# 77even/Fast-nnUNet

Measured on AMD Instinct MI355X. Metric: 3d_fullres patches/sec (distilled r=2 student, sliding window, one 512^3 CT; volume resident in HBM at step start; step ends with: fp16 logits resident in HBM), higher is better.
Workload: dtype f16; 1 GPU; bone_turbo_r2: PlainConvUNet student r=2, features [16, 32, 64, 128, 160, 160], 1 input channel, patch 160x96x96, 61 classes, 512^3 volume, tile_step_size 0.5, Gaussian on, mirroring off, 600 patches/volume; patches_per_forward=32, folds=1, accumulators=fp16, step_output=fp16 logits [heads, X, Y, Z] in HBM (predict_sliding_window_return_logits), gpu_max_hw_queues=4, parallelism=single GPU

## Files before the change

fast-nnunet_amd/csrc/conv3d.hip:

```cpp
#include "fnn_device.h"
#include "conv_common.h"
#include <cstdlib>

template <int NB>
__global__ __launch_bounds__(256) void conv3d_mfma_kernel(const ConvParams p) {
    extern __shared__ __attribute__((aligned(16))) char smem[];
    const int tid = threadIdx.x, lane = tid & 63, wave = tid >> 6;

    int t = blockIdx.x;
    const int tw = t % p.tiles_w; t /= p.tiles_w;
    const int th = t % p.tiles_h; t /= p.tiles_h;
    const int td = t % p.tiles_d;
    const int n = t / p.tiles_d;
    const int cb0 = blockIdx.y * NB;

    const int od0 = td * FNN_TILE_D, oh0 = th * FNN_TILE_H, ow0 = tw * FNN_TILE_W;
    const int ID = (FNN_TILE_D - 1) * p.sd + p.kd;
    const int IH = (FNN_TILE_H - 1) * p.sh + p.kh;
    const int IW = (FNN_TILE_W - 1) * p.sw + p.kw;
    const int IVOX = ID * IH * IW;
    const int T = p.kd * p.kh * p.kw;
    const int cin_total = p.chunks * 16;

    char *sA = smem;
    char *sB = sA + ((IVOX * 32 + 1023) & ~1023);
    int *sOff = (int *)(sB + p.ksteps * NB * 1024);
    float2 *sSS = (float2 *)(sOff + ((IVOX + 3) & ~3));
    int *sTap = (int *)(sSS + cin_total);

    {
        const int id0 = od0 * p.sd - p.pd, ih0 = oh0 * p.sh - p.ph, iw0 = ow0 * p.sw - p.pw;
        for (int v = tid; v < IVOX; v += 256) {
            const int zw = v % IW, zh = (v / IW) % IH, zd = v / (IW * IH);
            const int gd = id0 + zd, gh = ih0 + zh, gw = iw0 + zw;
            const bool ok = gd >= 0 && gd < p.Di && gh >= 0 && gh < p.Hi && gw >= 0 && gw < p.Wi;
            sOff[v] = ok ? ((n * p.Di + gd) * p.Hi + gh) * p.Wi + gw : -1;
        }
        if (tid < 2 * p.ksteps) {
            int off = 0;
            if (tid < T) {
                const int a = tid / (p.kh * p.kw), b = (tid / p.kw) % p.kh, c = tid % p.kw;
                off = ((a * IH + b) * IW + c) * 32;
            }
            sTap[tid] = off;
        }
        for (int c = tid; c < cin_total; c += 256) {
            const int s = (c < p.src[0].C) ? 0 : 1;
            const int cl = c - (s ? p.src[0].C : 0);
            sSS[c] = p.src[s].ss ? make_float2(p.src[s].ss[(size_t)(2 * n) * p.src[s].C + cl], p.src[s].ss[(size_t)(2 * n + 1) * p.src[s].C + cl])
                                 : make_float2(1.f, 0.f);
        }
    }

    int base[4];
#pragma unroll
    for (int mb = 0; mb < 4; ++mb) {
        const int r = lane & 15;
        const int oh_l = 2 * mb + (r >> 3), ow_l = r & 7;
        base[mb] = ((wave * p.sd * IH + oh_l * p.sh) * IW + ow_l * p.sw) * 32 + ((lane >> 4) & 1) * 16;
    }

    f32x4 acc[4][NB];
#pragma unroll
    for (int mb = 0; mb < 4; ++mb)
#pragma unroll
        for (int nb = 0; nb < NB; ++nb) acc[mb][nb] = (f32x4){0.f, 0.f, 0.f, 0.f};

    __syncthreads();

    const int cg = tid & 1;
    for (int ch = 0; ch < p.chunks; ++ch) {
        const int c_glob = ch * 16;
        const int s = (c_glob < p.src[0].C) ? 0 : 1;
        const int c_loc = c_glob - (s ? p.src[0].C : 0) + cg * 8;
        const int sC = p.src[s].C;
        const size_t nvox = (size_t)n * p.Di * p.Hi * p.Wi;
        const int vs = FNN_VS(p.src[s]);
        const f16 *sp = p.src[s].ptr + nvox * sC + (c_loc >> 4) * FNN_CS(p.src[s]) + (c_loc & 15);
        const f16 slope_h = (f16)p.src[s].slope;
        float sc[8], sh[8];
#pragma unroll
        for (int j = 0; j < 8; ++j) {
            const float2 v = sSS[c_glob + cg * 8 + j];
            sc[j] = v.x; sh[j] = v.y;
        }
        for (int base = tid; base < IVOX * 2; base += 256 * 8) {
            int off[8];
            f16x8 x[8];
#pragma unroll
            for (int u = 0; u < 8; ++u) {
                const int idx = base + u * 256;
                off[u] = idx < IVOX * 2 ? sOff[idx >> 1] : -2;
            }
#pragma unroll
            for (int u = 0; u < 8; ++u)
                x[u] = *(const f16x8 *)(sp + (off[u] >= 0 ? (size_t)off[u] - nvox : 0) * vs);
#pragma unroll
            for (int u = 0; u < 8; ++u) {
                if (off[u] == -2) continue;
                f16x8 o;
                if (off[u] >= 0) {
#pragma unroll
                    for (int j = 0; j < 8; ++j) o[j] = (f16)fmaf((float)x[u][j], sc[j], sh[j]);
                    o = __builtin_elementwise_max(o, o * slope_h);
                } else {
#pragma unroll
                    for (int j = 0; j < 8; ++j) o[j] = (f16)0.f;
                }
                *(f16x8 *)(sA + ((base + u * 256) >> 1) * 32 + cg * 16) = o;
            }
        }
        {
            const int per_nb = p.ksteps * 64;
            const int total = NB * per_nb;
            for (int base = tid; base < total; base += 256 * 8) {
                uint4 v[8];
#pragma unroll
                for (int u = 0; u < 8; ++u) {
                    const int idx = base + u * 256;
                    const int idc = idx < total ? idx : 0;
                    const int nb = idc / per_nb, r = idc - nb * per_nb;
                    v[u] = ((const uint4 *)(p.wpk + ((size_t)((cb0 + nb) * p.chunks + ch) * p.ksteps) * 512))[r];
                }
#pragma unroll
                for (int u = 0; u < 8; ++u) {
                    const int idx = base + u * 256;
                    if (idx < total) ((uint4 *)sB)[idx] = v[u];
                }
            }
        }
        __syncthreads();

        for (int ks = 0; ks < p.ksteps; ++ks) {
            const int toff = sTap[2 * ks + (lane >> 5)];
            f16x8 xf[4];
#pragma unroll
            for (int mb = 0; mb < 4; ++mb) xf[mb] = *(const f16x8 *)(sA + base[mb] + toff);
#pragma unroll
            for (int nb = 0; nb < NB; ++nb) {
                const f16x8 wf = *(const f16x8 *)(sB + ((nb * p.ksteps + ks) * 64 + lane) * 16);
#pragma unroll
                for (int mb = 0; mb < 4; ++mb)
                    acc[mb][nb] = __builtin_amdgcn_mfma_f32_16x16x32_f16(wf, xf[mb], acc[mb][nb], 0, 0, 0);
            }
        }
        __syncthreads();
    }

    const int q = lane >> 4, r = lane & 15;
    const int od = od0 + wave;
    float s1[NB][4], s2[NB][4];
#pragma unroll
    for (int nb = 0; nb < NB; ++nb)
#pragma unroll
        for (int j = 0; j < 4; ++j) { s1[nb][j] = 0.f; s2[nb][j] = 0.f; }

#pragma unroll
    for (int mb = 0; mb < 4; ++mb) {
        const int oh = oh0 + 2 * mb + (r >> 3), ow = ow0 + (r & 7);
        const bool ok = od < p.Do && oh < p.Ho && ow < p.Wo;
        const size_t vox = ((size_t)od * p.Ho + oh) * p.Wo + ow;
        f16 *outn = p.out + (size_t)n * p.Do * p.Ho * p.Wo * p.Cout;
#pragma unroll
        for (int nb = 0; nb < NB; ++nb) {
            const int co = (cb0 + nb) * 16 + q * 4;
            const float4 bv = *(const float4 *)(p.bias + co);
            f16x4 o;
            o[0] = (f16)(acc[mb][nb][0] + bv.x);
            o[1] = (f16)(acc[mb][nb][1] + bv.y);
            o[2] = (f16)(acc[mb][nb][2] + bv.z);
            o[3] = (f16)(acc[mb][nb][3] + bv.w);
            if (ok) {
                *(f16x4 *)(outn + vox * FNN_OVS(p) + (co >> 4) * FNN_OCS(p) + (co & 15)) = o;
#pragma unroll
                for (int j = 0; j < 4; ++j) {
                    const float v = (float)o[j];
                    s1[nb][j] += v; s2[nb][j] += v * v;
                }
            }
        }
    }
    if (p.stats_out) {
#pragma unroll
        for (int nb = 0; nb < NB; ++nb)
#pragma unroll
            for (int j = 0; j < 4; ++j) {
#pragma unroll
                for (int m = 1; m < 16; m <<= 1) {
                    s1[nb][j] += __shfl_xor(s1[nb][j], m, 64);
                    s2[nb][j] += __shfl_xor(s2[nb][j], m, 64);
                }
            }
        float *sRed = (float *)smem;
        if (r == 0) {
#pragma unroll
            for (int nb = 0; nb < NB; ++nb)
#pragma unroll
                for (int j = 0; j < 4; ++j) {
                    const int c = nb * 16 + q * 4 + j;
                    sRed[(wave * NB * 16 + c) * 2] = s1[nb][j];
                    sRed[(wave * NB * 16 + c) * 2 + 1] = s2[nb][j];
                }
        }
        __syncthreads();
        if (tid < NB * 16 * 2) {
            const int c = tid >> 1, which = tid & 1;
            double v = 0;
#pragma unroll
            for (int w = 0; w < 4; ++w) v += (double)sRed[(w * NB * 16 + c) * 2 + which];
            double *dst = p.stats_out + (((size_t)n * FNN_STAT_REPL + (blockIdx.x & (FNN_STAT_REPL - 1))) * p.Cout
                                         + cb0 * 16 + c) * 2 + which;
            unsafeAtomicAdd(dst, v);
        }
    }
}

static int lds_pitch(int IW) { return (IW & 7) ? ((IW + 3) & ~7) + 4 : IW; }

template <int NB, int MB, int PF>
__global__ __launch_bounds__(256, 2) void conv3d_lds_kernel(const ConvParams p) {
    extern __shared__ __attribute__((aligned(16))) char smem[];
    const int tid = threadIdx.x, lane = tid & 63, wave = tid >> 6;
    FNN_STAMP_DECL
    FNN_STAMP();
    constexpr int TD = MB == 2 ? 2 : MB;

    int t = fnn_xcd_tile(gridDim.x, blockIdx.x);
    const int tw = t % p.tiles_w; t /= p.tiles_w;
    const int th = t % p.tiles_h; t /= p.tiles_h;
    const int td = t % p.tiles_d;
    const int n = t / p.tiles_d;
    const int cb0 = blockIdx.y * NB;

    const int od0 = td * TD, oh0 = th * FNN_TILE_H, ow0 = tw * FNN_TILE_W;
    const int ID = (TD - 1) * p.sd + p.kd, IH = (FNN_TILE_H - 1) * p.sh + p.kh, IW = (FNN_TILE_W - 1) * p.sw + p.kw;
    const int IVOX = ID * IH * IW;
    const int T = p.kd * p.kh * p.kw;
    const int swz = p.sw == 1 && (IW & 7) != 0;
    const int PWp = swz ? ((IW + 3) & ~7) + 4 : IW;
    const int abytes = (ID * IH * PWp * 32 + 1023) & ~1023;

    constexpr int WPF = (NB * 14 * 64 + 255) / 256;
    char *sA0 = smem;
    char *sW = smem + abytes;
    int *sTap = (int *)(sW + NB * p.ksteps * 1024);
    float *sBias = (float *)(sTap + 4 * p.ksteps + 4);

    {
        if (tid < 2 * p.ksteps) {
            int off = 0, par = 0;
            if (tid < T) {
                const int a = tid / (p.kh * p.kw), b = (tid / p.kw) % p.kh, c = tid % p.kw;
                off = ((a * IH + b) * PWp + c) * 32;
                par = swz & b & 1;
            }
            sTap[tid * 2] = off + 16 * par;
            sTap[tid * 2 + 1] = off + 16 * (1 - par);
        }
        if (tid >= 64 && tid < 64 + NB * 16) sBias[tid - 64] = p.bias[cb0 * 16 + tid - 64];
    }

    int base[MB];
#pragma unroll
    for (int mb = 0; mb < MB; ++mb) {
        const int r = lane & 15;
        int od_l, oh_l, ow_l;
        mb_coords<MB>(wave, mb, r, od_l, oh_l, ow_l);
        base[mb] = ((od_l * p.sd * IH + oh_l * p.sh) * PWp + ow_l * p.sw) * 32;
    }
    const int kgp = ((lane >> 4) & 1) ^ (swz & ((lane & 15) >> 3));

    f32x4 acc[MB][NB];
#pragma unroll
    for (int mb = 0; mb < MB; ++mb)
#pragma unroll
        for (int nb = 0; nb < NB; ++nb) acc[mb][nb] = (f32x4){0.f, 0.f, 0.f, 0.f};

    const int per_nb = p.ksteps * 64;
    const int wtotal = NB * per_nb;
    f16x8 wr[WPF];
    int wofs[WPF];
#pragma unroll
    for (int u = 0; u < WPF; ++u) {
        const int idx = tid + u * 256;
        const int idc = idx < wtotal ? idx : wtotal - 1;
        const int nb = (idc >= per_nb) + (idc >= 2 * per_nb) + (idc >= 3 * per_nb);
        wofs[u] = (cb0 + nb) * p.chunks * per_nb + idc - nb * per_nb;
    }
    float4 scr[2], shr[2];
    float slope_next = 1.f;
    __syncthreads();

    const int cg = tid & 1;
    int offv[PF];
    int ldso[PF];
    {
        const int id0 = od0 * p.sd - p.pd, ih0 = oh0 * p.sh - p.ph, iw0 = ow0 * p.sw - p.pw;
        const float rcp_iw = 1.0f / (float)IW, rcp_ih = 1.0f / (float)IH;
#pragma unroll
        for (int u = 0; u < PF; ++u) {
            const int idx = tid + u * 256;
            const int v = idx >> 1;
            const int row = small_div(v, IW, rcp_iw), zw = v - row * IW;
            const int zd = small_div(row, IH, rcp_ih), zh = row - zd * IH;
            const int gd = id0 + zd, gh = ih0 + zh, gw = iw0 + zw;
            const bool ok = gd >= 0 && gd < p.Di && gh >= 0 && gh < p.Hi && gw >= 0 && gw < p.Wi;
            offv[u] = idx < IVOX * 2 ? (ok ? ((n * p.Di + gd) * p.Hi + gh) * p.Wi + gw : -1) : -2;
            ldso[u] = ((zd * IH + zh) * PWp + zw) * 32 + ((cg ^ (swz & zh & 1)) * 16);
        }
    }
    f16x8 xr[PF];

    auto issue = [&](int ch) {
        const int c_glob = ch * 16;
        const int s = (c_glob < p.src[0].C) ? 0 : 1;
        const int sC = p.src[s].C, c_loc = c_glob - (s ? p.src[0].C : 0) + cg * 8;
        const size_t nvox = (size_t)n * p.Di * p.Hi * p.Wi;
        const int vs = FNN_VS(p.src[s]);
        const f16 *sp = p.src[s].ptr + nvox * sC + (c_loc >> 4) * FNN_CS(p.src[s]) + (c_loc & 15);
#pragma unroll
        for (int u = 0; u < PF; ++u)
            xr[u] = *(const f16x8 *)(sp + (offv[u] >= 0 ? (size_t)offv[u] - nvox : 0) * vs);
#pragma unroll
        for (int u = 0; u < WPF; ++u) wr[u] = ((const f16x8 *)p.wpk)[wofs[u] + ch * per_nb];
        slope_next = p.src[s].slope;
        if (p.src[s].ss) {
            const float *q4 = p.src[s].ss + (size_t)(2 * n) * sC + (c_glob - (s ? p.src[0].C : 0)) + cg * 8;
            scr[0] = *(const float4 *)q4; scr[1] = *(const float4 *)(q4 + 4);
            shr[0] = *(const float4 *)(q4 + sC); shr[1] = *(const float4 *)(q4 + sC + 4);
        } else {
            scr[0] = scr[1] = make_float4(1.f, 1.f, 1.f, 1.f);
            shr[0] = shr[1] = make_float4(0.f, 0.f, 0.f, 0.f);
        }
    };
    auto commit = [&](int ch, char *dst) {
        (void)ch;
        const f16 slope_h = (f16)slope_next;
        const float sc[8] = {scr[0].x, scr[0].y, scr[0].z, scr[0].w, scr[1].x, scr[1].y, scr[1].z, scr[1].w};
        const float sh[8] = {shr[0].x, shr[0].y, shr[0].z, shr[0].w, shr[1].x, shr[1].y, shr[1].z, shr[1].w};
#pragma unroll
        for (int u = 0; u < PF; ++u) {
            if (u * 256 >= IVOX * 2 || offv[u] == -2) continue;
            f16x8 o;
            if (offv[u] >= 0) {
#pragma unroll
                for (int j = 0; j < 8; ++j) o[j] = (f16)fmaf((float)xr[u][j], sc[j], sh[j]);
                o = __builtin_elementwise_max(o, o * slope_h);
            } else {
#pragma unroll
                for (int j = 0; j < 8; ++j) o[j] = (f16)0.f;
            }
            *(f16x8 *)(dst + ldso[u]) = o;
        }
#pragma unroll
        for (int u = 0; u < WPF; ++u) {
            const int idx = tid + u * 256;
            if (idx < wtotal) ((f16x8 *)sW)[idx] = wr[u];
        }
    };

    FNN_STAMP();
    issue(0);
    FNN_STAMP();
    commit(0, sA0);
    __syncthreads();
    FNN_STAMP();

    auto kloop = [&]() {
        for (int ks = 0; ks < p.ksteps; ++ks) {
            const int toff = sTap[(2 * ks + (lane >> 5)) * 2 + kgp];
            f16x8 xf[MB];
#pragma unroll
            for (int mb = 0; mb < MB; ++mb) xf[mb] = *(const f16x8 *)(sA0 + base[mb] + toff);
#pragma unroll
            for (int nb = 0; nb < NB; ++nb) {
                const f16x8 wf = *(const f16x8 *)(sW + ((nb * p.ksteps + ks) * 64 + lane) * 16);
#pragma unroll
                for (int mb = 0; mb < MB; ++mb)
                    acc[mb][nb] = __builtin_amdgcn_mfma_f32_16x16x32_f16(wf, xf[mb], acc[mb][nb], 0, 0, 0);
            }
        }
    };
    for (int ch = 0; ch + 1 < p.chunks; ++ch) {
        issue(ch + 1);
        kloop();
        FNN_STAMP();
        __syncthreads();
        commit(ch + 1, sA0);
        __syncthreads();
        FNN_STAMP();
    }
    kloop();
    FNN_STAMP();
    __syncthreads();

    {
        float4 bv[NB];
#pragma unroll
        for (int nb = 0; nb < NB; ++nb) bv[nb] = *(const float4 *)(sBias + nb * 16 + (lane >> 4) * 4);
        float t1[NB][4], t2[NB][4];
#pragma unroll
        for (int nb = 0; nb < NB; ++nb)
#pragma unroll
            for (int j = 0; j < 4; ++j) { t1[nb][j] = 0.f; t2[nb][j] = 0.f; }
        tile_epilogue<NB, MB>(p, acc, bv, n, od0, oh0, ow0, cb0, wave, lane, t1, t2);
        if (p.stats_out) stats_to_global<NB>(p, t1, t2, (float *)smem, n, cb0, wave, lane, tid);
    }
    FNN_STAMP();
    FNN_STAMP_FLUSH(p.dbg);
}

static size_t ldsk_lds_bytes(const ConvParams &p, int nb, int mb) {
    const int td = mb == 2 ? 2 : mb;
    const int ID = (td - 1) * p.sd + p.kd, IH = (FNN_TILE_H - 1) * p.sh + p.kh, IW = (FNN_TILE_W - 1) * p.sw + p.kw;
    const int pitch = p.sw == 1 ? lds_pitch(IW) : IW;
    size_t b = (size_t)((ID * IH * pitch * 32 + 1023) & ~1023) + (size_t)nb * p.ksteps * 1024;
    b += 4 * p.ksteps * 4 + 16 + (size_t)nb * 16 * 4 + 64;
    const size_t red = (size_t)4 * nb * 16 * 2 * 4;
    return b > red ? b : red;
}

template <int NB, int MB, int PF = 8>
static int launch_ldsk(ConvParams p, hipStream_t st) {
    constexpr int TD = MB == 2 ? 2 : MB;
    p.tile_d = TD;
    p.tiles_d = (p.Do + TD - 1) / TD;
    p.tiles_h = (p.Ho + FNN_TILE_H - 1) / FNN_TILE_H;
    p.tiles_w = (p.Wo + FNN_TILE_W - 1) / FNN_TILE_W;
    const size_t lds = ldsk_lds_bytes(p, NB, MB);
    dim3 grid(p.N * p.tiles_d * p.tiles_h * p.tiles_w, (p.Cout / 16) / NB);
    return fnn_launch_lds<conv3d_lds_kernel<NB, MB, PF>>(grid, dim3(256), lds, st, p);
}

template <int NB, int MB, bool WRES, int KS, int CH, int PF = 8, bool SBUF = false>
__global__ __launch_bounds__(256, (NB == 1 && MB == 4 && WRES && PF == 4) ? 3 : 2) void conv3d_persist_kernel(const ConvParams p, const int total_tiles) {
    extern __shared__ __attribute__((aligned(16))) char smem[];
    const int tid = threadIdx.x, lane = tid & 63, wave = tid >> 6;
    FNN_STAMP_DECL
    constexpr int TD = MB;

    const int ID = (TD - 1) * p.sd + p.kd, IH = (FNN_TILE_H - 1) * p.sh + p.kh, IW = (FNN_TILE_W - 1) * p.sw + p.kw;
    const int IVOX = ID * IH * IW;
    const int T = p.kd * p.kh * p.kw;
    const int TS = p.chunks * p.ksteps;
    const int swz = p.sw == 1 && (IW & 7) != 0;
    const int PWp = swz ? ((IW + 3) & ~7) + 4 : IW;
    const int abytes = (ID * IH * PWp * 32 + 1023) & ~1023;
    const int cb0 = blockIdx.y * NB;

    constexpr int NBUF = (WRES && !SBUF) ? 2 : 1;
    constexpr int WPF = WRES ? 1 : (NB * 14 * 64 + 255) / 256;
    char *sA0 = smem;
    char *sW = smem + NBUF * abytes;
    int *sTap = (int *)(sW + NB * (WRES ? TS : p.ksteps) * 1024);
    double *sRed = (double *)(sTap + 64);

    int t_begin, t_end;
    {
        const int nwg = gridDim.x, bid = blockIdx.x;
        const int g = fnn_xcd_tile(nwg, bid);
        t_begin = (int)((long long)total_tiles * g / nwg);
        t_end = (int)((long long)total_tiles * (g + 1) / nwg);
    }
    if (t_begin >= t_end) return;

    if (WRES) {
        for (int idx = tid; idx < NB * TS * 64; idx += 256) {
            const int nb = idx / (TS * 64), r = idx - nb * (TS * 64);
            ((uint4 *)sW)[idx] = ((const uint4 *)(p.wpk + (size_t)(cb0 + nb) * TS * 512))[r];
        }
    }
    const int per_nb = p.ksteps * 64, wtotal = NB * per_nb;
    f16x8 wr[WPF];
    int wofs[WPF];
#pragma unroll
    for (int u = 0; u < WPF; ++u) {
        const int idx = tid + u * 256;
        const int idc = idx < wtotal ? idx : wtotal - 1;
        const int nb = idc / per_nb, r = idc - nb * per_nb;
        wofs[u] = (cb0 + nb) * p.chunks * per_nb + r;
    }
    if (tid < 2 * p.ksteps) {
        int off = 0, par = 0;
        if (tid < T) {
            const int a = tid / (p.kh * p.kw), b = (tid / p.kw) % p.kh, c = tid % p.kw;
            off = ((a * IH + b) * PWp + c) * 32;
            par = swz & b & 1;
        }
        sTap[tid * 2] = off + 16 * par;
        sTap[tid * 2 + 1] = off + 16 * (1 - par);
    }
    const int cg = tid & 1;
    constexpr bool REL_LDS = false && PF >= 12;
    int *sRel = (int *)(sRed + 4 * NB * 16 * 2) + tid;
    int relr[REL_LDS ? 1 : PF];
#pragma unroll
    for (int u = 0; u < PF; ++u) {
        const int idx = tid + u * 256;
        const int v = idx >> 1;
        const int zw = v % IW, zh = (v / IW) % IH, zd = v / (IW * IH);
        const int rv = idx < IVOX * 2 ? (zd << 16) | (zh << 8) | zw : -1;
        if (REL_LDS) sRel[u * 256] = rv; else relr[REL_LDS ? 0 : u] = rv;
    }
#define FNN_REL(u) (REL_LDS ? sRel[(u) * 256] : relr[REL_LDS ? 0 : (u)])
    int base[MB];
#pragma unroll
    for (int mb = 0; mb < MB; ++mb) {
        const int r = lane & 15;
        int od_l, oh_l, ow_l;
        mb_coords<MB>(wave, mb, r, od_l, oh_l, ow_l);
        base[mb] = ((od_l * p.sd * IH + oh_l * p.sh) * PWp + ow_l * p.sw) * 32;
    }
    const int kgp = ((lane >> 4) & 1) ^ (swz & ((lane & 15) >> 3));

    f32x4 acc[MB][NB];
    for (int i = tid; i < 4 * NB * 16 * 2; i += 256) sRed[i] = 0.0;
    double dsum[NB][4][2];
#pragma unroll
    for (int nb = 0; nb < NB; ++nb)
#pragma unroll
        for (int j = 0; j < 4; ++j) { dsum[nb][j][0] = 0.0; dsum[nb][j][1] = 0.0; }

    float4 bv[NB];
#pragma unroll
    for (int nb = 0; nb < NB; ++nb) bv[nb] = *(const float4 *)(p.bias + (cb0 + nb) * 16 + (lane >> 4) * 4);

    int offv[PF];
    f16x8 xr[PF];
    float4 scr[2], shr[2];
    float slope_next = 1.f;

    auto tile_coords = [&](int t, int &n, int &od0, int &oh0, int &ow0) {
        const int tw = t % p.tiles_w; t /= p.tiles_w;
        const int th = t % p.tiles_h; t /= p.tiles_h;
        const int td = t % p.tiles_d;
        n = t / p.tiles_d;
        od0 = td * TD; oh0 = th * FNN_TILE_H; ow0 = tw * FNN_TILE_W;
    };
    auto next_tile = [&](int &n, int &od0, int &oh0, int &ow0) {
        ow0 += FNN_TILE_W;
        if (ow0 >= p.tiles_w * FNN_TILE_W) {
            ow0 = 0; oh0 += FNN_TILE_H;
            if (oh0 >= p.tiles_h * FNN_TILE_H) {
                oh0 = 0; od0 += TD;
                if (od0 >= p.tiles_d * TD) { od0 = 0; ++n; }
            }
        }
    };
    auto set_offsets = [&](int od0, int oh0, int ow0) {
        const int id0 = od0 * p.sd - p.pd, ih0 = oh0 * p.sh - p.ph, iw0 = ow0 * p.sw - p.pw;
#pragma unroll
        for (int u = 0; u < PF; ++u) {
            const int rel_u = FNN_REL(u);
            const unsigned gd = (unsigned)(id0 + (rel_u >> 16)), gh = (unsigned)(ih0 + ((rel_u >> 8) & 255)),
                           gw = (unsigned)(iw0 + (rel_u & 255));
            const bool ok = rel_u >= 0 && gd < (unsigned)p.Di && gh < (unsigned)p.Hi && gw < (unsigned)p.Wi;
            offv[u] = ok ? (int)(__umul24(__umul24(gd, (unsigned)p.Hi) + gh, (unsigned)p.Wi) + gw) : -1;
        }
    };
    auto issue = [&](int n, int ch) {
        const int c_glob = ch * 16;
        const int s = (c_glob < p.src[0].C) ? 0 : 1;
        const int c_loc = c_glob - (s ? p.src[0].C : 0) + cg * 8;
        const int sC = p.src[s].C;
        const int vs = FNN_VS(p.src[s]);
        const char *sp = (const char *)(p.src[s].ptr + (size_t)n * p.Di * p.Hi * p.Wi * sC + (c_loc >> 4) * FNN_CS(p.src[s]) + (c_loc & 15));
        slope_next = p.src[s].slope;
        const float *qs = p.src[s].ss ? p.src[s].ss + (size_t)(2 * n) * sC + c_loc : p.ident_ss + c_loc;
        const float *qh = p.src[s].ss ? qs + sC : p.ident_ss + 512 + c_loc;
        scr[0] = *(const float4 *)qs; scr[1] = *(const float4 *)(qs + 4);
        shr[0] = *(const float4 *)qh; shr[1] = *(const float4 *)(qh + 4);
        __builtin_amdgcn_sched_barrier(0);
#pragma unroll
        for (int u = 0; u < PF; ++u)
            xr[u] = *(const f16x8 *)(sp + (unsigned)((offv[u] >= 0 ? offv[u] : 0) * vs * 2));
        if (!WRES) {
#pragma unroll
            for (int u = 0; u < WPF; ++u) wr[u] = ((const f16x8 *)p.wpk)[wofs[u] + ch * per_nb];
        }
    };
    auto commit = [&](char *dst) {
        const f16 slope_h = (f16)slope_next;
        const float sc[8] = {scr[0].x, scr[0].y, scr[0].z, scr[0].w, scr[1].x, scr[1].y, scr[1].z, scr[1].w};
        const float sh[8] = {shr[0].x, shr[0].y, shr[0].z, shr[0].w, shr[1].x, shr[1].y, shr[1].z, shr[1].w};
#pragma unroll
        for (int u = 0; u < PF; ++u) {
            if (u * 256 >= IVOX * 2) continue;
            f16x8 o = fnn_norm_leaky8(xr[u], sc, sh, slope_h);
            if (offv[u] < 0) o = (f16x8){0, 0, 0, 0, 0, 0, 0, 0};
            const int rel_u = FNN_REL(u);
            const int zd = rel_u >> 16, zh = (rel_u >> 8) & 255, zw = rel_u & 255;
            if (rel_u >= 0) *(f16x8 *)(dst + ((zd * IH + zh) * PWp + zw) * 32 + ((cg ^ (swz & zh & 1)) * 16)) = o;
        }
        if (!WRES) {
#pragma unroll
            for (int u = 0; u < WPF; ++u) {
                const int idx = tid + u * 256;
                if (idx < wtotal) ((f16x8 *)sW)[idx] = wr[u];
            }
        }
    };
    auto flush_stats = [&](int n) {
        if (!p.stats_out) return;
        {
            const int q = lane >> 4;
#pragma unroll
            for (int nb = 0; nb < NB; ++nb)
#pragma unroll
                for (int j = 0; j < 4; ++j) {
                    const double a = row16_sum_f64(dsum[nb][j][0]), b = row16_sum_f64(dsum[nb][j][1]);
                    if ((lane & 15) == 0) {
                        double *slot = sRed + (wave * NB * 16 + nb * 16 + q * 4 + j) * 2;
                        slot[0] = a; slot[1] = b;
                    }
                    dsum[nb][j][0] = 0.0; dsum[nb][j][1] = 0.0;
                }
        }
        __syncthreads();
        if (tid < NB * 16 * 2) {
            const int c = tid >> 1, which = tid & 1;
            double v = 0;
#pragma unroll
            for (int w = 0; w < 4; ++w) { v += sRed[(w * NB * 16 + c) * 2 + which]; sRed[(w * NB * 16 + c) * 2 + which] = 0.0; }
            unsafeAtomicAdd(p.stats_out + (((size_t)n * FNN_STAT_REPL + (blockIdx.x & (FNN_STAT_REPL - 1))) * p.Cout
                                           + cb0 * 16 + c) * 2 + which, v);
        }
        __syncthreads();
    };

    int n_cur, od0, oh0, ow0;
    tile_coords(t_begin, n_cur, od0, oh0, ow0);
    set_offsets(od0, oh0, ow0);
    issue(n_cur, 0);
    commit(sA0);
    __syncthreads();
    int toffs[14];
    if (KS) {
#pragma unroll
        for (int ks = 0; ks < (KS < 14 ? KS : 14); ++ks) toffs[ks] = sTap[(2 * ks + (lane >> 5)) * 2 + kgp];
    }

    int buf = 0;
    for (int t = t_begin; t < t_end; ++t) {
#pragma unroll
        for (int mb = 0; mb < MB; ++mb)
#pragma unroll
            for (int nb = 0; nb < NB; ++nb) acc[mb][nb] = (f32x4){0.f, 0.f, 0.f, 0.f};
        int n_next = n_cur, nod0 = od0, noh0 = oh0, now0 = ow0;
        constexpr int CHU = CH ? CH : 1;
#pragma unroll CHU
        for (int ch = 0; ch < (CH ? CH : p.chunks); ++ch) {
#ifdef FNN_STAMPS
            const bool stamp_it = t == t_begin + 2 && ch == 0;
            if (stamp_it) FNN_STAMP();
#endif
            const bool last_chunk = ch + 1 == (CH ? CH : p.chunks);
            if (last_chunk) {
                if (t + 1 < t_end) next_tile(n_next, nod0, noh0, now0);
                set_offsets(nod0, noh0, now0);
                issue(n_next, 0);
            } else {
                issue(n_cur, ch + 1);
            }
#ifdef FNN_STAMPS
            if (stamp_it) FNN_STAMP();
#endif
            const char *sA = sA0 + (NBUF == 2 ? buf * abytes : 0);
#pragma unroll
            for (int ks = 0; ks < (KS ? KS : p.ksteps); ++ks) {
                const int toff = KS ? toffs[ks < 14 ? ks : 0] : sTap[(2 * ks + (lane >> 5)) * 2 + kgp];
                f16x8 xf[MB];
#pragma unroll
                for (int mb = 0; mb < MB; ++mb) xf[mb] = *(const f16x8 *)(sA + base[mb] + toff);
#pragma unroll
                for (int nb = 0; nb < NB; ++nb) {
                    const f16x8 wf = *(const f16x8 *)(sW + ((size_t)(WRES ? nb * TS + ch * p.ksteps + ks : nb * p.ksteps + ks) * 64 + lane) * 16);
#pragma unroll
                    for (int mb = 0; mb < MB; ++mb)
                        acc[mb][nb] = __builtin_amdgcn_mfma_f32_16x16x32_f16(wf, xf[mb], acc[mb][nb], 0, 0, 0);
                }
            }
#ifdef FNN_STAMPS
            if (stamp_it) FNN_STAMP();
#endif
            if (last_chunk) {
                float t1[NB][4], t2[NB][4];
#pragma unroll
                for (int nb = 0; nb < NB; ++nb)
#pragma unroll
                    for (int j = 0; j < 4; ++j) { t1[nb][j] = 0.f; t2[nb][j] = 0.f; }
                tile_epilogue<NB, MB>(p, acc, bv, n_cur, od0, oh0, ow0, cb0, wave, lane, t1, t2);
                if (p.stats_out) {
#pragma unroll
                    for (int nb = 0; nb < NB; ++nb)
#pragma unroll
                        for (int j = 0; j < 4; ++j) {
                            dsum[nb][j][0] += (double)t1[nb][j];
                            dsum[nb][j][1] += (double)t2[nb][j];
                        }
                }
                if (NBUF == 1) __syncthreads();
                commit(sA0 + (NBUF == 2 ? (buf ^ 1) * abytes : 0));
            } else {
                if (NBUF == 1) __syncthreads();
                commit(sA0 + (NBUF == 2 ? (buf ^ 1) * abytes : 0));
            }
#ifdef FNN_STAMPS
            if (stamp_it) FNN_STAMP();
#endif
            __syncthreads();
#ifdef FNN_STAMPS
            if (stamp_it) FNN_STAMP();
#endif
            buf ^= 1;
        }
        if (n_next != n_cur || t + 1 == t_end) flush_stats(n_cur);
        n_cur = n_next; od0 = nod0; oh0 = noh0; ow0 = now0;
    }
    FNN_STAMP_FLUSH(p.dbg);
#undef FNN_REL
}

static size_t persist_lds_bytes(const ConvParams &p, int nb, int mb, bool wres, bool sbuf = false, int pf = 8) {
    const int ID = (mb - 1) * p.sd + p.kd, IH = (FNN_TILE_H - 1) * p.sh + p.kh, IW = (FNN_TILE_W - 1) * p.sw + p.kw;
    const size_t ab = (size_t)((ID * IH * (p.sw == 1 ? lds_pitch(IW) : IW) * 32 + 1023) & ~1023);
    return (wres && !sbuf ? 2 : 1) * ab + (size_t)nb * (wres ? p.chunks : 1) * p.ksteps * 1024 + 256 + (size_t)4 * nb * 16 * 2 * 8 +
           (false && pf >= 12 ? (size_t)pf * 256 * 4 : 0);
}

template <int NB, int MB, bool WRES, int KS, int CH = 0, int PF = 8, bool SBUF = false>
static int launch_persist_ks(ConvParams p, int wgs_per_cu, hipStream_t st, int gx_exact = 0) {
    p.tile_d = MB;
    p.tiles_d = (p.Do + MB - 1) / MB;
    p.tiles_h = (p.Ho + FNN_TILE_H - 1) / FNN_TILE_H;
    p.tiles_w = (p.Wo + FNN_TILE_W - 1) / FNN_TILE_W;
    const int total = p.N * p.tiles_d * p.tiles_h * p.tiles_w;
    p.ident_ss = conv3d_identity_ss();
    if (!p.ident_ss) return -2;
    const size_t lds = persist_lds_bytes(p, NB, MB, WRES, SBUF, PF);
    int gx = gx_exact > 0 ? gx_exact : 256 * wgs_per_cu;
    if (gx > total) gx = total;
    dim3 grid(gx, (p.Cout / 16) / NB);
    return fnn_launch_lds<conv3d_persist_kernel<NB, MB, WRES, KS, CH, PF, SBUF>>(grid, dim3(256), lds, st, p, total);
}

static int launch_persist(const ConvParams &p, const ConvChoice &c, hipStream_t st) {
    const int mb = c.t[1], wres = c.t[2], ks = c.t[3], ch = c.t[4];
    if (c.t[0] == 2) return launch_persist_ks<2, 2, true, 0, 1, 12, true>(p, c.wpc, st, c.gx);
    if (ch == 1) return launch_persist_ks<1, 4, true, 5, 1, 4>(p, c.wpc, st);
    if (ch == 2) return launch_persist_ks<1, 4, true, 5, 2, 4>(p, c.wpc, st);
    if (mb == 8) {
        if (wres) return ks == 5 ? launch_persist_ks<1, 8, true, 5>(p, c.wpc, st) : launch_persist_ks<1, 8, true, 0>(p, c.wpc, st);
        return ks == 5 ? launch_persist_ks<1, 8, false, 5>(p, c.wpc, st) : launch_persist_ks<1, 8, false, 14>(p, c.wpc, st);
    }
    if (wres) return ks == 5 ? launch_persist_ks<1, 4, true, 5>(p, c.wpc, st) : launch_persist_ks<1, 4, true, 0>(p, c.wpc, st);
    return launch_persist_ks<1, 4, false, 5>(p, c.wpc, st);
}

size_t conv3d_lds_bytes(const ConvParams &p, int nb) {
    const int ID = (FNN_TILE_D - 1) * p.sd + p.kd;
    const int IH = (FNN_TILE_H - 1) * p.sh + p.kh;
    const int IW = (FNN_TILE_W - 1) * p.sw + p.kw;
    const int IVOX = ID * IH * IW;
    size_t b = (size_t)((IVOX * 32 + 1023) & ~1023);
    b += (size_t)p.ksteps * nb * 1024;
    b += (size_t)((IVOX + 3) & ~3) * 4;
    b += (size_t)p.chunks * 16 * 8;
    b += 2 * p.ksteps * 4 + 64;
    const size_t red = (size_t)4 * nb * 16 * 2 * 4;
    return b > red ? b : red;
}

const float *conv3d_identity_ss() {
    static const float *tab[16] = {nullptr};
    int dev = 0;
    if (hipGetDevice(&dev) != hipSuccess || dev < 0 || dev >= 16) return nullptr;
    if (!tab[dev]) {
        float h[1024];
        for (int i = 0; i < 512; ++i) { h[i] = 1.f; h[512 + i] = 0.f; }
        float *d = nullptr;
        if (hipMalloc((void **)&d, sizeof(h)) != hipSuccess) return nullptr;
        if (hipMemcpy(d, h, sizeof(h), hipMemcpyHostToDevice) != hipSuccess) { (void)hipFree(d); return nullptr; }
        tab[dev] = d;
    }
    return tab[dev];
}

const unsigned short *conv3d_identity_ssh() {
    static const unsigned short *tab[16] = {nullptr};
    int dev = 0;
    if (hipGetDevice(&dev) != hipSuccess || dev < 0 || dev >= 16) return nullptr;
    if (!tab[dev]) {
        unsigned short h[1024];
        for (int i = 0; i < 1024; ++i) h[i] = (i & 8) ? 0 : 0x3c00;
        unsigned short *d = nullptr;
        if (hipMalloc((void **)&d, sizeof(h)) != hipSuccess) return nullptr;
        if (hipMemcpy(d, h, sizeof(h), hipMemcpyHostToDevice) != hipSuccess) { (void)hipFree(d); return nullptr; }
        tab[dev] = d;
    }
    return tab[dev];
}

int conv3d_pick_nb(int nblk) { return (nblk % 4 == 0) ? 4 : (nblk % 2 == 0) ? 2 : 1; }

template <int NB>
static int launch_conv_nb(ConvParams p, hipStream_t st) {
    p.tile_d = FNN_TILE_D;
    p.tiles_d = (p.Do + FNN_TILE_D - 1) / FNN_TILE_D;
    p.tiles_h = (p.Ho + FNN_TILE_H - 1) / FNN_TILE_H;
    p.tiles_w = (p.Wo + FNN_TILE_W - 1) / FNN_TILE_W;
    const size_t lds = conv3d_lds_bytes(p, NB);
    dim3 grid(p.N * p.tiles_d * p.tiles_h * p.tiles_w, (p.Cout / 16) / NB);
    return fnn_launch_lds<conv3d_mfma_kernel<NB>>(grid, dim3(256), lds, st, p);
}

static void set_persist(ConvChoice &c, int nb, int mb, int wres, int ks, int ch, int pf, int sbuf, int wpc) {
    c.kernel = CK_PERSIST;
    const int t[7] = {nb, mb, wres, ks, ch, pf, sbuf};
    for (int i = 0; i < 7; ++i) c.t[i] = t[i];
    c.wpc = wpc;
    snprintf(c.name, sizeof c.name, "conv3d_persist_kernel<%d,%d,%d,%d,%d,%d,%d>", nb, mb, wres, ks, ch, pf, sbuf);
}

static void set_ldsk(ConvChoice &c, int nb, int mb, int pf) {
    c.kernel = CK_LDSK; c.t[0] = nb; c.t[1] = mb; c.t[2] = pf;
    snprintf(c.name, sizeof c.name, "conv3d_lds_kernel<%d,%d,%d>", nb, mb, pf);
}

static bool conv_choose_linear(const ConvParams &p_in, const ConvOverrides &o, ConvChoice &c) {
    ConvParams p = p_in;
    c.packing = FNN_PACK_LINEAR; c.ksteps = conv3d_ksteps(FNN_PACK_LINEAR, p.kd * p.kh * p.kw); c.chunks = p.chunks;
    p.ksteps = c.ksteps;
    p.tiles_h = (p.Ho + FNN_TILE_H - 1) / FNN_TILE_H;
    p.tiles_w = (p.Wo + FNN_TILE_W - 1) / FNN_TILE_W;
    const int plan_n = p.plan_N > 0 ? p.plan_N : p.N;
    int nb = conv3d_pick_nb(p.Cout / 16);
    if (!o.conv_v1 && p.sd == 1 && p.sh == 1 && p.sw == 1) {
        const int nblk = p.Cout / 16;
        const int cand[4][2] = {{2, 8}, {2, 4}, {1, 8}, {1, 4}};
        int pick = -1, best = -1;
        long long best_wgs = -1;
        for (int i = 0; i < 4; ++i) {
            const int cnb = cand[i][0], cmb = cand[i][1];
            if (nblk % cnb) continue;
            if (cmb == 8 && p.Do < 8) continue;
            const long long wgs = (long long)plan_n * ((p.Do + cmb - 1) / cmb) * p.tiles_h * p.tiles_w * (nblk / cnb);
            if (pick < 0 && wgs >= 768) pick = i;
            if (wgs > best_wgs) { best_wgs = wgs; best = i; }
        }
        if (pick < 0) pick = best;
        nb = cand[pick][0];
        const int mbsel = cand[pick][1];
        if (p.ksteps <= 14 && nb == 1) {
            for (int mb = mbsel; mb >= 4; mb -= 4) {
                const long long tiles = (long long)plan_n * ((p.Do + mb - 1) / mb) * p.tiles_h * p.tiles_w;
                if (tiles < 256LL * 2 * 4) continue;
                for (int wres = 1; wres >= 0; --wres) {
                    if (!wres && !(p.ksteps == 5 || (p.ksteps == 14 && mb == 8))) continue;
                    const size_t lds = persist_lds_bytes(p, nb, mb, wres != 0);
                    const int per_cu = (int)((160 * 1024) / lds);
                    if (per_cu < 2) continue;
                    const int wpc = per_cu > 3 ? 3 : per_cu;
                    if (wres && mb == 8 && p.ksteps == 5 && (p.chunks == 1 || p.chunks == 2)) {
                        const int ivox4 = (3 * p.sd + p.kd) * ((FNN_TILE_H - 1) * p.sh + p.kh) * ((FNN_TILE_W - 1) * p.sw + p.kw);
                        if (ivox4 * 2 <= 4 * 256 && persist_lds_bytes(p, 1, 4, true) * 3 <= 160 * 1024) {
                            set_persist(c, 1, 4, 1, 5, p.chunks, 4, 0, 3);
                            return true;
                        }
                    }
                    set_persist(c, 1, mb, wres, p.ksteps == 5 ? 5 : wres ? 0 : 14, 0, 8, 0, wpc);
                    return true;
                }
            }
        }
        if (p.ksteps <= 14) {
            set_ldsk(c, nb, mbsel, 8);
            return true;
        }
    }
    if (!o.conv_v1 && s2_choose(p, c)) return true;
    if (!o.conv_v1 && p.ksteps <= 14) {
        const int nbs = (p.Cout / 16) % 2 == 0 ? 2 : 1;
        const int ID = (2 - 1) * p.sd + p.kd, IH = (FNN_TILE_H - 1) * p.sh + p.kh, IW = (FNN_TILE_W - 1) * p.sw + p.kw;
        const long long tiles = (long long)plan_n * ((p.Do + 1) / 2) * p.tiles_h * p.tiles_w;
        const int groups = (p.Cout / 16) / nbs;
        if (nbs == 2 && ID * IH * IW * 2 <= 12 * 256 && persist_lds_bytes(p, 2, 2, false, false, 12) <= 80 * 1024 &&
            tiles >= 8LL * (512 / groups) && 512 / groups >= 8 && p.chunks == 1 && persist_lds_bytes(p, 2, 2, true, true, 12) <= 80 * 1024) {
            set_persist(c, 2, 2, 1, 0, 1, 12, 1, 2);
            c.gx = 512 / groups;
            return true;
        }
        if (ID * IH * IW * 2 <= 16 * 256 && ldsk_lds_bytes(p, nbs, 2) <= 80 * 1024) {
            set_ldsk(c, nbs, 2, ID * IH * IW * 2 <= 8 * 256 ? 8 : 16);
            return true;
        }
    }
    if (nb == 4 && conv3d_lds_bytes(p, 4) > 160 * 1024) nb = 2;
    if (conv3d_lds_bytes(p, nb) > 160 * 1024) return false;
    c.kernel = CK_NB; c.t[0] = nb;
    snprintf(c.name, sizeof c.name, "conv3d_mfma_kernel<%d> (generic fallback)", nb);
    return true;
}

ConvOverrides ConvOverrides::from_env() {
    ConvOverrides o;
    o.conv_v1 = fnn_knob("FNN_CONV_V1") != nullptr;
    o.no_row = fnn_knob("FNN_NO_ROW") != nullptr;
    o.no_stem_row = fnn_knob("FNN_NO_STEM_ROW") != nullptr;
    o.no_zr6 = fnn_knob("FNN_NO_ZR6") != nullptr;
    o.no_zrp = fnn_knob("FNN_NO_ZRP") != nullptr;
    o.no_zq12 = fnn_knob("FNN_NO_ZQ12") != nullptr;
    o.no_zsw = fnn_knob("FNN_NO_ZSW") != nullptr;
    o.no_zp = fnn_knob("FNN_NO_ZP") != nullptr;
    o.zp_no_half = fnn_knob("FNN_ZP_NO_HALF") != nullptr;
    o.zps_no_half = fnn_knob("FNN_ZPS_NO_HALF") != nullptr;
    if (const char *v = fnn_knob("FNN_ZR_MIN_WGS")) o.zr_min_wgs = atoi(v);
    if (const char *v = fnn_knob("FNN_FP8_LEVELS")) o.fp8_levels = atoi(v);
    return o;
}

bool conv_choose(const ThinParams &tp, const ConvOverrides &o, ConvChoice &c) {
    c = ConvChoice{};
    if (tp.fuse) {
        ConvChoice t;
        if (!thin_choose(tp, t)) return false;
        if (!row_choose(tp, o, c)) c = t;
        return true;
    }
    const ConvParams &p = tp.c;
    const unsigned long long out_item = 2ull * p.Do * p.Ho * p.Wo * p.Cout;
    unsigned long long in_item = 0;
    for (int i = 0; i < p.n_src; ++i) {
        const unsigned long long b = 2ull * p.Di * p.Hi * p.Wi * p.src[i].C;
        in_item = b > in_item ? b : in_item;
    }
    if (out_item >= (1ull << 31) || in_item >= (1ull << 32) || (long long)p.Di * p.Hi >= (1 << 24) || p.Wi >= (1 << 24)) return false;
    if (zp_choose(p, o, c) || zr_choose(p, o, c)) return true;
    c = ConvChoice{};
    return row_choose(tp, o, c) || conv_choose_linear(p, o, c);
}

bool conv_choose_fp8(ThinParams &tp, const ConvOverrides &o, ConvChoice &c) {
    ConvParams &p = tp.c;
    if (p.fp8 && !(p.kd * p.kh * p.kw == 27 && p.sd == 1 && p.sh == 1 && p.sw == 1)) p.fp8 = 0;
    bool ok = conv_choose(tp, o, c);
    if (p.fp8 && c.packing != FNN_PACK_ZR) { p.fp8 = 0; ok = conv_choose(tp, o, c); }
    return ok;
}

int launch_conv(const ThinParams &tp_in, const ConvChoice &c, hipStream_t st) {
    if (c.kernel == CK_ROW_STEM && tp_in.Y * tp_in.Z >= (1ll << 30)) {
        ConvChoice t;
        return thin_choose(tp_in, t) ? launch_conv(tp_in, t, st) : -1;
    }
    fnn_note_kernel("%s", c.name);
    ThinParams tp = tp_in;
    ConvParams &p = tp.c;
    p.packing = c.packing; p.ksteps = c.ksteps; p.chunks = c.chunks; p.stats_slots = c.stats_slots;
    switch (c.kernel) {
        case CK_ZS: case CK_ZSP: case CK_ZSW: case CK_ZR: case CK_ZR8: case CK_ZQ12: case CK_ZR12: case CK_ZRW:
            return launch_conv3d_zr(p, c, st);
        case CK_ZP: case CK_ZPS: return launch_conv2d_zp(p, c, st);
        case CK_ROW: case CK_ROW_STEM: return launch_conv_row(tp, c, st);
        case CK_THIN: return launch_conv_thin(tp, c, st);
        case CK_PERSIST: return launch_persist(p, c, st);
        case CK_LDSK:
            if (c.t[1] == 2) {
                if (c.t[2] == 8) return c.t[0] == 2 ? launch_ldsk<2, 2, 8>(p, st) : launch_ldsk<1, 2, 8>(p, st);
                return c.t[0] == 2 ? launch_ldsk<2, 2, 16>(p, st) : launch_ldsk<1, 2, 16>(p, st);
            }
            if (c.t[0] == 1) return c.t[1] == 8 ? launch_ldsk<1, 8>(p, st) : launch_ldsk<1, 4>(p, st);
            return c.t[1] == 8 ? launch_ldsk<2, 8>(p, st) : launch_ldsk<2, 4>(p, st);
        case CK_S2: return launch_conv3d_s2(p, c, st);
        case CK_NB: return c.t[0] == 4 ? launch_conv_nb<4>(p, st) : c.t[0] == 2 ? launch_conv_nb<2>(p, st) : launch_conv_nb<1>(p, st);
    }
    return -1;
}
```

fast-nnunet_amd/csrc/conv3d_zq.hip:

```cpp
#include "fnn_device.h"
#include "conv_zr_common.h"
#include <cstdlib>

namespace {

typedef unsigned zq_u32x4 __attribute__((ext_vector_type(4)));

constexpr int ZQ_TD = 8, ZQ_ID = ZQ_TD + 2, ZQ_IH = 14, ZQ_IW = 14;
using Zq12Lds = Zr12Lds<ZQ_TD, 8>;
constexpr int ZQ_PW = Zq12Lds::PW, ZQ_PS = Zq12Lds::PS;
constexpr int ZQ_ABYTES = Zq12Lds::image;
constexpr int ZQ_KS = 15, ZQ_WB = ZQ_KS * 64;
constexpr int ZQ_NT = 512, ZQ_NB = 2;
constexpr int ZQ_WBYTES = Zq12Lds::weights;

__global__ __launch_bounds__(512, 2) void conv3d_zq12_kernel(const ConvParams p) {
    extern __shared__ __attribute__((aligned(16))) char smem[];
    const int tid = threadIdx.x, lane = tid & 63, wave = __builtin_amdgcn_readfirstlane(tid >> 6);
    const int dq = wave >> 1, grp = (wave ^ (wave >> 2)) & 1;
    const int nblk = grp ? 4 : 5, b0 = grp ? 5 : 0;
    const int td = blockIdx.x % p.tiles_d, n = blockIdx.x / p.tiles_d;
    const int cb0 = blockIdx.y * ZQ_NB;
    const int od0 = td * ZQ_TD;

    char *sA = smem;
    char *sW = smem + ZQ_ABYTES;
    float *sRed = (float *)(sW + ZQ_WBYTES);

    const int col = tid >> 1, cg = tid & 1;
    const int zh = (col * 2341) >> 15, zw = col - zh * ZQ_IW;
    const bool has_col = tid < 2 * ZQ_IH * ZQ_IW;
    const int gh = zh - 1, gw = zw - 1;
    const bool ok_hw = has_col & ((unsigned)gh < (unsigned)p.Hi) & ((unsigned)gw < (unsigned)p.Wi);
    const int hw_lin = __mul24(gh, p.Wi) + gw;
    const int ldso0 = (zh * ZQ_PW + zw) * 32 + ((cg ^ (zh & 1)) * 16);
    const int wlds = ZQ_ABYTES + tid * 16;
    unsigned pmask = (1u << ZQ_ID) - 1;
    if (od0 == 0) pmask &= ~1u;
    {
        const int over = od0 + ZQ_TD + 1 - p.Di;
        if (over > 0) pmask &= (1u << (ZQ_ID - over)) - 1;
    }
    pmask = __builtin_amdgcn_readfirstlane(pmask);

    f32x4 acc[5][2][ZQ_NB];
    zq_u32x4 xr[ZQ_ID], wr[ZQ_NB][2];
    zq_u32x4 ssv[2];
    float slope_next = 1.f;
    __amdgpu_buffer_rsrc_t rx, rw[ZQ_NB];
    unsigned voff = 0x80000000u, plane_bytes = 0;
    auto prep = [&](int ch) {
        const int c_glob = ch * 16;
        const int s = (c_glob < p.src[0].C) ? 0 : 1;
        const int c_uni = c_glob - (s ? p.src[0].C : 0);
        const int sC = p.src[s].C;
        const int vs = FNN_VS(p.src[s]);
        const unsigned item_bytes = (unsigned)p.Di * p.Hi * p.Wi * sC * 2;
        const f16 *sp = p.src[s].ptr + (size_t)n * (item_bytes >> 1) + (c_uni >> 4) * FNN_CS(p.src[s]);
        rx = __builtin_amdgcn_make_buffer_rsrc((void *)sp, 0, item_bytes, 0x00020000);
        slope_next = p.src[s].slope;
        {
            const zq_u32x4 *qv = (const zq_u32x4 *)(fnn_ssh_rows(p.src[s].ssh, sC, n, c_uni, p.ident_ssh) + cg * 16);
            ssv[0] = qv[0]; ssv[1] = qv[1];
        }
        voff = ok_hw ? (unsigned)hw_lin * (unsigned)(vs * 2) + cg * 16 : 0x80000000u;
        plane_bytes = (unsigned)p.Hi * p.Wi * vs * 2;
#pragma unroll
        for (int nb = 0; nb < ZQ_NB; ++nb) {
            const f16 *wp = p.wpk + ((size_t)((cb0 + nb) * p.chunks + ch) * ZQ_WB) * 8;
            rw[nb] = __builtin_amdgcn_make_buffer_rsrc((void *)wp, 0, ZQ_WB * 16, 0x00020000);
        }
    };
    auto load_part = [&](int part) {
#pragma unroll
        for (int u = 0; u < ZQ_ID; ++u) {
            if (u * 5 / ZQ_ID != part) continue;
            int gd = od0 - 1 + u;
            gd = gd < 0 ? 0 : (gd >= p.Di ? p.Di - 1 : gd);
            xr[u] = __builtin_bit_cast(zq_u32x4, __builtin_amdgcn_raw_buffer_load_b128(rx, voff, (unsigned)gd * plane_bytes, 0));
        }
#pragma unroll
        for (int e = 0; e < ZQ_NB * 2; ++e) {
            if (e * 5 / (ZQ_NB * 2) != part) continue;
            const int nb = e >> 1, u = e & 1;
            wr[nb][u] = __builtin_bit_cast(zq_u32x4, __builtin_amdgcn_raw_buffer_load_b128(rw[nb], tid * 16, u * 8192, 0));
        }
    };
    auto commit = [&]() {
        const f16 slope_h = (f16)slope_next;
        const zq_u32x4 zero4 = {0u, 0u, 0u, 0u};
        const f16x8 sc_h = __builtin_bit_cast(f16x8, ok_hw ? ssv[0] : zero4), sh_h = __builtin_bit_cast(f16x8, ok_hw ? ssv[1] : zero4);
        if (has_col) {
#pragma unroll
            for (int u = 0; u < ZQ_ID; ++u)
                *(f16x8 *)(sA + ldso0 + u * ZQ_PS) = fnn_norm_leaky8(__builtin_bit_cast(f16x8, xr[u]), sc_h, sh_h, slope_h);
            if (pmask != (1u << ZQ_ID) - 1) {
                unsigned pm = pmask;
                asm volatile("" : "+s"(pm));
#pragma unroll
                for (int u = 0; u < ZQ_ID; ++u)
                    if (!((pm >> u) & 1)) *(f16x8 *)(sA + ldso0 + u * ZQ_PS) = (f16x8){0, 0, 0, 0, 0, 0, 0, 0};
            }
        }
#pragma unroll
        for (int nb = 0; nb < ZQ_NB; ++nb) {
            *(zq_u32x4 *)(smem + wlds + nb * ZQ_WB * 16) = wr[nb][0];
            if (tid < ZQ_WB - 512) *(zq_u32x4 *)(smem + wlds + (nb * ZQ_WB + 512) * 16) = wr[nb][1];
        }
    };

    int toff[5];
    zr_tap_offsets<ZQ_PW, true>(toff, lane, [](int r) { return r >> 2; }, [](int r) { return r & 3; }, dq * 2 * ZQ_PS);
    int boff[5];
#pragma unroll
    for (int i = 0; i < 5; ++i) {
        const int b = b0 + i, bh = (b * 11) >> 5, bw = b - bh * 3;
        boff[i] = __builtin_amdgcn_readfirstlane((4 * bh * ZQ_PW + 4 * bw) * 32);
    }

    auto read_x = [&](f16x8 (&xf)[4], int pr, int i) {
        const char *bp = sA + toff[pr] + boff[i];
#pragma unroll
        for (int pl = 0; pl < 4; ++pl) xf[pl] = *(const f16x8 *)(bp + pl * ZQ_PS);
    };
    auto kloop = [&](bool prefetch) {
#pragma unroll
        for (int pr = 0; pr < 5; ++pr) {
            if (prefetch) load_part(pr);
            f16x8 wf[3][ZQ_NB];
#pragma unroll
            for (int dz = 0; dz < 3; ++dz)
#pragma unroll
                for (int nb = 0; nb < ZQ_NB; ++nb) wf[dz][nb] = *(const f16x8 *)(sW + ((nb * ZQ_KS + pr * 3 + dz) * 64 + lane) * 16);
            f16x8 xa[4], xb[4];
            read_x(xa, pr, 0);
#pragma unroll
            for (int i = 0; i < 5; ++i) {
                f16x8 (&cur)[4] = (i & 1) ? xb : xa;
                f16x8 (&nxt)[4] = (i & 1) ? xa : xb;
                if (i + 1 < 5 && (i + 1 < 4 || nblk == 5)) read_x(nxt, pr, i + 1);
                __builtin_amdgcn_sched_barrier(0);
                if (i < 4 || nblk == 5) {
#pragma unroll
                    for (int dz = 0; dz < 3; ++dz)
#pragma unroll
                        for (int j = 0; j < 2; ++j)
#pragma unroll
                            for (int nb = 0; nb < ZQ_NB; ++nb)
                                acc[i][j][nb] = __builtin_amdgcn_mfma_f32_16x16x32_f16(wf[dz][nb], cur[j + dz], acc[i][j][nb], 0, 0, 0);
                }
                __builtin_amdgcn_sched_barrier(0);
            }
        }
    };

    prep(0);
#pragma unroll
    for (int part = 0; part < 5; ++part) load_part(part);
    __builtin_amdgcn_sched_barrier(0);
#pragma unroll
    for (int i = 0; i < 5; ++i)
#pragma unroll
        for (int j = 0; j < 2; ++j)
#pragma unroll
            for (int nb = 0; nb < ZQ_NB; ++nb) acc[i][j][nb] = (f32x4){0.f, 0.f, 0.f, 0.f};
    commit();
    __syncthreads();
    for (int ch = 0; ch + 1 < p.chunks; ++ch) {
        prep(ch + 1);
        kloop(true);
        __syncthreads();
        commit();
        __syncthreads();
    }
    kloop(false);

    {
        const int q = lane >> 4, r = lane & 15;
        float4 bv[ZQ_NB];
#pragma unroll
        for (int nb = 0; nb < ZQ_NB; ++nb) bv[nb] = *(const float4 *)(p.bias + cb0 * 16 + q * 8 + nb * 4);
        float t1[ZQ_NB][4], t2[ZQ_NB][4];
#pragma unroll
        for (int nb = 0; nb < ZQ_NB; ++nb)
#pragma unroll
            for (int j = 0; j < 4; ++j) { t1[nb][j] = 0.f; t2[nb][j] = 0.f; }
#pragma unroll
        for (int i = 0; i < 5; ++i) {
            if (i == 4 && nblk == 4) break;
            const int b = b0 + i, bh = (b * 11) >> 5, bw = b - bh * 3;
            zr_epilogue_pair<2>(p, acc[i], bv, n, od0 + 2 * dq, 4 * bh + (r >> 2), 4 * bw + (r & 3), cb0, lane, t1, t2);
        }
        if (p.stats_out) {
#pragma unroll
            for (int nb = 0; nb < ZQ_NB; ++nb)
#pragma unroll
                for (int j = 0; j < 4; ++j) {
                    const float a = row16_sum(t1[nb][j]), b = row16_sum(t2[nb][j]);
                    if (r == 0) {
                        const int c = q * 8 + nb * 4 + j;
                        sRed[(wave * 32 + c) * 2] = a;
                        sRed[(wave * 32 + c) * 2 + 1] = b;
                    }
                }
            __syncthreads();
            if (tid < 64) {
                const int c = tid >> 1, which = tid & 1;
                double v = 0;
#pragma unroll
                for (int w = 0; w < 8; ++w) v += (double)sRed[(w * 32 + c) * 2 + which];
                p.stats_out[(((size_t)n * p.stats_slots + td) * p.Cout + cb0 * 16 + c) * 2 + which] = v;
            }
        }
    }
}

}

bool conv3d_zq12_fits(const ConvParams &p, int stats_slots) {
    if (p.fp8 || (p.Cout / 16) % 2 != 0 || p.Ho <= 8 || p.Ho > 12 || p.Wo <= 8 || p.Wo > 12 || p.Do < ZQ_TD) return false;
    if (((p.Do + 7) / 8) * 8 * 10 > ((p.Do + 3) / 4) * 4 * 11) return false;
    return stats_slots >= (p.Do + ZQ_TD - 1) / ZQ_TD;
}

int launch_conv3d_zq12(ConvParams p, hipStream_t st) {
    p.tile_d = ZQ_TD;
    p.tiles_d = (p.Do + ZQ_TD - 1) / ZQ_TD; p.tiles_h = 1; p.tiles_w = 1;
    p.ident_ss = conv3d_identity_ss();
    p.ident_ssh = conv3d_identity_ssh();
    if (!p.ident_ss || !p.ident_ssh) return -2;
    dim3 grid(p.N * p.tiles_d, (p.Cout / 16) / ZQ_NB);
    return fnn_launch_lds<conv3d_zq12_kernel>(grid, dim3(ZQ_NT), Zq12Lds::bytes(), st, p);
}
```

fast-nnunet_amd/csrc/conv3d_zr.hip:

```cpp
#include "fnn_device.h"
#include "conv_common.h"
#include "conv_zr_common.h"
#include <type_traits>
#include <cstdlib>

bool zr_choose(const ConvParams &p, const ConvOverrides &o, ConvChoice &c) {
    if (p.kd != 3 || p.kh != 3 || p.kw != 3 || p.sd != 1) return false;
    const int nblk = p.Cout / 16;
    const int plan_n = p.plan_N > 0 ? p.plan_N : p.N;
    c.packing = FNN_PACK_ZR; c.ksteps = 15; c.chunks = p.chunks;
    bool zr6_shape = false;
    if (p.sh == 2 && p.sw == 2) {
        if (p.fp8 || nblk % 2 != 0 || (long long)p.Di * p.Hi * p.Wi >= (1 << 23) || p.Do < 8) return false;
        const int tiles_d = (p.Do + 7) / 8, tiles_h = (p.Ho + 3) / 4, tiles_w = (p.Wo + 7) / 8, groups = nblk / 2;
        if ((long long)plan_n * tiles_d * tiles_h * tiles_w * (p.Cout / 32) < 768) return false;
        c.stats_slots = tiles_d * tiles_h * tiles_w;
        const bool persistent = p.chunks == 1 && p.n_src == 1 && plan_n * c.stats_slots >= 512 * 8;
        if (persistent && !o.no_zsw && tiles_d >= 4) {
            const long long cols = (long long)plan_n * tiles_h * tiles_w * groups;
            int segs = 1;
            while (cols * segs < 8 * 512 && segs * 2 <= tiles_d / 2) segs *= 2;
            c.tps = (tiles_d + segs - 1) / segs;
            c.segs = (tiles_d + c.tps - 1) / c.tps;
            c.kernel = CK_ZSW;
            snprintf(c.name, sizeof c.name, "conv3d_zsw_kernel");
        } else if (persistent) {
            c.gx = 512 / groups < 8 ? 8 : 512 / groups;
            c.kernel = CK_ZSP;
            snprintf(c.name, sizeof c.name, "conv3d_zsp_kernel");
        } else {
            c.kernel = CK_ZS; c.t[0] = 2;
            snprintf(c.name, sizeof c.name, "conv3d_zs_kernel<2>");
        }
        return true;
    }
    if (p.sh != 1 || p.sw != 1) return false;
    const long long vox = (long long)p.Do * p.Ho * p.Wo;
    if (vox >= (1 << 23)) return false;
    if (vox * 32 * (p.chunks > 0 ? p.chunks : 1) >= (1ll << 31) || vox * 2 * p.Cout >= (1ll << 31)) return false;
    const int nb = nblk % 2 == 0 ? 2 : 1;
    const int th = (p.Ho + 7) / 8, tw = (p.Wo + 7) / 8;
    zr6_shape = nb == 2 && !p.fp8 && p.Ho <= 6 && p.Wo <= 8 && p.Do >= 10 && p.Do % 10 == 0 &&
                (long long)plan_n * (p.Do / 10) * (nblk / 2) >= 160;
    if (zr6_shape && !o.no_zr6) {
        c.stats_slots = ((p.Do + 9) / 10) * th * tw;
        c.kernel = CK_ZR; c.t[0] = 2; c.t[1] = 10; c.t[2] = 6;
        snprintf(c.name, sizeof c.name, "conv3d_zr_kernel<%d,%d,%d>", 2, 10, 6);
        return true;
    }
    int td = 8;
    while (td >= 4 && (p.Do < td || (long long)plan_n * ((p.Do + td - 1) / td) * th * tw * (nblk / nb) < o.zr_min_wgs)) td -= 4;
    if (td < 4) return false;
    c.stats_slots = ((p.Do + td - 1) / td) * th * tw;
    c.t[0] = nb; c.t[1] = td;
    if (p.fp8) {
        c.kernel = CK_ZR8;
        snprintf(c.name, sizeof c.name, "conv3d_zr8_kernel<%d,%d>", nb, td);
    } else if (nb == 2 && !o.no_zq12 && conv3d_zq12_fits(p, c.stats_slots)) {
        c.kernel = CK_ZQ12;
        snprintf(c.name, sizeof c.name, "conv3d_zq12_kernel");
    } else if (nb == 2 && p.Ho > 8 && p.Ho <= 12 && p.Wo > 8 && p.Wo <= 12 && c.stats_slots >= (p.Do + 3) / 4) {
        c.kernel = CK_ZR12; c.t[0] = 4;
        snprintf(c.name, sizeof c.name, "conv3d_zr12_kernel<%d>", 4);
    } else if (p.chunks == 1 && td == 8 && (p.Do + 7) / 8 >= 4) {
        const int tiles_d = (p.Do + 7) / 8;
        const long long cols = (long long)plan_n * th * tw * (nblk / nb);
        int segs = 1;
        while (cols * segs < 2 * 768 && segs * 2 <= tiles_d / 2) segs *= 2;
        c.tps = (tiles_d + segs - 1) / segs;
        c.segs = (tiles_d + c.tps - 1) / c.tps;
        c.kernel = CK_ZRW;
        snprintf(c.name, sizeof c.name, "conv3d_zrw_kernel<%d>", nb);
    } else {
        c.kernel = CK_ZR;
        if (p.chunks >= 2 && !zr6_shape && !o.no_zrp) c.packing = FNN_PACK_ZRP;
        snprintf(c.name, sizeof c.name, "conv3d_zr_kernel<%d,%d>", nb, td);
    }
    return true;
}

typedef unsigned fnn_u32x4v __attribute__((ext_vector_type(4)));
template <int NB, int TD, int TH = 8>
__global__ __launch_bounds__(TH * 32, 2) void conv3d_zr_kernel(const ConvParams p) {
    extern __shared__ __attribute__((aligned(16))) char smem[];
    const int tid = threadIdx.x, lane = tid & 63, wave = __builtin_amdgcn_readfirstlane(tid >> 6);
    FNN_STAMP_DECL
    FNN_STAMP();
    constexpr int NT = TH * 32;
    using L = ZrLds<NB, TD, TH>;
    constexpr int IH = TH + 2, IW = 10, PW = L::PW, ID = TD + 2;
    constexpr int PS = L::PS, ABYTES = L::image;
    constexpr int KS = 15;
    constexpr int WB = KS * 64;
    constexpr int WPB = (WB + NT - 1) / NT;
    static_assert(WB - (WPB - 1) * NT == 192, "the last weight element group covers exactly waves 0 .. 2");

    int t = __builtin_amdgcn_readfirstlane(fnn_xcd_tile(gridDim.x, blockIdx.x));
    const int tw = __builtin_amdgcn_readfirstlane(t % p.tiles_w); t = __builtin_amdgcn_readfirstlane(t / p.tiles_w);
    const int th = __builtin_amdgcn_readfirstlane(t % p.tiles_h); t = __builtin_amdgcn_readfirstlane(t / p.tiles_h);
    const int td = __builtin_amdgcn_readfirstlane(t % p.tiles_d);
    const int n = __builtin_amdgcn_readfirstlane(t / p.tiles_d);
    const int cb0 = blockIdx.y * NB;
    const int od0 = td * TD, oh0 = th * 8, ow0 = tw * 8;

    char *sA = smem;
    char *sW = smem + ABYTES;

    const int col = tid >> 1, cg = tid & 1;
    const int zh = (col * 205) >> 11, zw = col - zh * IW;
    const bool has_col = tid < 2 * IH * IW;
    const int gh = oh0 - 1 + zh, gw = ow0 - 1 + zw;
    const bool ok_hw = has_col & ((unsigned)gh < (unsigned)p.Hi) & ((unsigned)gw < (unsigned)p.Wi);
    const int hw_lin = __mul24(gh, p.Wi) + gw;
    const int ldso0 = (zh * PW + zw) * 32 + ((cg ^ (zh & 1)) * 16);
    const int wlds = ABYTES + tid * 16;
    unsigned pmask = (1u << ID) - 1;
    if (od0 == 0) pmask &= ~1u;
    {
        const int over = od0 + TD + 1 - p.Di;
        if (over > 0) pmask &= (1u << (ID - over)) - 1;
    }
    pmask = __builtin_amdgcn_readfirstlane(pmask);

    f32x4 acc[TD][NB];
    fnn_u32x4v xr[ID], wr[NB][WPB];
    constexpr bool PAIR = TH == 8;
    const bool paired = PAIR && p.packing == FNN_PACK_ZRP;
    f16x8 xl[PAIR ? ID : 1];
#ifdef FNN_NORM_FP32
    float scu[16], shu[16];
#else
    fnn_u32x4v ssv[2];
#endif
    float slope_next = 1.f;
#ifdef FNN_TMODE
    bool first_chunk = true;
#endif

    __amdgpu_buffer_rsrc_t rx, rw[NB];
    unsigned voff = 0x80000000u, plane_bytes = 0;
    auto prep = [&](int ch) {
        const int c_glob = ch * 16;
        const int s = (c_glob < p.src[0].C) ? 0 : 1;
        const int c_uni = c_glob - (s ? p.src[0].C : 0);
        const int sC = p.src[s].C;
        const int vs = FNN_VS(p.src[s]);
        const unsigned item_bytes = (unsigned)p.Di * p.Hi * p.Wi * sC * 2;
        const f16 *sp = p.src[s].ptr + (size_t)n * (item_bytes >> 1) + (c_uni >> 4) * FNN_CS(p.src[s]);
        rx = __builtin_amdgcn_make_buffer_rsrc((void *)sp, 0, item_bytes, 0x00020000);
        slope_next = p.src[s].slope;
#ifdef FNN_NORM_FP32
        const float *qs, *qh;
        fnn_ss_rows(p.src[s].ss, sC, n, c_uni, p.ident_ss, qs, qh);
#pragma unroll
        for (int j = 0; j < 16; ++j) { scu[j] = qs[j]; shu[j] = qh[j]; }
#else
        {
            const fnn_u32x4v *qv = (const fnn_u32x4v *)(fnn_ssh_rows(p.src[s].ssh, sC, n, c_uni, p.ident_ssh) + cg * 16);
            ssv[0] = qv[0]; ssv[1] = qv[1];
        }
#endif
        voff = ok_hw ? (unsigned)hw_lin * (unsigned)(vs * 2) + cg * 16 : 0x80000000u;
        plane_bytes = (unsigned)p.Hi * p.Wi * vs * 2;
        const int wbytes = paired && ch % 2 == 0 && ch + 1 < p.chunks ? 12 * 64 * 16 : WB * 16;
#pragma unroll
        for (int nb = 0; nb < NB; ++nb) {
            const f16 *wp = p.wpk + ((size_t)((cb0 + nb) * p.chunks + ch) * WB) * 8;
            rw[nb] = __builtin_amdgcn_make_buffer_rsrc((void *)wp, 0, wbytes, 0x00020000);
        }
    };
#ifndef FNN_ZR_SLICES
#define FNN_ZR_SLICES 5
#endif
    constexpr int SL = FNN_ZR_SLICES;
    auto load_part = [&](int part) {
#pragma unroll
        for (int u = 0; u < ID; ++u) {
            if (u * SL / ID != part) continue;
            int gd = od0 - 1 + u;
            gd = gd < 0 ? 0 : (gd >= p.Di ? p.Di - 1 : gd);
            xr[u] = __builtin_bit_cast(fnn_u32x4v, __builtin_amdgcn_raw_buffer_load_b128(rx, voff, (unsigned)gd * plane_bytes, 0));
        }
#ifdef FNN_TMODE
        if ((p.tmode & 8) && !first_chunk) return;
#endif
#pragma unroll
        for (int e = 0; e < NB * WPB; ++e) {
            if (e * SL / (NB * WPB) != part) continue;
            const int nb = e / WPB, u = e % WPB;
            wr[nb][u] = __builtin_bit_cast(fnn_u32x4v, __builtin_amdgcn_raw_buffer_load_b128(rw[nb], tid * 16, u * (NT * 16), 0));
        }
    };
    auto commit = [&]() {
        const f16 slope_h = (f16)slope_next;
#ifdef FNN_NORM_FP32
        float sc[8], sh[8];
#pragma unroll
        for (int j = 0; j < 8; ++j) {
            sc[j] = ok_hw ? (cg ? scu[8 + j] : scu[j]) : 0.f;
            sh[j] = ok_hw ? (cg ? shu[8 + j] : shu[j]) : 0.f;
        }
#else
        const fnn_u32x4v zero4 = {0u, 0u, 0u, 0u};
        const f16x8 sc = __builtin_bit_cast(f16x8, ok_hw ? ssv[0] : zero4), sh = __builtin_bit_cast(f16x8, ok_hw ? ssv[1] : zero4);
#endif
        if (has_col) {
#pragma unroll
            for (int u = 0; u < ID; ++u)
                *(f16x8 *)(sA + ldso0 + u * PS) = fnn_norm_leaky8(__builtin_bit_cast(f16x8, xr[u]), sc, sh, slope_h);
            if (pmask != (1u << ID) - 1) {
                unsigned pm = pmask;
#ifdef FNN_NORM_FP32
                pm = __builtin_amdgcn_readfirstlane(pm);
#endif
                asm volatile("" : "+s"(pm));
#pragma unroll
                for (int u = 0; u < ID; ++u)
                    if (!((pm >> u) & 1)) *(f16x8 *)(sA + ldso0 + u * PS) = (f16x8){0, 0, 0, 0, 0, 0, 0, 0};
            }
        }
#ifdef FNN_TMODE
        if ((p.tmode & 8) && !first_chunk) return;
#endif
#pragma unroll
        for (int nb = 0; nb < NB; ++nb)
#pragma unroll
            for (int u = 0; u < WPB; ++u)
                if (u + 1 < WPB || wave < 3) *(fnn_u32x4v *)(smem + wlds + (nb * WB + u * NT) * 16) = wr[nb][u];
    };
    int toff[5];
    const bool khalf1 = lane >= 32;
    auto kloop = [&](bool prefetch, auto mode_c) __attribute__((always_inline)) {
        constexpr int MODE = decltype(mode_c)::value;
#pragma unroll
        for (int i = 0; i < 5; ++i) {
            const int pr = MODE == 2 ? (i + 4) % 5 : i;
            if (prefetch && i < SL) load_part(i);
            const char *bp = sA + toff[pr];
            if (MODE == 1 && pr == 4) {
#pragma unroll
                for (int pl = 0; pl < ID; ++pl) xl[pl] = *(const f16x8 *)(bp + pl * PS);
                break;
            }
            f16x8 xf[ID];
#pragma unroll
            for (int pl = 0; pl < ID; ++pl) xf[pl] = *(const f16x8 *)(bp + pl * PS);
            if (MODE == 2 && pr == 4) {
#pragma unroll
                for (int pl = 0; pl < ID; ++pl) xf[pl] = khalf1 ? xf[pl] : xl[pl];
            }
            zr_pair_mfma<TD, NB, KS>(acc, xf, sW, pr, lane);
        }
    };
    prep(0);
#pragma unroll
    for (int part = 0; part < SL; ++part) load_part(part);
    __builtin_amdgcn_sched_barrier(0);
    FNN_STAMP();
    {
        f32x4 b0[NB];
#pragma unroll
        for (int nb = 0; nb < NB; ++nb)
            b0[nb] = *(const f32x4 *)(p.bias + cb0 * 16 + (NB == 2 ? (lane >> 4) * 8 + nb * 4 : nb * 16 + (lane >> 4) * 4));
#pragma unroll
        for (int j = 0; j < TD; ++j)
#pragma unroll
            for (int nb = 0; nb < NB; ++nb) acc[j][nb] = b0[nb];
    }
    {
        const int r = lane & 15, hl = lane >> 5, kh = (lane >> 4) & 1;
#pragma unroll
        for (int pr = 0; pr < 5; ++pr) {
            const int tp = 2 * pr + hl < 9 ? 2 * pr + hl : 8;
            const int row = 2 * wave + (r >> 3) + tp / 3, col2 = (r & 7) + tp % 3;
            toff[pr] = (row * PW + col2) * 32 + ((kh ^ (row & 1)) * 16);
        }
    }

    commit();
#ifdef FNN_TMODE
    first_chunk = false;
#endif
    __syncthreads();
    FNN_STAMP();
    using M0 = std::integral_constant<int, 0>;
    using M1 = std::integral_constant<int, 1>;
    using M2 = std::integral_constant<int, 2>;
    auto next_chunk = [&](int ch, auto mode_c) __attribute__((always_inline)) {
        prep(ch + 1);
        kloop(true, mode_c);
        FNN_STAMP();
        __syncthreads();
        commit();
        __syncthreads();
        FNN_STAMP();
    };
    if (PAIR && paired) {
        int ch = 0;
        for (; ch + 2 < p.chunks; ch += 2) {
            next_chunk(ch, M1{});
            next_chunk(ch + 1, M2{});
        }
        if (ch + 1 < p.chunks) {
            next_chunk(ch, M1{});
            kloop(false, M2{});
        } else {
            kloop(false, M0{});
        }
    } else {
        for (int ch = 0; ch + 1 < p.chunks; ++ch) next_chunk(ch, M0{});
        kloop(false, M0{});
    }
    FNN_STAMP();
    __syncthreads();

    {
        float4 bv[NB];
#pragma unroll
        for (int nb = 0; nb < NB; ++nb) bv[nb] = make_float4(0.f, 0.f, 0.f, 0.f);
        float t1[NB][4], t2[NB][4];
#pragma unroll
        for (int nb = 0; nb < NB; ++nb)
#pragma unroll
            for (int j = 0; j < 4; ++j) { t1[nb][j] = 0.f; t2[nb][j] = 0.f; }
        if constexpr (NB == 2) zr_epilogue_pair<TD, false>(p, acc, bv, n, od0, oh0 + 2 * wave + ((lane & 15) >> 3), ow0 + (lane & 7), cb0, lane, t1, t2);
        else tile_epilogue<NB, TD, true, false>(p, acc, bv, n, od0, oh0, ow0, cb0, wave, lane, t1, t2);
        if (p.stats_out) stats_to_global<NB, true, NB == 2, TH / 2>(p, t1, t2, (float *)smem, n, cb0, wave, lane, tid, (td * p.tiles_h + th) * p.tiles_w + tw);
    }
    FNN_STAMP();
    FNN_STAMP_FLUSH(p.dbg);
}


template <int NB>
__global__ __launch_bounds__(256, NB == 1 ? 3 : 2) void conv3d_zrw_kernel(const ConvParams p, const int segs, const int tps) {
    extern __shared__ __attribute__((aligned(16))) char smem[];
    const int tid = threadIdx.x, lane = tid & 63, wave = __builtin_amdgcn_readfirstlane(tid >> 6);
    using L = ZrLds<NB, 8>;
    constexpr int TD = 8, IH = 10, IW = 10, PW = L::PW, ID = TD + 2;
    constexpr int PS = L::PS, ABYTES = L::image, KS = 15, WB = KS * 64, WPB = (WB + 255) / 256;

    int t = __builtin_amdgcn_readfirstlane(fnn_xcd_tile(gridDim.x, blockIdx.x));
    const int tw = __builtin_amdgcn_readfirstlane(t % p.tiles_w); t = __builtin_amdgcn_readfirstlane(t / p.tiles_w);
    const int th = __builtin_amdgcn_readfirstlane(t % p.tiles_h); t = __builtin_amdgcn_readfirstlane(t / p.tiles_h);
    const int seg = __builtin_amdgcn_readfirstlane(t % segs);
    const int n = __builtin_amdgcn_readfirstlane(t / segs);
    const int td0 = seg * tps, td1 = td0 + tps < p.tiles_d ? td0 + tps : p.tiles_d;
    if (td0 >= td1) return;
    const int cb0 = blockIdx.y * NB;
    const int oh0 = th * 8, ow0 = tw * 8;

    char *sA = smem;
    char *sW = smem + ABYTES;
    auto sred_at = [&](int i) { const int k = i >> 4; return (float *)(sA + (k / IH) * PS + ((k % IH) * PW + IW) * 32) + (i & 15); };

    const int col = tid >> 1, cg = tid & 1;
    const int zh = (col * 205) >> 11, zw = col - zh * IW;
    const bool has_col = tid < 2 * IH * IW;
    const int gh = oh0 - 1 + zh, gw = ow0 - 1 + zw;
    const bool ok_hw = has_col & ((unsigned)gh < (unsigned)p.Hi) & ((unsigned)gw < (unsigned)p.Wi);
    const int hw_lin = __mul24(gh, p.Wi) + gw;
    const int ldso0 = (zh * PW + zw) * 32 + ((cg ^ (zh & 1)) * 16);

    const int sC = p.src[0].C, vs = FNN_VS(p.src[0]);
    const unsigned item_bytes = (unsigned)p.Di * p.Hi * p.Wi * sC * 2;
    const __amdgpu_buffer_rsrc_t rx = __builtin_amdgcn_make_buffer_rsrc((void *)(p.src[0].ptr + (size_t)n * (item_bytes >> 1)), 0, item_bytes, 0x00020000);
    const unsigned voff = ok_hw ? (unsigned)hw_lin * (unsigned)(vs * 2) + cg * 16 : 0x80000000u;
    const unsigned plane_bytes = (unsigned)p.Hi * p.Wi * vs * 2;
    const f16 slope_h = (f16)p.src[0].slope;
#ifdef FNN_NORM_FP32
    float sc[8], sh[8];
    {
        const float *qs, *qh;
        fnn_ss_rows(p.src[0].ss, sC, n, 0, p.ident_ss, qs, qh);
#pragma unroll
        for (int j = 0; j < 8; ++j) { sc[j] = ok_hw ? qs[cg * 8 + j] : 0.f; sh[j] = ok_hw ? qh[cg * 8 + j] : 0.f; }
    }
#else
    f16x8 sc, sh;
    {
        const fnn_u32x4v *qv = (const fnn_u32x4v *)(fnn_ssh_rows(p.src[0].ssh, sC, n, 0, p.ident_ssh) + cg * 16);
        const fnn_u32x4v zero4 = {0u, 0u, 0u, 0u};
        sc = __builtin_bit_cast(f16x8, ok_hw ? qv[0] : zero4); sh = __builtin_bit_cast(f16x8, ok_hw ? qv[1] : zero4);
    }
#endif

    fnn_u32x4v xr[ID];
    auto load_planes = [&](int td, int u0) {
#pragma unroll
        for (int u = 0; u < ID; ++u) {
            if (u < u0) continue;
            int gd = td * TD - 1 + u;
            gd = gd < 0 ? 0 : (gd >= p.Di ? p.Di - 1 : gd);
            xr[u] = __builtin_bit_cast(fnn_u32x4v, __builtin_amdgcn_raw_buffer_load_b128(rx, voff, (unsigned)gd * plane_bytes, 0));
        }
    };
    auto stage = [&](int td, int u0) {
        if (!has_col) return;
        const int k0 = (td - td0) * TD;
#pragma unroll
        for (int u = 0; u < ID; ++u) {
            if (u < u0) continue;
            f16x8 o = fnn_norm_leaky8(__builtin_bit_cast(f16x8, xr[u]), sc, sh, slope_h);
            const int gd = td * TD - 1 + u;
            if ((unsigned)gd >= (unsigned)p.Di) o = (f16x8){0, 0, 0, 0, 0, 0, 0, 0};
            *(f16x8 *)(sA + ldso0 + ((k0 + u) % ID) * PS) = o;
        }
    };
    int toff[5];
    f32x4 acc[TD][NB];
    auto kloop = [&](int td) {
        const int k0 = (td - td0) * TD;
        int roff[ID];
#pragma unroll
        for (int pl = 0; pl < ID; ++pl) roff[pl] = ((k0 + pl) % ID) * PS;
        zr_kloop<TD, NB, KS>(acc, sA, toff, sW, lane, [&](int pl) { return roff[pl]; });
    };

    load_planes(td0, 0);
    fnn_u32x4v wr[NB][WPB];
#pragma unroll
    for (int nb = 0; nb < NB; ++nb) {
        const f16 *wp = p.wpk + ((size_t)((cb0 + nb) * p.chunks) * WB) * 8;
        const __amdgpu_buffer_rsrc_t rw = __builtin_amdgcn_make_buffer_rsrc((void *)wp, 0, WB * 16, 0x00020000);
#pragma unroll
        for (int u = 0; u < WPB; ++u) wr[nb][u] = __builtin_bit_cast(fnn_u32x4v, __builtin_amdgcn_raw_buffer_load_b128(rw, tid * 16, u * 4096, 0));
    }
    f32x4 b0[NB];
#pragma unroll
    for (int nb = 0; nb < NB; ++nb)
        b0[nb] = *(const f32x4 *)(p.bias + cb0 * 16 + (NB == 2 ? (lane >> 4) * 8 + nb * 4 : nb * 16 + (lane >> 4) * 4));
    zr_tap_offsets<PW, true>(toff, lane, [=](int r) { return 2 * wave + (r >> 3); }, [](int r) { return r & 7; });
    stage(td0, 0);
#pragma unroll
    for (int nb = 0; nb < NB; ++nb)
#pragma unroll
        for (int u = 0; u < WPB; ++u)
            if (u + 1 < WPB || wave < 3) *(fnn_u32x4v *)(sW + ((nb * WB + u * 256) + tid) * 16) = wr[nb][u];
    __syncthreads();

    auto finish = [&](int td) {
        float4 bv[NB];
#pragma unroll
        for (int nb = 0; nb < NB; ++nb) bv[nb] = make_float4(0.f, 0.f, 0.f, 0.f);
        float t1[NB][4], t2[NB][4];
#pragma unroll
        for (int nb = 0; nb < NB; ++nb)
#pragma unroll
            for (int j = 0; j < 4; ++j) { t1[nb][j] = 0.f; t2[nb][j] = 0.f; }
        if constexpr (NB == 2) zr_epilogue_pair<TD, false>(p, acc, bv, n, td * TD, oh0 + 2 * wave + ((lane & 15) >> 3), ow0 + (lane & 7), cb0, lane, t1, t2);
        else tile_epilogue<NB, TD, true, false>(p, acc, bv, n, td * TD, oh0, ow0, cb0, wave, lane, t1, t2);
        if (p.stats_out) stats_to_global_at<NB, true, NB == 2>(p, t1, t2, sred_at, n, cb0, wave, lane, tid, (td * p.tiles_h + th) * p.tiles_w + tw);
        else __syncthreads();
    };
    for (int td = td0; td + 1 < td1; ++td) {
#pragma unroll
        for (int j = 0; j < TD; ++j)
#pragma unroll
            for (int nb = 0; nb < NB; ++nb) acc[j][nb] = b0[nb];
        load_planes(td + 1, 2);
        kloop(td);
        __syncthreads();
        stage(td + 1, 2);
        finish(td);
    }
#pragma unroll
    for (int j = 0; j < TD; ++j)
#pragma unroll
        for (int nb = 0; nb < NB; ++nb) acc[j][nb] = b0[nb];
    kloop(td1 - 1);
    __syncthreads();
    finish(td1 - 1);
}

template <int TD>
__global__ __launch_bounds__(576, 1) void conv3d_zr12_kernel(const ConvParams p) {
    constexpr int NB = 2, NT = 576;
    extern __shared__ __attribute__((aligned(16))) char smem[];
    const int tid = threadIdx.x, lane = tid & 63, wave = tid >> 6;
    using L = Zr12Lds<TD, 9>;
    constexpr int IH = 14, IW = 14, PW = L::PW, ID = TD + 2;
    constexpr int PS = L::PS, ABYTES = L::image;
    constexpr int KS = 15;
    constexpr int IELEM = ID * IH * IW * 2;
    constexpr int PF = (IELEM + NT - 1) / NT;
    constexpr int WTOT = NB * KS * 64;
    constexpr int WPF = (WTOT + NT - 1) / NT;

    const int td = blockIdx.x % p.tiles_d, n = blockIdx.x / p.tiles_d;
    const int cb0 = blockIdx.y * NB;
    const int od0 = td * TD;
    const int bh = wave / 3, bw = wave - bh * 3;

    char *sA = smem;
    char *sW = smem + ABYTES;
    float *sRed = (float *)(sW + L::weights);

    const int cg = tid & 1;
    int offv[PF], ldso[PF];
#pragma unroll
    for (int u = 0; u < PF; ++u) {
        const int idx = tid + u * NT;
        const int v = idx >> 1;
        const int zd = v / (IH * IW), rem = v - zd * (IH * IW), zh = rem / IW, zw = rem - zh * IW;
        const int gd = od0 - 1 + zd, gh = zh - 1, gw = zw - 1;
        const bool ok = ((unsigned)gd < (unsigned)p.Di) & ((unsigned)gh < (unsigned)p.Hi) & ((unsigned)gw < (unsigned)p.Wi);
        offv[u] = idx < IELEM ? (ok ? __mul24(__mul24(gd, p.Hi) + gh, p.Wi) + gw : -1) : -2;
        ldso[u] = zd * PS + (zh * PW + zw) * 32 + ((cg ^ (zh & 1)) * 16);
    }
    const int wbase = cb0 * p.chunks * (KS * 64), wskip = (p.chunks - 1) * (KS * 64);
    f16x8 xr[PF], wr[WPF];
    float scu[16], shu[16];
    float slope_next = 1.f;
    auto issue = [&](int ch) {
        const int c_glob = ch * 16;
        const int s = (c_glob < p.src[0].C) ? 0 : 1;
        const int c_uni = c_glob - (s ? p.src[0].C : 0);
        const int sC = p.src[s].C;
        const int vs = FNN_VS(p.src[s]);
        const char *sp = (const char *)(p.src[s].ptr + (size_t)n * p.Di * p.Hi * p.Wi * sC + (c_uni >> 4) * FNN_CS(p.src[s]));
        slope_next = p.src[s].slope;
        const float *qs, *qh;
        fnn_ss_rows(p.src[s].ss, sC, n, c_uni, p.ident_ss, qs, qh);
#pragma unroll
        for (int j = 0; j < 16; ++j) { scu[j] = qs[j]; shu[j] = qh[j]; }
#pragma unroll
        for (int u = 0; u < PF; ++u)
            xr[u] = *(const f16x8 *)(sp + (unsigned)(((offv[u] >= 0 ? offv[u] : 0) * vs + cg * 8) * 2));
#pragma unroll
        for (int u = 0; u < WPF; ++u) {
            const int idx = tid + u * NT, idc = idx < WTOT ? idx : WTOT - 1;
            int e = idc + (idc >= KS * 64 ? wskip : 0);
            asm volatile("" : "+v"(e));
            wr[u] = *(const f16x8 *)((const char *)p.wpk + (unsigned)((wbase + e + ch * (KS * 64)) * 16));
        }
    };
    auto commit = [&]() {
        const f16 slope_h = (f16)slope_next;
        float sc[8], sh[8];
#pragma unroll
        for (int j = 0; j < 8; ++j) { sc[j] = cg ? scu[8 + j] : scu[j]; sh[j] = cg ? shu[8 + j] : shu[j]; }
#pragma unroll
        for (int u = 0; u < PF; ++u) {
            if ((u + 1) * NT > IELEM && offv[u] == -2) continue;
            f16x8 o = fnn_norm_leaky8(xr[u], sc, sh, slope_h);
            if (offv[u] < 0) o = (f16x8){0, 0, 0, 0, 0, 0, 0, 0};
            *(f16x8 *)(sA + ldso[u]) = o;
        }
#pragma unroll
        for (int u = 0; u < WPF; ++u) {
            const int idx = tid + u * NT;
            if ((u + 1) * NT <= WTOT || idx < WTOT) ((f16x8 *)sW)[idx] = wr[u];
        }
    };
    int toff[5];
    f32x4 acc[TD][NB];
    auto kloop = [&]() { zr_kloop<TD, NB, KS>(acc, sA, toff, sW, lane, [](int pl) { return pl * PS; }); };

    issue(0);
    __builtin_amdgcn_sched_barrier(0);
    zr_tap_offsets<PW, true>(toff, lane, [=](int r) { return 4 * bh + (r >> 2); }, [=](int r) { return 4 * bw + (r & 3); });
#pragma unroll
    for (int j = 0; j < TD; ++j)
#pragma unroll
        for (int nb = 0; nb < NB; ++nb) acc[j][nb] = (f32x4){0.f, 0.f, 0.f, 0.f};
    commit();
    __syncthreads();
    for (int ch = 0; ch + 1 < p.chunks; ++ch) {
        issue(ch + 1);
        kloop();
        __syncthreads();
        commit();
        __syncthreads();
    }
    kloop();

    {
        const int q = lane >> 4, r = lane & 15;
        float4 bv[NB];
#pragma unroll
        for (int nb = 0; nb < NB; ++nb) bv[nb] = *(const float4 *)(p.bias + cb0 * 16 + q * 8 + nb * 4);
        float t1[NB][4], t2[NB][4];
#pragma unroll
        for (int nb = 0; nb < NB; ++nb)
#pragma unroll
            for (int j = 0; j < 4; ++j) { t1[nb][j] = 0.f; t2[nb][j] = 0.f; }
        zr_epilogue_pair<TD>(p, acc, bv, n, od0, 4 * bh + (r >> 2), 4 * bw + (r & 3), cb0, lane, t1, t2);
        if (p.stats_out) {
#pragma unroll
            for (int nb = 0; nb < NB; ++nb)
#pragma unroll
                for (int j = 0; j < 4; ++j) {
                    const float a = row16_sum(t1[nb][j]), b = row16_sum(t2[nb][j]);
                    if (r == 0) {
                        const int c = q * 8 + nb * 4 + j;
                        sRed[(wave * 32 + c) * 2] = a;
                        sRed[(wave * 32 + c) * 2 + 1] = b;
                    }
                }
            __syncthreads();
            if (tid < 64) {
                const int c = tid >> 1, which = tid & 1;
                double v = 0;
#pragma unroll
                for (int w = 0; w < 9; ++w) v += (double)sRed[(w * 32 + c) * 2 + which];
                p.stats_out[(((size_t)n * p.stats_slots + td) * p.Cout + cb0 * 16 + c) * 2 + which] = v;
            }
        }
    }
}

template <int TD>
static int launch_zr12(ConvParams p, hipStream_t st) {
    p.tile_d = TD;
    p.tiles_d = (p.Do + TD - 1) / TD; p.tiles_h = 1; p.tiles_w = 1;
    p.ident_ss = conv3d_identity_ss();
    if (!p.ident_ss) return -2;
    dim3 grid(p.N * p.tiles_d, (p.Cout / 16) / 2);
    return fnn_launch_lds<conv3d_zr12_kernel<TD>>(grid, dim3(576), Zr12Lds<TD, 9>::bytes(), st, p);
}

template <int NB>
__global__ __launch_bounds__(256, 2) void conv3d_zs_kernel(const ConvParams p) {
    static_assert(NB == 2, "two cout blocks per workgroup");
    extern __shared__ __attribute__((aligned(16))) char smem[];
    const int tid = threadIdx.x, lane = tid & 63, wave = tid >> 6;
    using L = ZsLds<NB, false>;
    constexpr int TD = 8, TH = 4, TDW = 4;
    constexpr int ID = TD + 2, IH = 2 * TH + 1, IW = 17, PW = L::PW;
    constexpr int PS = L::PS, ABYTES = L::image;
    constexpr int KS = 15;
    constexpr int IELEM = ID * IH * IW * 2;
    constexpr int PF = (IELEM + 255) / 256;
    constexpr int WTOT = NB * KS * 64;
    constexpr int WPF = (WTOT + 255) / 256;

    int t = fnn_xcd_tile(gridDim.x, blockIdx.x);
    const int tw = t % p.tiles_w; t /= p.tiles_w;
    const int th = t % p.tiles_h; t /= p.tiles_h;
    const int td = t % p.tiles_d;
    const int n = t / p.tiles_d;
    const int cb0 = blockIdx.y * NB;
    const int od0 = td * TD, oh0 = th * TH, ow0 = tw * 8;
    const int hp = wave & 1, dh = wave >> 1;

    char *sA = smem;
    char *sW = smem + ABYTES;
    float *sBias = (float *)(sW + L::weights);

    int toff[5];
    f32x4 acc[TDW][NB];
    const int cg = tid & 1;
    int offv[PF], ldso[PF];
    {
        const int id0 = od0 - 1, ih0 = 2 * oh0 - 1, iw0 = 2 * ow0 - 1;
#pragma unroll
        for (int u = 0; u < PF; ++u) {
            const int idx = tid + u * 256;
            const int v = idx >> 1;
            const int zd = v / (IH * IW), rem = v - zd * (IH * IW), zh = rem / IW, zw = rem - zh * IW;
            const int gd = id0 + zd, gh = ih0 + zh, gw = iw0 + zw;
            const bool ok = ((unsigned)gd < (unsigned)p.Di) & ((unsigned)gh < (unsigned)p.Hi) & ((unsigned)gw < (unsigned)p.Wi);
            const int lin = __mul24(__mul24(gd, p.Hi) + gh, p.Wi) + gw;
            offv[u] = idx < IELEM ? (ok ? lin : -1) : -2;
            ldso[u] = zd * PS + (zh * PW + zw) * 32 + cg * 16;
        }
    }
    int wofs[WPF];
#pragma unroll
    for (int u = 0; u < WPF; ++u) {
        const int idx = tid + u * 256;
        const int idc = idx < WTOT ? idx : WTOT - 1;
        const int nb = idc >= KS * 64 ? 1 : 0;
        wofs[u] = (cb0 + nb) * p.chunks * (KS * 64) + idc - nb * (KS * 64);
    }
    f16x8 xr[PF], wr[WPF];
    float scu[16], shu[16];
    float slope_next = 1.f;

    auto issue = [&](int ch) {
        const int c_glob = ch * 16;
        const int s = (c_glob < p.src[0].C) ? 0 : 1;
        const int c_uni = c_glob - (s ? p.src[0].C : 0);
        const int sC = p.src[s].C;
        const int vs = FNN_VS(p.src[s]);
        const char *sp = (const char *)(p.src[s].ptr + (size_t)n * p.Di * p.Hi * p.Wi * sC + (c_uni >> 4) * FNN_CS(p.src[s]));
        slope_next = p.src[s].slope;
        const float *qs = p.src[s].ss ? p.src[s].ss + (size_t)(2 * n) * sC + c_uni : p.ident_ss + c_uni;
        const float *qh = p.src[s].ss ? qs + sC : p.ident_ss + 512 + c_uni;
#pragma unroll
        for (int j = 0; j < 16; ++j) { scu[j] = qs[j]; shu[j] = qh[j]; }
#pragma unroll
        for (int u = 0; u < PF; ++u)
            xr[u] = *(const f16x8 *)(sp + (unsigned)(((offv[u] >= 0 ? offv[u] : 0) * vs + cg * 8) * 2));
#pragma unroll
        for (int u = 0; u < WPF; ++u) wr[u] = *(const f16x8 *)((const char *)p.wpk + (unsigned)((wofs[u] + ch * (KS * 64)) * 16));
    };
    auto commit = [&]() {
        const f16 slope_h = (f16)slope_next;
        float sc[8], sh[8];
#pragma unroll
        for (int j = 0; j < 8; ++j) { sc[j] = cg ? scu[8 + j] : scu[j]; sh[j] = cg ? shu[8 + j] : shu[j]; }
#pragma unroll
        for (int u = 0; u < PF; ++u) {
            if ((u + 1) * 256 > IELEM && offv[u] == -2) continue;
            f16x8 o = fnn_norm_leaky8(xr[u], sc, sh, slope_h);
            if (offv[u] < 0) o = (f16x8){0, 0, 0, 0, 0, 0, 0, 0};
            *(f16x8 *)(sA + ldso[u]) = o;
        }
#pragma unroll
        for (int u = 0; u < WPF; ++u) {
            const int idx = tid + u * 256;
            if ((u + 1) * 256 <= WTOT || idx < WTOT) ((f16x8 *)sW)[idx] = wr[u];
        }
    };
    auto kloop = [&]() { zr_kloop<TDW, NB, KS>(acc, sA, toff, sW, lane, [](int pl) { return pl * PS; }); };

    if (tid < NB * 16) sBias[tid] = p.bias[cb0 * 16 + tid];
    issue(0);
    __builtin_amdgcn_sched_barrier(0);
    zr_tap_offsets<PW, false>(toff, lane, [=](int r) { return 2 * (2 * hp + (r >> 3)); }, [](int r) { return 2 * (r & 7); }, (TDW * dh) * PS);
#pragma unroll
    for (int j = 0; j < TDW; ++j)
#pragma unroll
        for (int nb = 0; nb < NB; ++nb) acc[j][nb] = (f32x4){0.f, 0.f, 0.f, 0.f};

    commit();
    __syncthreads();
    for (int ch = 0; ch + 1 < p.chunks; ++ch) {
        issue(ch + 1);
        kloop();
        __syncthreads();
        commit();
        __syncthreads();
    }
    kloop();
    __syncthreads();

    {
        const int q = lane >> 4, r = lane & 15;
        float4 bv[NB];
#pragma unroll
        for (int nb = 0; nb < NB; ++nb) bv[nb] = *(const float4 *)(sBias + q * 8 + nb * 4);
        float t1[NB][4], t2[NB][4];
#pragma unroll
        for (int nb = 0; nb < NB; ++nb)
#pragma unroll
            for (int j = 0; j < 4; ++j) { t1[nb][j] = 0.f; t2[nb][j] = 0.f; }
        zr_epilogue_pair<TDW>(p, acc, bv, n, od0 + TDW * dh, oh0 + 2 * hp + (r >> 3), ow0 + (r & 7), cb0, lane, t1, t2);
        if (p.stats_out) stats_to_global<NB, true, true>(p, t1, t2, (float *)smem, n, cb0, wave, lane, tid, (td * p.tiles_h + th) * p.tiles_w + tw);
    }
}

__global__ __launch_bounds__(256, 2) void conv3d_zsp_kernel(const ConvParams p, const int total_tiles) {
    constexpr int NB = 2;
    extern __shared__ __attribute__((aligned(16))) char smem[];
    const int tid = threadIdx.x, lane = tid & 63, wave = tid >> 6;
    using L = ZsLds<NB, true>;
    constexpr int TD = 8, TH = 4, TDW = 4;
    constexpr int ID = TD + 2, IH = 2 * TH + 1, IW = 17, PW = L::PW;
    constexpr int PS = L::PS, ABYTES = L::image;
    constexpr int KS = 15;
    constexpr int IELEM = ID * IH * IW * 2;
    constexpr int PF = (IELEM + 255) / 256;
    constexpr int WTOT = NB * KS * 64;
    const int hp = wave & 1, dh = wave >> 1;

    char *sA = smem;
    char *sW = smem + ABYTES;
    float *sRed = (float *)(sW + L::weights);

    int t_first, t_stride, t_end;
    {
        const int nwg = gridDim.x, idx = blockIdx.x >> 3;
        int wg_lo, wg_n;
        fnn_xcd_range(nwg, blockIdx.x, wg_lo, wg_n);
        const int r_lo = (int)((long long)total_tiles * wg_lo / nwg), r_hi = (int)((long long)total_tiles * (wg_lo + wg_n) / nwg);
        t_first = r_lo + idx; t_stride = wg_n; t_end = r_hi;
    }
    if (t_first >= t_end) return;
    const int cb0 = blockIdx.y * NB;

    for (int idx = tid; idx < WTOT; idx += 256) {
        const int nb = idx >= KS * 64 ? 1 : 0;
        ((f16x8 *)sW)[idx] = ((const f16x8 *)p.wpk)[(cb0 + nb) * p.chunks * (KS * 64) + idx - nb * (KS * 64)];
    }
    const int cg = tid & 1;
    unsigned relp[PF / 2];
    static_assert(PF % 2 == 0, "pairs");
#pragma unroll
    for (int u = 0; u < PF; ++u) {
        const int idx = tid + u * 256, v = (idx < IELEM ? idx : IELEM - 1) >> 1;
        const int zd = v / (IH * IW), rem = v - zd * (IH * IW), zh = rem / IW, zw = rem - zh * IW;
        const unsigned t = (unsigned)((zd << 9) | (zh << 5) | zw);
        if (u & 1) relp[u >> 1] |= t << 16; else relp[u >> 1] = t;
    }
    const bool has_last = tid + (PF - 1) * 256 < IELEM;
#define ZSP_REL(u) ((relp[(u) >> 1] >> (((u) & 1) * 16)) & 0x1fffu)
    int toff[5];
    zr_tap_offsets<PW, false>(toff, lane, [=](int r) { return 2 * (2 * hp + (r >> 3)); }, [](int r) { return 2 * (r & 7); }, (TDW * dh) * PS);
    const int q = lane >> 4, r = lane & 15;
    float4 bv[NB];
#pragma unroll
    for (int nb = 0; nb < NB; ++nb) bv[nb] = *(const float4 *)(p.bias + cb0 * 16 + q * 8 + nb * 4);

    int offv[PF];
    f16x8 xr[PF];
    float scu[16], shu[16];
    auto tile_coords = [&](int t, int &n, int &od0, int &oh0, int &ow0, int &slot) {
        const int tw = t % p.tiles_w; t /= p.tiles_w;
        const int th = t % p.tiles_h; t /= p.tiles_h;
        const int td = t % p.tiles_d;
        n = t / p.tiles_d;
        od0 = td * TD; oh0 = th * TH; ow0 = tw * 8;
        slot = (td * p.tiles_h + th) * p.tiles_w + tw;
    };
    auto set_offsets = [&](int od0, int oh0, int ow0) {
        const int id0 = od0 - 1, ih0 = 2 * oh0 - 1, iw0 = 2 * ow0 - 1;
#pragma unroll
        for (int u = 0; u < PF; ++u) {
            unsigned t = ZSP_REL(u);
            asm volatile("" : "+v"(t));
            const unsigned gd = (unsigned)(id0 + (int)(t >> 9)), gh = (unsigned)(ih0 + (int)((t >> 5) & 15)), gw = (unsigned)(iw0 + (int)(t & 31));
            const bool ok = gd < (unsigned)p.Di && gh < (unsigned)p.Hi && gw < (unsigned)p.Wi;
            offv[u] = ok ? (int)(__umul24(__umul24(gd, (unsigned)p.Hi) + gh, (unsigned)p.Wi) + gw) : -1;
        }
    };
    auto issue = [&](int n) {
        const int sC = p.src[0].C;
        const int vs = FNN_VS(p.src[0]);
        const char *sp = (const char *)(p.src[0].ptr + (size_t)n * p.Di * p.Hi * p.Wi * sC);
        const float *qs, *qh;
        fnn_ss_rows(p.src[0].ss, sC, n, 0, p.ident_ss, qs, qh);
#pragma unroll
        for (int j = 0; j < 16; ++j) { scu[j] = qs[j]; shu[j] = qh[j]; }
#pragma unroll
        for (int u = 0; u < PF; ++u)
            xr[u] = *(const f16x8 *)(sp + (unsigned)(((offv[u] >= 0 ? offv[u] : 0) * vs + cg * 8) * 2));
    };
    auto commit = [&]() {
        const f16 slope_h = (f16)p.src[0].slope;
        float sc[8], sh[8];
#pragma unroll
        for (int j = 0; j < 8; ++j) { sc[j] = cg ? scu[8 + j] : scu[j]; sh[j] = cg ? shu[8 + j] : shu[j]; }
#pragma unroll
        for (int u = 0; u < PF; ++u) {
            f16x8 o = fnn_norm_leaky8(xr[u], sc, sh, slope_h);
            if (offv[u] < 0) o = (f16x8){0, 0, 0, 0, 0, 0, 0, 0};
            unsigned t = ZSP_REL(u);
            asm volatile("" : "+v"(t));
            const int zd = (int)(t >> 9), zh = (int)((t >> 5) & 15), zw = (int)(t & 31);
            if (u + 1 < PF || has_last) *(f16x8 *)(sA + zd * PS + (zh * PW + zw) * 32 + cg * 16) = o;
        }
    };

    int n_cur, od0, oh0, ow0, slot;
    tile_coords(t_first, n_cur, od0, oh0, ow0, slot);
    set_offsets(od0, oh0, ow0);
    issue(n_cur);
    commit();
    __syncthreads();
    const f16x2 ones = {(f16)1.f, (f16)1.f};
    for (int t = t_first; t < t_end; t += t_stride) {
        int n_nx = n_cur, d_nx = od0, h_nx = oh0, w_nx = ow0, s_nx = slot;
        if (t + t_stride < t_end) tile_coords(t + t_stride, n_nx, d_nx, h_nx, w_nx, s_nx);
        set_offsets(d_nx, h_nx, w_nx);
        issue(n_nx);
        f32x4 acc[TDW][NB];
#pragma unroll
        for (int j = 0; j < TDW; ++j)
#pragma unroll
            for (int nb = 0; nb < NB; ++nb) acc[j][nb] = (f32x4){0.f, 0.f, 0.f, 0.f};
#pragma unroll
        for (int pr = 0; pr < 5; ++pr) {
            const char *bp = sA + toff[pr];
            f16x8 xf[TDW + 2];
#pragma unroll
            for (int pl = 0; pl < TDW + 2; ++pl) xf[pl] = *(const f16x8 *)(bp + pl * PS);
#pragma unroll
            for (int dz = 0; dz < 3; ++dz) {
                f16x8 wf[NB];
#pragma unroll
                for (int nb = 0; nb < NB; ++nb) wf[nb] = *(const f16x8 *)(sW + ((nb * KS + pr * 3 + dz) * 64 + lane) * 16);
#pragma unroll
                for (int j = 0; j < TDW; ++j)
#pragma unroll
                    for (int nb = 0; nb < NB; ++nb)
                        acc[j][nb] = __builtin_amdgcn_mfma_f32_16x16x32_f16(wf[nb], xf[j + dz], acc[j][nb], 0, 0, 0);
            }
            __builtin_amdgcn_sched_barrier(0);
        }
        float t1[NB][4], t2[NB][4];
#pragma unroll
        for (int nb = 0; nb < NB; ++nb)
#pragma unroll
            for (int j = 0; j < 4; ++j) { t1[nb][j] = 0.f; t2[nb][j] = 0.f; }
        {
            const unsigned item_bytes = (unsigned)p.Do * p.Ho * p.Wo * p.Cout * 2;
            const __amdgpu_buffer_rsrc_t rsrc = __builtin_amdgcn_make_buffer_rsrc(p.out + (size_t)n_cur * (item_bytes >> 1), 0, item_bytes, 0x00020000);
            const unsigned ovs2 = (unsigned)FNN_OVS(p) * 2;
            const unsigned coff = (unsigned)(cb0 + (q >> 1)) * (unsigned)(FNN_OCS(p) * 2) + (unsigned)(q & 1) * 16;
            const int oh = oh0 + 2 * hp + (r >> 3), ow = ow0 + (r & 7);
            const bool ok_hw = oh < p.Ho && ow < p.Wo;
#pragma unroll
            for (int mb = 0; mb < TDW; mb += 2) {
                f16x8 o[2];
#pragma unroll
                for (int h = 0; h < 2; ++h) {
                    const int od = od0 + TDW * dh + mb + h;
                    const bool ok = ok_hw && od < p.Do;
                    const unsigned voff = ok ? (unsigned)((od * p.Ho + oh) * p.Wo + ow) * ovs2 + coff : 0x80000000u;
#pragma unroll
                    for (int nb = 0; nb < 2; ++nb) {
                        o[h][nb * 4 + 0] = (f16)(acc[mb + h][nb][0] + bv[nb].x);
                        o[h][nb * 4 + 1] = (f16)(acc[mb + h][nb][1] + bv[nb].y);
                        o[h][nb * 4 + 2] = (f16)(acc[mb + h][nb][2] + bv[nb].z);
                        o[h][nb * 4 + 3] = (f16)(acc[mb + h][nb][3] + bv[nb].w);
                    }
                    __builtin_amdgcn_raw_buffer_store_b128(__builtin_bit_cast(fnn_i32x4, o[h]), rsrc, voff, 0, 0);
                    if (!ok) o[h] = (f16x8){0, 0, 0, 0, 0, 0, 0, 0};
                }
#pragma unroll
                for (int nb = 0; nb < 2; ++nb)
#pragma unroll
                    for (int j = 0; j < 4; ++j) {
                        const f16x2 pr = {o[0][nb * 4 + j], o[1][nb * 4 + j]};
                        t1[nb][j] = __builtin_amdgcn_fdot2(pr, ones, t1[nb][j], false);
                        t2[nb][j] = __builtin_amdgcn_fdot2(pr, pr, t2[nb][j], false);
                    }
            }
        }
        if (p.stats_out) {
#pragma unroll
            for (int nb = 0; nb < NB; ++nb)
#pragma unroll
                for (int j = 0; j < 4; ++j) {
                    const float a = row16_sum(t1[nb][j]), b = row16_sum(t2[nb][j]);
                    if (r == 0) {
                        const int c = q * 8 + nb * 4 + j;
                        sRed[(wave * 32 + c) * 2] = a;
                        sRed[(wave * 32 + c) * 2 + 1] = b;
                    }
                }
        }
        __syncthreads();
        if (p.stats_out && tid < 64) {
            const int c = tid >> 1, which = tid & 1;
            double v = 0;
#pragma unroll
            for (int w = 0; w < 4; ++w) v += (double)sRed[(w * 32 + c) * 2 + which];
            p.stats_out[(((size_t)n_cur * p.stats_slots + slot) * p.Cout + cb0 * 16 + c) * 2 + which] = v;
        }
        commit();
        __syncthreads();
        n_cur = n_nx; od0 = d_nx; oh0 = h_nx; ow0 = w_nx; slot = s_nx;
    }
#undef ZSP_REL
}

__global__ __launch_bounds__(256, 2) void conv3d_zsw_kernel(const ConvParams p, const int segs, const int tps) {
    constexpr int NB = 2;
    extern __shared__ __attribute__((aligned(16))) char smem[];
    const int tid = threadIdx.x, lane = tid & 63, wave = __builtin_amdgcn_readfirstlane(tid >> 6);
    using L = ZsLds<NB, true>;
    constexpr int TD = 8, TH = 4, TDW = 4;
    constexpr int ID = TD + 2, IH = 2 * TH + 1, IW = 17, PW = L::PW;
    constexpr int PS = L::PS, ABYTES = L::image;
    constexpr int KS = 15, WB = KS * 64, WPB = (WB + 255) / 256;
    constexpr int NCOL = IH * IW * 2;
    const int hp = wave & 1, dh = wave >> 1;

    int t = __builtin_amdgcn_readfirstlane(fnn_xcd_tile(gridDim.x, blockIdx.x));
    const int tw = __builtin_amdgcn_readfirstlane(t % p.tiles_w); t = __builtin_amdgcn_readfirstlane(t / p.tiles_w);
    const int th = __builtin_amdgcn_readfirstlane(t % p.tiles_h); t = __builtin_amdgcn_readfirstlane(t / p.tiles_h);
    const int seg = __builtin_amdgcn_readfirstlane(t % segs);
    const int n = __builtin_amdgcn_readfirstlane(t / segs);
    const int td0 = seg * tps, td1 = td0 + tps < p.tiles_d ? td0 + tps : p.tiles_d;
    if (td0 >= td1) return;
    const int cb0 = blockIdx.y * NB;
    const int oh0 = th * TH, ow0 = tw * 8;

    char *sA = smem;
    char *sW = smem + ABYTES;
    float *sRed = (float *)(sW + L::weights);

    const int sC = p.src[0].C, vs = FNN_VS(p.src[0]);
    const unsigned item_bytes = (unsigned)p.Di * p.Hi * p.Wi * sC * 2;
    const __amdgpu_buffer_rsrc_t rx = __builtin_amdgcn_make_buffer_rsrc((void *)(p.src[0].ptr + (size_t)n * (item_bytes >> 1)), 0, item_bytes, 0x00020000);
    const unsigned plane_bytes = (unsigned)p.Hi * p.Wi * vs * 2;
    const int cg = tid & 1;
    unsigned voff[2];
    int ldso[2];
    bool has[2], okc[2];
#pragma unroll
    for (int k = 0; k < 2; ++k) {
        const int e = tid + 256 * k;
        has[k] = e < NCOL;
        const int col = (has[k] ? e : 0) >> 1;
        const int zh = (col * 241) >> 12, zw = col - zh * IW;
        const int gh = 2 * oh0 - 1 + zh, gw = 2 * ow0 - 1 + zw;
        okc[k] = has[k] & ((unsigned)gh < (unsigned)p.Hi) & ((unsigned)gw < (unsigned)p.Wi);
        voff[k] = okc[k] ? (unsigned)(__mul24(gh, p.Wi) + gw) * (unsigned)(vs * 2) + cg * 16 : 0x80000000u;
        ldso[k] = (zh * PW + zw) * 32 + cg * 16;
    }
    const f16 slope_h = (f16)p.src[0].slope;
    float sc[8], sh[8];
    {
        const float *qs, *qh;
        fnn_ss_rows(p.src[0].ss, sC, n, 0, p.ident_ss, qs, qh);
#pragma unroll
        for (int j = 0; j < 8; ++j) { sc[j] = qs[cg * 8 + j]; sh[j] = qh[cg * 8 + j]; }
    }

    fnn_u32x4v xr[2][ID];
    auto load_planes = [&](int td, int u0) {
#pragma unroll
        for (int u = 0; u < ID; ++u) {
            if (u < u0) continue;
            int gd = td * TD - 1 + u;
            gd = gd < 0 ? 0 : (gd >= p.Di ? p.Di - 1 : gd);
#pragma unroll
            for (int k = 0; k < 2; ++k)
                xr[k][u] = __builtin_bit_cast(fnn_u32x4v, __builtin_amdgcn_raw_buffer_load_b128(rx, voff[k], (unsigned)gd * plane_bytes, 0));
        }
    };
    auto stage = [&](int td, int u0) {
        const int k0 = (td - td0) * TD;
#pragma unroll
        for (int u = 0; u < ID; ++u) {
            if (u < u0) continue;
            const int gd = td * TD - 1 + u;
            const bool plane_ok = (unsigned)gd < (unsigned)p.Di;
            char *dst = sA + ((k0 + u) % ID) * PS;
#pragma unroll
            for (int k = 0; k < 2; ++k) {
                f16x8 o = fnn_norm_leaky8(__builtin_bit_cast(f16x8, xr[k][u]), sc, sh, slope_h);
                if (!okc[k] || !plane_ok) o = (f16x8){0, 0, 0, 0, 0, 0, 0, 0};
                if (has[k]) *(f16x8 *)(dst + ldso[k]) = o;
            }
        }
    };
    int toff[5];
    zr_tap_offsets<PW, false>(toff, lane, [=](int r) { return 2 * (2 * hp + (r >> 3)); }, [](int r) { return 2 * (r & 7); });
    const int q = lane >> 4, r = lane & 15;
    float4 bv[NB];
#pragma unroll
    for (int nb = 0; nb < NB; ++nb) bv[nb] = *(const float4 *)(p.bias + cb0 * 16 + q * 8 + nb * 4);
    f32x4 acc[TDW][NB];
    auto kloop = [&](int td) {
        const int k0 = (td - td0) * TD + TDW * dh;
        int roff[TDW + 2];
#pragma unroll
        for (int pl = 0; pl < TDW + 2; ++pl) roff[pl] = ((k0 + pl) % ID) * PS;
#pragma unroll
        for (int j = 0; j < TDW; ++j)
#pragma unroll
            for (int nb = 0; nb < NB; ++nb) acc[j][nb] = (f32x4){0.f, 0.f, 0.f, 0.f};
        zr_kloop<TDW, NB, KS>(acc, sA, toff, sW, lane, [&](int pl) { return roff[pl]; });
    };
    auto finish = [&](int td) {
        const int od0 = td * TD;
        float t1[NB][4], t2[NB][4];
#pragma unroll
        for (int nb = 0; nb < NB; ++nb)
#pragma unroll
            for (int j = 0; j < 4; ++j) { t1[nb][j] = 0.f; t2[nb][j] = 0.f; }
        zr_epilogue_pair<TDW>(p, acc, bv, n, od0 + TDW * dh, oh0 + 2 * hp + (r >> 3), ow0 + (r & 7), cb0, lane, t1, t2);
        if (p.stats_out) {
#pragma unroll
            for (int nb = 0; nb < NB; ++nb)
#pragma unroll
                for (int j = 0; j < 4; ++j) {
                    const float a = row16_sum(t1[nb][j]), b = row16_sum(t2[nb][j]);
                    if (r == 0) {
                        const int c = q * 8 + nb * 4 + j;
                        sRed[(wave * 32 + c) * 2] = a;
                        sRed[(wave * 32 + c) * 2 + 1] = b;
                    }
                }
        }
        __syncthreads();
        if (p.stats_out && tid < 64) {
            const int c = tid >> 1, which = tid & 1;
            double v = 0;
#pragma unroll
            for (int w = 0; w < 4; ++w) v += (double)sRed[(w * 32 + c) * 2 + which];
            p.stats_out[(((size_t)n * p.stats_slots + (td * p.tiles_h + th) * p.tiles_w + tw) * p.Cout + cb0 * 16 + c) * 2 + which] = v;
        }
    };

    load_planes(td0, 0);
    fnn_u32x4v wr[NB][WPB];
#pragma unroll
    for (int nb = 0; nb < NB; ++nb) {
        const f16 *wp = p.wpk + ((size_t)((cb0 + nb) * p.chunks) * WB) * 8;
        const __amdgpu_buffer_rsrc_t rw = __builtin_amdgcn_make_buffer_rsrc((void *)wp, 0, WB * 16, 0x00020000);
#pragma unroll
        for (int u = 0; u < WPB; ++u) wr[nb][u] = __builtin_bit_cast(fnn_u32x4v, __builtin_amdgcn_raw_buffer_load_b128(rw, tid * 16, u * 4096, 0));
    }
    stage(td0, 0);
#pragma unroll
    for (int nb = 0; nb < NB; ++nb)
#pragma unroll
        for (int u = 0; u < WPB; ++u)
            if (u + 1 < WPB || wave < 3) *(fnn_u32x4v *)(sW + ((nb * WB + u * 256) + tid) * 16) = wr[nb][u];
    __syncthreads();

    for (int td = td0; td + 1 < td1; ++td) {
        load_planes(td + 1, 2);
        kloop(td);
        __syncthreads();
        stage(td + 1, 2);
        finish(td);
    }
    kloop(td1 - 1);
    __syncthreads();
    finish(td1 - 1);
}

static int launch_zs(ConvParams p, const ConvChoice &c, hipStream_t st) {
    p.tile_d = 8;
    p.tiles_d = (p.Do + 7) / 8;
    p.tiles_h = (p.Ho + 3) / 4;
    p.tiles_w = (p.Wo + 7) / 8;
    fnn_allow_lds<conv3d_zs_kernel<2>>();
    p.ident_ss = conv3d_identity_ss();
    if (!p.ident_ss) return -2;
    const int total = p.N * p.tiles_d * p.tiles_h * p.tiles_w, groups = (p.Cout / 16) / 2;
    if (c.kernel == CK_ZSW) {
        return fnn_launch_lds<conv3d_zsw_kernel>(dim3(p.N * p.tiles_h * p.tiles_w * c.segs, groups), dim3(256), ZsLds<2, true>::bytes(), st, p, c.segs, c.tps);
    }
    if (c.kernel == CK_ZSP) {
        return fnn_launch_lds<conv3d_zsp_kernel>(dim3(c.gx, groups), dim3(256), ZsLds<2, true>::bytes(), st, p, total);
    }
    return fnn_launch_lds<conv3d_zs_kernel<2>>(dim3(total, groups), dim3(256), ZsLds<2, false>::bytes(), st, p);
}

typedef long fnn_i64;
typedef unsigned fnn_u32x4 __attribute__((ext_vector_type(4)));
template <int NB, int TD>
__global__ __launch_bounds__(256, 2) void conv3d_zr8_kernel(const ConvParams p) {
    extern __shared__ __attribute__((aligned(16))) char smem[];
    const int tid = threadIdx.x, lane = tid & 63, wave = tid >> 6;
    using L = Zr8Lds<NB, TD>;
    constexpr int IH = 10, IW = 10, ID = TD + 2;
    constexpr int SUB = L::SUB, PS = L::PS, ABYTES = L::image;
    constexpr int KS = 15;
    constexpr int IELEM = ID * IH * IW * 2;
    constexpr int PF = (IELEM + 255) / 256;
    constexpr int WTOT = NB * KS * 32;
    constexpr int WPF = (WTOT + 255) / 256;

    int t = fnn_xcd_tile(gridDim.x, blockIdx.x);
    const int tw = t % p.tiles_w; t /= p.tiles_w;
    const int th = t % p.tiles_h; t /= p.tiles_h;
    const int td = t % p.tiles_d;
    const int n = t / p.tiles_d;
    const int cb0 = blockIdx.y * NB;
    const int od0 = td * TD, oh0 = th * 8, ow0 = tw * 8;

    char *sA = smem;
    char *sW = smem + ABYTES;
    float *sBias = (float *)(sW + L::weights);

    int toff[5];
    f32x4 acc[TD][NB];
    const int cg = tid & 1;
    int offv[PF], ldso[PF];
    {
        const int id0 = od0 - 1, ih0 = oh0 - 1, iw0 = ow0 - 1;
#pragma unroll
        for (int u = 0; u < PF; ++u) {
            const int idx = tid + u * 256;
            const int v = idx >> 1;
            const int zd = v / (IH * IW), rem = v - zd * (IH * IW), zh = rem / IW, zw = rem - zh * IW;
            const int gd = id0 + zd, gh = ih0 + zh, gw = iw0 + zw;
            const bool ok = gd >= 0 && gd < p.Di && gh >= 0 && gh < p.Hi && gw >= 0 && gw < p.Wi;
            offv[u] = idx < IELEM ? (ok ? (gd * p.Hi + gh) * p.Wi + gw : -1) : -2;
            ldso[u] = zd * PS + (zh * 2 + cg) * SUB + zw * 8;
        }
    }
    int wofs[WPF];
#pragma unroll
    for (int u = 0; u < WPF; ++u) {
        const int idx = tid + u * 256;
        const int idc = idx < WTOT ? idx : WTOT - 1;
        const int nb = idc >= KS * 32 ? 1 : 0;
        wofs[u] = (cb0 + nb) * p.chunks * (KS * 32) + idc - nb * (KS * 32);
    }
    f16x8 xr[PF];
    fnn_u32x4 wr[WPF];
    float4 scr[2], shr[2];
    float slope_next = 1.f;

    auto issue = [&](int ch) {
        const int c_glob = ch * 16;
        const int s = (c_glob < p.src[0].C) ? 0 : 1;
        const int c_uni = c_glob - (s ? p.src[0].C : 0);
        const int c_loc = c_uni + cg * 8;
        const int sC = p.src[s].C;
        const int vs = FNN_VS(p.src[s]);
        const char *sp = (const char *)(p.src[s].ptr + (size_t)n * p.Di * p.Hi * p.Wi * sC + (c_uni >> 4) * FNN_CS(p.src[s]));
        slope_next = p.src[s].slope;
        const float *qs = p.src[s].ss ? p.src[s].ss + (size_t)(2 * n) * sC + c_loc : p.ident_ss + c_loc;
        const float *qh = p.src[s].ss ? qs + sC : p.ident_ss + 512 + c_loc;
        scr[0] = *(const float4 *)qs; scr[1] = *(const float4 *)(qs + 4);
        shr[0] = *(const float4 *)qh; shr[1] = *(const float4 *)(qh + 4);
        __builtin_amdgcn_sched_barrier(0);
#pragma unroll
        for (int u = 0; u < PF; ++u)
            xr[u] = *(const f16x8 *)(sp + (unsigned)(((offv[u] >= 0 ? offv[u] : 0) * vs + cg * 8) * 2));
#pragma unroll
        for (int u = 0; u < WPF; ++u) wr[u] = *(const fnn_u32x4 *)((const char *)p.wpk + (unsigned)((wofs[u] + ch * (KS * 32)) * 16));
    };
    auto commit = [&]() {
        const float am = p.act_mult, slope = slope_next;
        const float sc[8] = {scr[0].x * am, scr[0].y * am, scr[0].z * am, scr[0].w * am, scr[1].x * am, scr[1].y * am, scr[1].z * am, scr[1].w * am};
        const float sh[8] = {shr[0].x * am, shr[0].y * am, shr[0].z * am, shr[0].w * am, shr[1].x * am, shr[1].y * am, shr[1].z * am, shr[1].w * am};
#pragma unroll
        for (int u = 0; u < PF; ++u) {
            if ((u + 1) * 256 > IELEM && offv[u] == -2) continue;
            auto q = [&](int j) {
                const float v = fmaf((float)xr[u][j], sc[j], sh[j]);
                return __builtin_amdgcn_fmed3f(fmaxf(v, v * slope), -448.f, 448.f);
            };
            int lo = 0, hi = 0;
            lo = __builtin_amdgcn_cvt_pk_fp8_f32(q(0), q(1), lo, false);
            lo = __builtin_amdgcn_cvt_pk_fp8_f32(q(2), q(3), lo, true);
            hi = __builtin_amdgcn_cvt_pk_fp8_f32(q(4), q(5), hi, false);
            hi = __builtin_amdgcn_cvt_pk_fp8_f32(q(6), q(7), hi, true);
            if (offv[u] < 0) { lo = 0; hi = 0; }
            *(int2 *)(sA + ldso[u]) = make_int2(lo, hi);
        }
#pragma unroll
        for (int u = 0; u < WPF; ++u) {
            const int idx = tid + u * 256;
            if ((u + 1) * 256 <= WTOT || idx < WTOT) ((fnn_u32x4 *)sW)[idx] = wr[u];
        }
    };
    auto kloop = [&]() {
#pragma unroll
        for (int pr = 0; pr < 5; ++pr) {
            const char *bp = sA + toff[pr];
            fnn_i64 xf[ID];
#pragma unroll
            for (int pl = 0; pl < ID; ++pl) xf[pl] = *(const fnn_i64 *)(bp + pl * PS);
#pragma unroll
            for (int dz = 0; dz < 3; ++dz) {
                fnn_i64 wf[NB];
#pragma unroll
                for (int nb = 0; nb < NB; ++nb) wf[nb] = *(const fnn_i64 *)(sW + ((nb * KS + pr * 3 + dz) * 64 + lane) * 8);
#pragma unroll
                for (int j = 0; j < TD; ++j)
#pragma unroll
                    for (int nb = 0; nb < NB; ++nb)
                        acc[j][nb] = __builtin_amdgcn_mfma_f32_16x16x32_fp8_fp8(wf[nb], xf[j + dz], acc[j][nb], 0, 0, 0);
            }
            __builtin_amdgcn_sched_barrier(0);
        }
    };

    issue(0);
    __builtin_amdgcn_sched_barrier(0);
    if (tid < NB * 16) { sBias[tid] = p.bias[cb0 * 16 + tid]; sBias[NB * 16 + tid] = p.oscale[cb0 * 16 + tid]; }
    zr_tap_offsets(toff, lane, [=](int r) { return 2 * wave + (r >> 3); }, [](int r) { return r & 7; }, [](int row, int col, int kh) { return (row * 2 + kh) * SUB + col * 8; });
#pragma unroll
    for (int j = 0; j < TD; ++j)
#pragma unroll
        for (int nb = 0; nb < NB; ++nb) acc[j][nb] = (f32x4){0.f, 0.f, 0.f, 0.f};

    commit();
    __syncthreads();
    for (int ch = 0; ch + 1 < p.chunks; ++ch) {
        issue(ch + 1);
        kloop();
        __syncthreads();
        commit();
        __syncthreads();
    }
    kloop();
    __syncthreads();
    {
        float4 bv[NB];
#pragma unroll
        for (int nb = 0; nb < NB; ++nb) {
            const int co = NB == 2 ? (lane >> 4) * 8 + nb * 4 : nb * 16 + (lane >> 4) * 4;
            bv[nb] = *(const float4 *)(sBias + co);
            const float4 sv = *(const float4 *)(sBias + NB * 16 + co);
#pragma unroll
            for (int j = 0; j < TD; ++j) {
                acc[j][nb][0] *= sv.x; acc[j][nb][1] *= sv.y; acc[j][nb][2] *= sv.z; acc[j][nb][3] *= sv.w;
            }
        }
        float t1[NB][4], t2[NB][4];
#pragma unroll
        for (int nb = 0; nb < NB; ++nb)
#pragma unroll
            for (int j = 0; j < 4; ++j) { t1[nb][j] = 0.f; t2[nb][j] = 0.f; }
        if constexpr (NB == 2) zr_epilogue_pair<TD>(p, acc, bv, n, od0, oh0 + 2 * wave + ((lane & 15) >> 3), ow0 + (lane & 7), cb0, lane, t1, t2);
        else tile_epilogue<NB, TD, true>(p, acc, bv, n, od0, oh0, ow0, cb0, wave, lane, t1, t2);
        if (p.stats_out) stats_to_global<NB, true, NB == 2>(p, t1, t2, (float *)smem, n, cb0, wave, lane, tid, (td * p.tiles_h + th) * p.tiles_w + tw);
    }
}

template <int NB, int TD>
static int launch_zr8(ConvParams p, hipStream_t st) {
    p.tile_d = TD;
    p.tiles_d = (p.Do + TD - 1) / TD;
    p.tiles_h = (p.Ho + 7) / 8;
    p.tiles_w = (p.Wo + 7) / 8;
    p.ident_ss = conv3d_identity_ss();
    if (!p.ident_ss || !p.oscale) return -2;
    dim3 grid(p.N * p.tiles_d * p.tiles_h * p.tiles_w, (p.Cout / 16) / NB);
    return fnn_launch_lds<conv3d_zr8_kernel<NB, TD>>(grid, dim3(256), Zr8Lds<NB, TD>::bytes(), st, p);
}

template <int NB, int TD, int TH = 8>
static int launch_zr(ConvParams p, hipStream_t st) {
    p.tile_d = TD;
    p.tiles_d = (p.Do + TD - 1) / TD;
    p.tiles_h = (p.Ho + 7) / 8;
    p.tiles_w = (p.Wo + 7) / 8;
    size_t lds = ZrLds<NB, TD, TH>::bytes();
    if (const char *pad = fnn_knob("FNN_ZR_LDS_PAD")) lds += (size_t)atoi(pad);
    p.ident_ss = conv3d_identity_ss();
    p.ident_ssh = conv3d_identity_ssh();
    if (!p.ident_ss || !p.ident_ssh) return -2;
    dim3 grid(p.N * p.tiles_d * p.tiles_h * p.tiles_w, (p.Cout / 16) / NB);
#ifdef FNN_TMODE
    p.tmode = getenv("FNN_ZR_TMODE") ? atoi(getenv("FNN_ZR_TMODE")) : 0;
#endif
    return fnn_launch_lds<conv3d_zr_kernel<NB, TD, TH>>(grid, dim3(TH * 32), lds, st, p);
}

template <int NB>
static int launch_zrw(ConvParams p, const ConvChoice &c, hipStream_t st) {
    constexpr int TD = 8;
    p.tile_d = TD;
    p.tiles_d = (p.Do + TD - 1) / TD;
    p.tiles_h = (p.Ho + 7) / 8;
    p.tiles_w = (p.Wo + 7) / 8;
    p.ident_ss = conv3d_identity_ss();
    p.ident_ssh = conv3d_identity_ssh();
    if (!p.ident_ss || !p.ident_ssh) return -2;
    dim3 grid(p.N * p.tiles_h * p.tiles_w * c.segs, (p.Cout / 16) / NB);
    return fnn_launch_lds<conv3d_zrw_kernel<NB>>(grid, dim3(256), ZrLds<NB, TD>::bytes(), st, p, c.segs, c.tps);
}

int launch_conv3d_zr(ConvParams p, const ConvChoice &c, hipStream_t st) {
    const int nb = c.t[0], td = c.t[1];
    switch (c.kernel) {
        case CK_ZS: case CK_ZSP: case CK_ZSW: return launch_zs(p, c, st);
        case CK_ZR8:
            if (nb == 2) return td == 8 ? launch_zr8<2, 8>(p, st) : launch_zr8<2, 4>(p, st);
            return td == 8 ? launch_zr8<1, 8>(p, st) : launch_zr8<1, 4>(p, st);
        case CK_ZQ12: return launch_conv3d_zq12(p, st);
        case CK_ZR12: return launch_zr12<4>(p, st);
        case CK_ZRW: return nb == 2 ? launch_zrw<2>(p, c, st) : launch_zrw<1>(p, c, st);
        case CK_ZR:
            if (c.t[2] == 6) return launch_zr<2, 10, 6>(p, st);
            if (nb == 2) return td == 8 ? launch_zr<2, 8>(p, st) : launch_zr<2, 4>(p, st);
            return td == 8 ? launch_zr<1, 8>(p, st) : launch_zr<1, 4>(p, st);
    }
    return -1;
}
```

fast-nnunet_amd/csrc/conv_pack.hip:

```cpp
#include "fnn_device.h"
#include <algorithm>
#include <cmath>
#include <vector>

int conv3d_ksteps(int packing, int taps) {
    return packing == FNN_PACK_ZR || packing == FNN_PACK_ZRP ? 15 : packing == FNN_PACK_ZP ? 9 : (taps + 1) / 2;
}

int conv3d_kstep_tap(int packing, int ks, int half, int taps, int ch, int chunks, int *tch) {
    *tch = ch;
    if (packing == FNN_PACK_ZR || packing == FNN_PACK_ZRP) {
        const int pr = ks / 3, dz = ks % 3;
        if (pr < 4) return dz * 9 + 2 * pr + half;
        if (packing == FNN_PACK_ZR || (ch % 2 == 0 && ch + 1 == chunks)) return half ? -1 : dz * 9 + 8;
        if (ch % 2 == 0) return -1;
        *tch = ch - 1 + half;
        return dz * 9 + 8;
    }
    const int t = 2 * ks + half;
    return t < taps ? t : -1;
}

int conv3d_pack_cout(int packing, int nblk, int cb, int m) {
    if ((packing != FNN_PACK_ZR && packing != FNN_PACK_ZRP && packing != FNN_PACK_ZP) || nblk % 2 != 0) return cb * 16 + m;
    return (cb >> 1) * 32 + (m >> 2) * 8 + (cb & 1) * 4 + (m & 3);
}

size_t conv_packed_halves(const ConvChoice &c, int cout_pad) { return (size_t)(cout_pad / 16) * c.chunks * c.ksteps * 512; }

uint8_t f2e4m3(float f) {
    const uint8_t sign = std::signbit(f) ? 0x80 : 0;
    float a = std::fabs(f);
    if (!(a == a)) return sign | 0x7f;
    if (a >= 448.f) return sign | 0x7e;
    if (a < 0x1p-6f) {
        const int q = (int)std::nearbyint(a * 512.f);
        return sign | (uint8_t)q;
    }
    int e;
    const float m = std::frexp(a, &e);
    int q = (int)std::nearbyint(m * 16.f);
    int E = e - 1;
    if (q == 16) { q = 8; ++E; }
    if (E > 8 || (E == 8 && q > 14)) return sign | 0x7e;
    return sign | (uint8_t)(((E + 7) << 3) | (q - 8));
}

void conv_pack_weights(const ConvParams &p, const ConvChoice &c, int cout_real, const int cin_real[2], const float *W, void *dst,
                       float *scales) {
    const int cin_real1 = p.n_src > 1 ? cin_real[1] : 0, cin_pad0 = p.src[0].C;
    if (c.packing == FNN_PACK_ZP) {
        conv_zp_pack(W, cout_real, p.Cout, cin_real[0], cin_pad0, cin_real1, p.n_src > 1 ? p.src[1].C : 0, (unsigned short *)dst);
        return;
    }
    const int T = p.kd * p.kh * p.kw, cin_tot = cin_real[0] + cin_real1, nblk = p.Cout / 16;
    std::vector<float> inv(p.Cout, 1.f);
    if (p.fp8)
        for (int co = 0; co < p.Cout; ++co) {
            float mx = 0.f;
            if (co < cout_real)
                for (size_t i = 0; i < (size_t)cin_tot * T; ++i) mx = std::max(mx, std::fabs(W[(size_t)co * cin_tot * T + i]));
            float ws = mx / 448.f, iv = 1.f / ws;
            if (!(mx > 0.f) || !std::isfinite(iv)) { ws = 1.f; iv = 0.f; }
            inv[co] = iv;
            scales[co] = ws / FNN_FP8_ACT_MULT;
        }
    for (int cb = 0; cb < nblk; ++cb)
        for (int ch = 0; ch < c.chunks; ++ch)
            for (int ks = 0; ks < c.ksteps; ++ks)
                for (int lane = 0; lane < 64; ++lane)
                    for (int j = 0; j < 8; ++j) {
                        const int k = 8 * (lane >> 4) + j;
                        int tch;
                        const int tap = conv3d_kstep_tap(c.packing, ks, k >> 4, T, ch, c.chunks, &tch), ci = tch * 16 + (k & 15);
                        const int co = conv3d_pack_cout(c.packing, nblk, cb, lane & 15);
                        const int src = ci >= cin_pad0, cl = src ? ci - cin_pad0 : ci;
                        float v = 0.f;
                        if (tap >= 0 && co < cout_real && cl < (src ? cin_real1 : cin_real[0]))
                            v = W[((size_t)co * cin_tot + (src ? cin_real[0] : 0) + cl) * T + tap] * inv[co];
                        const size_t i = ((((size_t)cb * c.chunks + ch) * c.ksteps + ks) * 64 + lane) * 8 + j;
                        if (p.fp8) ((uint8_t *)dst)[i] = f2e4m3(v);
                        else ((unsigned short *)dst)[i] = fnn_half_bits(v);
                    }
}
```

fast-nnunet_amd/csrc/conv_zr_common.h:

```cpp
#pragma once
#include "conv_common.h"

template <int NB, int TD, int TH = 8>
struct ZrLds {
    static constexpr int PW = 12, PS = (TH + 2) * PW * 32;
    static constexpr int image = (TD + 2) * PS;
    static constexpr int weights = NB * 15 * 1024;
    static constexpr int bytes() { return image + weights; }
};
template <int TD, int NW>
struct Zr12Lds {
    static constexpr int PW = 20, PS = 14 * PW * 32;
    static constexpr int image = (TD + 2) * PS;
    static constexpr int weights = 2 * 15 * 1024;
    static constexpr int tail = NW * 32 * 2 * 4;
    static constexpr int bytes() { return image + weights + tail; }
};
template <int NB, bool RED>
struct ZsLds {
    static constexpr int PW = 17, PS = 9 * PW * 32;
    static constexpr int image = (10 * PS + 1023) & ~1023;
    static constexpr int weights = NB * 15 * 1024;
    static constexpr int tail = RED ? 4 * NB * 16 * 2 * 4 : NB * 16 * 4;
    static constexpr int bytes() { return image + weights + tail; }
};
template <int NB, int TD>
struct Zr8Lds {
    static constexpr int SUB = 192, PS = 10 * 2 * SUB;
    static constexpr int image = ((TD + 2) * PS + 1023) & ~1023;
    static constexpr int weights = NB * 15 * 512;
    static constexpr int tail = NB * 128;
    static constexpr int bytes() { return image + weights + tail; }
};

template <class Row, class Col, class At>
static __device__ __forceinline__ void zr_tap_offsets(int (&toff)[5], int lane, Row row_of_r, Col col_of_r, At at) {
    const int r = lane & 15, hl = lane >> 5, kh = (lane >> 4) & 1;
#pragma unroll
    for (int pr = 0; pr < 5; ++pr) {
        const int tp = 2 * pr + hl < 9 ? 2 * pr + hl : 8;
        const int row = row_of_r(r) + tp / 3, col = col_of_r(r) + tp % 3;
        toff[pr] = at(row, col, kh);
    }
}
template <int PW, bool SWAP, class Row, class Col>
static __device__ __forceinline__ void zr_tap_offsets(int (&toff)[5], int lane, Row row_of_r, Col col_of_r, int base = 0) {
    zr_tap_offsets(toff, lane, row_of_r, col_of_r,
                   [base](int row, int col, int kh) { return base + (row * PW + col) * 32 + ((SWAP ? kh ^ (row & 1) : kh) * 16); });
}

template <int TDW, int NB, int KS>
static __device__ __forceinline__ void zr_pair_mfma(f32x4 (&acc)[TDW][NB], const f16x8 (&xf)[TDW + 2], const char *sW, int pr, int lane) {
#pragma unroll
    for (int dz = 0; dz < 3; ++dz) {
        f16x8 wf[NB];
#pragma unroll
        for (int nb = 0; nb < NB; ++nb) wf[nb] = *(const f16x8 *)(sW + ((nb * KS + pr * 3 + dz) * 64 + lane) * 16);
#pragma unroll
        for (int j = 0; j < TDW; ++j)
#pragma unroll
            for (int nb = 0; nb < NB; ++nb)
                acc[j][nb] = __builtin_amdgcn_mfma_f32_16x16x32_f16(wf[nb], xf[j + dz], acc[j][nb], 0, 0, 0);
    }
    __builtin_amdgcn_sched_barrier(0);
}
template <int TDW, int NB, int KS, class PlaneOff>
static __device__ __forceinline__ void zr_kloop(f32x4 (&acc)[TDW][NB], const char *sA, const int (&toff)[5], const char *sW, int lane,
                                                PlaneOff plane_off) {
#pragma unroll
    for (int pr = 0; pr < 5; ++pr) {
        const char *bp = sA + toff[pr];
        f16x8 xf[TDW + 2];
#pragma unroll
        for (int pl = 0; pl < TDW + 2; ++pl) xf[pl] = *(const f16x8 *)(bp + plane_off(pl));
        zr_pair_mfma<TDW, NB, KS>(acc, xf, sW, pr, lane);
    }
}

typedef int fnn_i32x4 __attribute__((ext_vector_type(4)));
template <int TDW, bool BIAS = true>
static __device__ __forceinline__ void zr_epilogue_pair(const ConvParams &p, const f32x4 (&acc)[TDW][2], const float4 (&bv)[2],
                                                        int n, int od0, int oh, int ow, int cb0, int lane,
                                                        float (&t1)[2][4], float (&t2)[2][4]) {
    const int q = lane >> 4;
    const unsigned item_bytes = (unsigned)p.Do * p.Ho * p.Wo * p.Cout * 2;
    const __amdgpu_buffer_rsrc_t rsrc = __builtin_amdgcn_make_buffer_rsrc(p.out + (size_t)n * (item_bytes >> 1), 0,
                                                                           item_bytes, 0x00020000);
    const unsigned ovs2 = (unsigned)FNN_OVS(p) * 2;
    const unsigned coff = (unsigned)(cb0 + (q >> 1)) * (unsigned)(FNN_OCS(p) * 2) + (unsigned)(q & 1) * 16;
    const bool ok_hw = oh < p.Ho && ow < p.Wo;
    const f16x2 ones = {(f16)1.f, (f16)1.f};
#pragma unroll
    for (int mb = 0; mb < TDW; mb += 2) {
        f16x8 o[2];
#pragma unroll
        for (int h = 0; h < 2; ++h) {
            const int od = od0 + mb + h;
            const bool ok = ok_hw && od < p.Do;
            unsigned voff = ok ? (unsigned)((od * p.Ho + oh) * p.Wo + ow) * ovs2 + coff : 0x80000000u;
#ifdef FNN_TMODE
            if (p.tmode & 4) voff = 0x80000000u;
#endif
#pragma unroll
            for (int nb = 0; nb < 2; ++nb) {
                o[h][nb * 4 + 0] = (f16)(BIAS ? acc[mb + h][nb][0] + bv[nb].x : acc[mb + h][nb][0]);
                o[h][nb * 4 + 1] = (f16)(BIAS ? acc[mb + h][nb][1] + bv[nb].y : acc[mb + h][nb][1]);
                o[h][nb * 4 + 2] = (f16)(BIAS ? acc[mb + h][nb][2] + bv[nb].z : acc[mb + h][nb][2]);
                o[h][nb * 4 + 3] = (f16)(BIAS ? acc[mb + h][nb][3] + bv[nb].w : acc[mb + h][nb][3]);
            }
            __builtin_amdgcn_raw_buffer_store_b128(__builtin_bit_cast(fnn_i32x4, o[h]), rsrc, voff, 0, 0);
            if (!ok) o[h] = (f16x8){0, 0, 0, 0, 0, 0, 0, 0};
        }
#pragma unroll
        for (int nb = 0; nb < 2; ++nb)
#pragma unroll
            for (int j = 0; j < 4; ++j) {
                const f16x2 pr = {o[0][nb * 4 + j], o[1][nb * 4 + j]};
                t1[nb][j] = __builtin_amdgcn_fdot2(pr, ones, t1[nb][j], false);
                t2[nb][j] = __builtin_amdgcn_fdot2(pr, pr, t2[nb][j], false);
            }
    }
}
```

fast-nnunet_amd/csrc/fnn_device.h:

```cpp
#pragma once
#include <hip/hip_runtime.h>
#include <stdint.h>
#include "../../include/fnn.h"

typedef _Float16 f16;
typedef f16 f16x8 __attribute__((ext_vector_type(8)));
typedef f16 f16x4 __attribute__((ext_vector_type(4)));
typedef f16 f16x2 __attribute__((ext_vector_type(2)));
typedef float f32x4 __attribute__((ext_vector_type(4)));
typedef float f32x16 __attribute__((ext_vector_type(16)));

#define FNN_STAT_REPL 8
#define FNN_TILE_D 4
#define FNN_TILE_H 8
#define FNN_TILE_W 8

struct SrcDesc {
    const f16 *ptr;
    int C;
    const float *ss;
    float slope;
    int vs;
    long long cs;
    const unsigned short *ssh;
};
#define FNN_VS(S) ((S).vs ? (S).vs : (S).C)
#define FNN_CS(S) ((S).vs ? (S).cs : 16LL)
#define FNN_OVS(P) ((P).out_vs ? (P).out_vs : (P).Cout)
#define FNN_OCS(P) ((P).out_vs ? (P).out_cs : 16LL)

struct ConvParams {
    SrcDesc src[2];
    int n_src;
    int N, Di, Hi, Wi;
    int plan_N;
    int Do, Ho, Wo;
    int Cout;
    int kd, kh, kw, sd, sh, sw, pd, ph, pw;
    const f16 *wpk;
    const float *bias;
    f16 *out;
    int out_vs;
    long long out_cs;
    double *stats_out;
    int tiles_d, tiles_h, tiles_w;
    int tile_d;
    unsigned long long *dbg;
    int tmode;
    int chunks;
    int ksteps;
    const float *ident_ss;
    const unsigned short *ident_ssh;
    int packing;
    int fp8;
    const float *oscale;
    float act_mult;
    int stats_slots;
};

#define FNN_PACK_LINEAR 0
#define FNN_PACK_ZR 1
#define FNN_PACK_ZP 2
#define FNN_PACK_ZRP 3
int conv_zp_chunks(int cin_pad0, int cin_pad1);
void conv_zp_pack(const float *W, int cout_real, int cout_pad, int cin_real0, int cin_pad0, int cin_real1, int cin_pad1, unsigned short *dst);

struct StemParams {
    const float *vol;
    long long vol_batch_stride;
    int C;
    long long X, Y, Z;
    const int *origins;
    int flip_d, flip_h, flip_w;
    int PD, PH, PW;
    int kd, kh, kw;
    int Cout;
    const float *w;
    const float *bias;
    f16 *out;
    double *stats_out;
    int tiles_d, tiles_h, tiles_w;
};

#define FUSE_STEM 1
#define FUSE_TCONV 2
struct ThinParams {
    ConvParams c;
    int fuse;
    const f16 *fw;
    const float *fbias;
    const float *vol;
    long long vol_batch_stride;
    long long Y, Z;
    const int *origins;
    int flip_d, flip_h, flip_w;
    const float *fss;
    float fslope;
    SrcDesc low;
    int Dl, Hl, Wl;
    int tsd, tsh, tsw;
};

struct TconvParams {
    SrcDesc src;
    int N, Di, Hi, Wi;
    int sd, sh, sw;
    int Cout;
    const f16 *wpk;
    const float *bias;
    f16 *out;
    int out_vs;
    long long out_cs;
    int ksteps;
    int nblk;
    int row_store;
    int lds_w;
};

struct HeadParams {
    SrcDesc src;
    int b;
    int PD, PH, PW;
    int heads;
    int hblocks;
    int ksteps;
    const f16 *wpk;
    const float *bias;
    const f16 *gauss;
    void *acc;
    long long AX, Y, Z;
    int HP;
    int ox, oy, oz;
    int flip_d, flip_h, flip_w;
    int mode;
    float *patch_buf;
    int acc_fp32;
    int fx, fy, fz;
};

struct PatchAccParams {
    const float *patch_buf;
    int n_div;
    int PD, PH, PW, heads;
    const f16 *gauss;
    void *acc;
    long long AX, Y, Z;
    int HP;
    int ox, oy, oz;
    int acc_fp32;
};

struct GatherParams {
    const f16 *feat;
    const float *fss;
    const unsigned short *fssh;
    int n_eval;
    int flipmask[8];
    int n_slots, ring;
    int x_lo, x_hi;
    int y_lo, y_hi, z_lo, z_hi;
    const int *slot_tab;
    int C;
    float slope;
    const int *steps;
    int nx, ny, nz;
    const int *base_x, *base_y, *base_z;
    int windowed;
    int PD, PH, PW;
    const f16 *wpk;
    const float *bias;
    int heads, hblocks;
    int n_pass;
    const f16 *pass_wpk;
    const float *pass_bias;
    const f16 *gauss;
    int lo_x, lo_y, lo_z;
    long long OX, OY, OZ;
    int acc_mode, out_fp32, out_vec;
    int mode;
    void *out;
    void *labels;
    int label_u16;
    const int *order;
    int *inf_flag;
    int ieee_div;
};

bool gather_tile_windows(const long long *const steps[3], const int n[3], const int extent[3], const long long padded[3],
                         int *tab, int off[3], size_t *count);
struct FinalizeParams {
    const void *acc;
    long long AX, Y, Z;
    int HP;
    int lo_x, lo_y, lo_z;
    long long OX, OY, OZ;
    long long out_X, out_Y, out_Z;
    long long out_x, out_y, out_z;
    int heads;
    int acc_fp32;
    int out_fp32;
    int mode;
    void *out;
    int *inf_flag;
};

#ifdef FNN_STAMPS
#define FNN_STAMP_DECL unsigned long long _st[12]; int _si = 0;
#define FNN_STAMP() do { if (_si < 12) { __builtin_amdgcn_sched_barrier(0); _st[_si++] = __builtin_amdgcn_s_memtime(); __builtin_amdgcn_s_waitcnt(0xC07F); __builtin_amdgcn_sched_barrier(0); } } while (0)
#define FNN_STAMP_FLUSH(dbg) do { if ((dbg) && threadIdx.x == 0) { for (int _i = 0; _i < 12; ++_i) (dbg)[(size_t)blockIdx.x * 12 + _i] = _i < _si ? _st[_i] : 0ull; } } while (0)
#else
#define FNN_STAMP_DECL
#define FNN_STAMP() do {} while (0)
#define FNN_STAMP_FLUSH(dbg) do {} while (0)
#endif

const char *fnn_knob(const char *name);
void fnn_note_kernel(const char *fmt, ...) __attribute__((format(printf, 1, 2)));
void fnn_klog_target(void *vector_of_strings);
void fnn_op_klog_begin();
void fnn_op_klog_end();
struct FnnOpKlog {
    FnnOpKlog() { fnn_op_klog_begin(); }
    ~FnnOpKlog() { fnn_op_klog_end(); }
};
void fnn_set_global_error(const char *msg);
int fnn_fail(int code, const char *msg);
bool fnn_dev_ptr(const void *p);

static __device__ __forceinline__ float leaky(float x, float slope) { return x > 0.f ? x : x * slope; }

struct CropBox {
    long long lo[3], e[3];
    long long o[3];
    int tb[3];
};
inline int crop_box_fill(CropBox &b, const int64_t bbox[6], const int64_t before[3], const int32_t *transpose_backward,
                         const char *outside = "bbox outside shape_before_cropping") {
    for (int a = 0; a < 3; ++a) {
        b.lo[a] = bbox[2 * a]; b.e[a] = bbox[2 * a + 1] - bbox[2 * a];
        if (b.lo[a] < 0 || b.e[a] < 1 || bbox[2 * a + 1] > before[a]) return fnn_fail(FNN_E_INVALID, outside);
    }
    for (int j = 0; transpose_backward && j < 3; ++j) { b.tb[j] = transpose_backward[j]; b.o[j] = before[b.tb[j]]; }
    return FNN_OK;
}
static __device__ __forceinline__ bool crop_box_coords(const CropBox &b, long long i, long long (&d)[3]) {
    const long long oc[3] = {i / (b.o[1] * b.o[2]), (i / b.o[2]) % b.o[1], i % b.o[2]};
    long long t[3];
    t[b.tb[0]] = oc[0]; t[b.tb[1]] = oc[1]; t[b.tb[2]] = oc[2];
    d[0] = t[0] - b.lo[0]; d[1] = t[1] - b.lo[1]; d[2] = t[2] - b.lo[2];
    return d[0] >= 0 && d[0] < b.e[0] && d[1] >= 0 && d[1] < b.e[1] && d[2] >= 0 && d[2] < b.e[2];
}
static __device__ __forceinline__ bool crop_box_voxel(const CropBox &b, long long i, size_t &v) {
    long long d[3];
    if (!crop_box_coords(b, i, d)) return false;
    v = ((size_t)d[0] * b.e[1] + d[1]) * b.e[2] + d[2];
    return true;
}

typedef int fnn_u32x4r __attribute__((ext_vector_type(4)));
static __device__ __forceinline__ fnn_u32x4r pair_to_b128(const f16x4 &a, const f16x4 &b) {
    typedef unsigned u32x2 __attribute__((ext_vector_type(2)));
    const u32x2 ua = __builtin_bit_cast(u32x2, a), ub = __builtin_bit_cast(u32x2, b);
    const auto lo = __builtin_amdgcn_permlane16_swap(ua[0], ub[0], false, false);
    const auto hi = __builtin_amdgcn_permlane16_swap(ua[1], ub[1], false, false);
    return (fnn_u32x4r){(int)lo[0], (int)hi[0], (int)lo[1], (int)hi[1]};
}

static __device__ __forceinline__ f16x8 fnn_norm8(const f16x8 &x, const float (&sc)[8], const float (&sh)[8]) {
#ifdef FNN_NORM_FP32
    f16x8 o;
#pragma unroll
    for (int j = 0; j < 8; ++j) o[j] = (f16)fmaf((float)x[j], sc[j], sh[j]);
    return o;
#else
    f16x8 sc_h, sh_h;
#pragma unroll
    for (int j = 0; j < 8; ++j) { sc_h[j] = (f16)sc[j]; sh_h[j] = (f16)sh[j]; }
    return x * sc_h + sh_h;
#endif
}

struct PatchInputParams {
    const float *vol;
    long long vol_batch_stride;
    int C, Cpad;
    long long X, Y, Z;
    const int *origins;
    int flip_d, flip_h, flip_w;
    int PD, PH, PW, N;
    f16 *out;
    int out_vs;
    long long out_cs;
};
int launch_patch_input(const PatchInputParams &p, hipStream_t st);

struct PoolParams {
    SrcDesc src;
    int N, Di, Hi, Wi;
    int sd, sh, sw;
    f16 *out;
    int out_vs;
    long long out_cs;
};

struct CombineParams {
    SrcDesc a;
    SrcDesc b;
    long long vox;
    int N;
    float slope;
    f16 *out;
    int out_vs;
    long long out_cs;
    f16 *pool_out;
    int D, H, W, psd, psh, psw;
    int pool_vs;
    long long pool_cs;
};

struct StatsFinalizeParams {
    const double *stats;
    int nrep;
    const float *gamma, *beta;
    float *ss;
    unsigned short *ssh;
    int C;
    float inv_count, eps;
};

template <auto K> void fnn_allow_lds() {
    static bool attr_set = false;
    if (!attr_set) {
        (void)hipFuncSetAttribute((const void *)K, hipFuncAttributeMaxDynamicSharedMemorySize, 160 * 1024);
        attr_set = true;
    }
}
template <auto K, class... A> int fnn_launch_lds(dim3 grid, dim3 block, size_t lds, hipStream_t st, const A &...args) {
    fnn_allow_lds<K>();
    hipLaunchKernelGGL(K, grid, block, lds, st, args...);
    return hipGetLastError() == hipSuccess ? 0 : -2;
}

int launch_stats_finalize(const StatsFinalizeParams &p, int N, hipStream_t st);
int launch_region_copy(void *feat, long long n_slots, const int *regions, int n, void *message, int PD, int PH, int PW, int C, bool pack, hipStream_t st);
int launch_fss_to_ssh(const float *fss, unsigned short *ssh, long long items, int C, hipStream_t st);
int launch_avgpool(const PoolParams &p, hipStream_t st);
int launch_combine(const CombineParams &p, hipStream_t st);
bool combine_pool_ok(int D, int H, int W, int sd, int sh, int sw);
size_t conv3d_lds_bytes(const ConvParams &p, int nb);
int conv3d_pick_nb(int nblk);
const float *conv3d_identity_ss();
const unsigned short *conv3d_identity_ssh();
int conv3d_ksteps(int packing, int taps);
int conv3d_kstep_tap(int packing, int ks, int half, int taps, int ch, int chunks, int *tch);
int conv3d_pack_cout(int packing, int nblk, int cb, int m);

enum ConvKernel {
    CK_NONE, CK_ZS, CK_ZSP, CK_ZSW, CK_ZR, CK_ZR8, CK_ZQ12, CK_ZR12, CK_ZRW,
    CK_ZP, CK_ZPS,
    CK_ROW, CK_ROW_STEM, CK_THIN,
    CK_PERSIST, CK_LDSK, CK_S2, CK_NB
};
struct ConvChoice {
    int kernel = CK_NONE;
    int t[7] = {};
    int packing = 0, ksteps = 0, chunks = 0, stats_slots = FNN_STAT_REPL;
    int wpc = 0;
    int gx = 0;
    int segs = 0, tps = 0;
    char name[64] = "";
};
struct ConvOverrides {
    bool conv_v1 = false;
    bool no_row = false, no_stem_row = false, no_zr6 = false, no_zrp = false, no_zq12 = false, no_zsw = false, no_zp = false;
    bool zp_no_half = false, zps_no_half = false;
    int zr_min_wgs = 480;
    int fp8_levels = -1;
    static ConvOverrides from_env();
};
bool conv_choose(const ThinParams &tp, const ConvOverrides &o, ConvChoice &c);
bool conv_choose_fp8(ThinParams &tp, const ConvOverrides &o, ConvChoice &c);
int launch_conv(const ThinParams &tp, const ConvChoice &c, hipStream_t st);
#define FNN_FP8_ACT_MULT 8.0f
void conv_pack_weights(const ConvParams &p, const ConvChoice &c, int cout_real, const int cin_real[2], const float *W, void *dst,
                       float *scales);
size_t conv_packed_halves(const ConvChoice &c, int cout_pad);
inline size_t fnn_weight_alloc_bytes(size_t halves) { return halves * 2 + 1024; }
uint8_t f2e4m3(float f);
inline unsigned short fnn_half_bits(float f) { return __builtin_bit_cast(unsigned short, (f16)f); }
void pack_head(int heads, int cin, int hblocks, int ksteps, const float *W, unsigned short *dst);
void pack_head_bias(int heads, int hblocks, const float *bias, float *dst);
void tconv_pack_weights(const float *W, int cin, int cout, int cout_pad, int taps, int ksteps, unsigned short *dst);
bool zp_choose(const ConvParams &p, const ConvOverrides &o, ConvChoice &c);
int launch_conv2d_zp(ConvParams p, const ConvChoice &c, hipStream_t st);
bool zr_choose(const ConvParams &p, const ConvOverrides &o, ConvChoice &c);
int launch_conv3d_zr(ConvParams p, const ConvChoice &c, hipStream_t st);
bool conv3d_zq12_fits(const ConvParams &p, int stats_slots);
int launch_conv3d_zq12(ConvParams p, hipStream_t st);
bool row_choose(const ThinParams &tp, const ConvOverrides &o, ConvChoice &c);
int launch_conv_row(const ThinParams &tp, const ConvChoice &c, hipStream_t st);
bool thin_choose(const ThinParams &tp, ConvChoice &c);
int launch_conv_thin(const ThinParams &tp, const ConvChoice &c, hipStream_t st);
bool s2_choose(const ConvParams &p, ConvChoice &c);
int launch_conv3d_s2(ConvParams p, const ConvChoice &c, hipStream_t st);
int launch_tconv(const TconvParams &p, hipStream_t st);
bool stem_mfma_ok(int C, int kd, int kh, int kw, int cout_pad);
int stem_mfma_stats_slots(int PD, int PH, int PW);
int stem_mfma_ksteps(int C, int taps);
bool stem_mfma_kmap(int C, int taps, int ks, int k, int *c, int *tap);
void stem_mfma_pack(const float *W, int C, int taps, int cout_real, int cout_pad, unsigned short *dst);
int launch_stem_mfma(const StemParams &p, const f16 *wfrag, int N, hipStream_t st);
bool gather_ok(const GatherParams &p);
int launch_gather(const GatherParams &p, hipStream_t st);
int launch_quotient_check(unsigned long long *counts, hipStream_t st);
bool stem_row_ok(const StemParams &p);
int launch_stem_row(const StemParams &p, int N, hipStream_t st);
int launch_head(const HeadParams &p, hipStream_t st);
bool launch_head_first_visit_ok(const HeadParams &p);
int launch_patch_acc(const PatchAccParams &p, hipStream_t st);
int launch_finalize(const FinalizeParams &p, hipStream_t st);
int launch_labels_from_acc(const FinalizeParams &p, void *labels, int label_u16, const int *order, hipStream_t st);
int launch_scale_output(void *out, int out_fp32, long long n, int divisor, int *inf_flag, hipStream_t st);
int launch_argmax(const void *logits, int fp32, int heads, long long nvox, void *labels, int label_u16, const int *order,
                  hipStream_t st);
int launch_pad_volume(const float *src, float *dst, int C, const long long s[3], const long long d[3],
                      const long long lo[3], hipStream_t st);
```

Before: 3602 patches/s.

## Pair depth taps of the ninth spatial tap to drop the padded K-step

Adds a depth-paired weight packing (ZRD) for 3x3x3 convs in which the ninth (h,w) tap's three depth offsets are packed into two K-steps that span adjacent planes. This replaces the zero-padded fifteenth K-step, so each output needs 14 MFMA K-steps instead of 15, with fewer weight bytes in LDS. The change templates all ZR/ZQ/ZS kernels on KS and changes tap offsets and the weight packer. It becomes the default for non-fp8 layers unless ZRP packing is chosen, and it adds extra kernel instantiations and more complex indexing that could hurt scheduling.

```diff
diff --git a/fast-nnunet_amd/csrc/conv3d.hip b/fast-nnunet_amd/csrc/conv3d.hip
--- a/fast-nnunet_amd/csrc/conv3d.hip
+++ b/fast-nnunet_amd/csrc/conv3d.hip
@@ -909,6 +909,7 @@
     o.no_stem_row = fnn_knob("FNN_NO_STEM_ROW") != nullptr;
     o.no_zr6 = fnn_knob("FNN_NO_ZR6") != nullptr;
     o.no_zrp = fnn_knob("FNN_NO_ZRP") != nullptr;
+    o.no_zrd = fnn_knob("FNN_NO_ZRD") != nullptr;
     o.no_zq12 = fnn_knob("FNN_NO_ZQ12") != nullptr;
     o.no_zsw = fnn_knob("FNN_NO_ZSW") != nullptr;
     o.no_zp = fnn_knob("FNN_NO_ZP") != nullptr;
diff --git a/fast-nnunet_amd/csrc/conv3d_zq.hip b/fast-nnunet_amd/csrc/conv3d_zq.hip
--- a/fast-nnunet_amd/csrc/conv3d_zq.hip
+++ b/fast-nnunet_amd/csrc/conv3d_zq.hip
@@ -7,14 +7,16 @@
 typedef unsigned zq_u32x4 __attribute__((ext_vector_type(4)));
 
 constexpr int ZQ_TD = 8, ZQ_ID = ZQ_TD + 2, ZQ_IH = 14, ZQ_IW = 14;
-using Zq12Lds = Zr12Lds<ZQ_TD, 8>;
-constexpr int ZQ_PW = Zq12Lds::PW, ZQ_PS = Zq12Lds::PS;
-constexpr int ZQ_ABYTES = Zq12Lds::image;
-constexpr int ZQ_KS = 15, ZQ_WB = ZQ_KS * 64;
+template <int KS>
+using Zq12Lds = Zr12Lds<ZQ_TD, 8, KS>;
+constexpr int ZQ_PW = Zq12Lds<15>::PW, ZQ_PS = Zq12Lds<15>::PS;
+constexpr int ZQ_ABYTES = Zq12Lds<15>::image;
 constexpr int ZQ_NT = 512, ZQ_NB = 2;
-constexpr int ZQ_WBYTES = Zq12Lds::weights;
-
+
+template <int ZQ_KS>
 __global__ __launch_bounds__(512, 2) void conv3d_zq12_kernel(const ConvParams p) {
+    constexpr int ZQ_WB = ZQ_KS * 64;
+    constexpr int ZQ_WBYTES = Zq12Lds<ZQ_KS>::weights;
     extern __shared__ __attribute__((aligned(16))) char smem[];
     const int tid = threadIdx.x, lane = tid & 63, wave = __builtin_amdgcn_readfirstlane(tid >> 6);
     const int dq = wave >> 1, grp = (wave ^ (wave >> 2)) & 1;
@@ -110,7 +112,7 @@
     };
 
     int toff[5];
-    zr_tap_offsets<ZQ_PW, true>(toff, lane, [](int r) { return r >> 2; }, [](int r) { return r & 3; }, dq * 2 * ZQ_PS);
+    zr_tap_offsets<ZQ_PW, true>(toff, lane, [](int r) { return r >> 2; }, [](int r) { return r & 3; }, dq * 2 * ZQ_PS, ZQ_KS == 14 ? ZQ_PS : 0);
     int boff[5];
 #pragma unroll
     for (int i = 0; i < 5; ++i) {
@@ -121,17 +123,21 @@
     auto read_x = [&](f16x8 (&xf)[4], int pr, int i) {
         const char *bp = sA + toff[pr] + boff[i];
 #pragma unroll
-        for (int pl = 0; pl < 4; ++pl) xf[pl] = *(const f16x8 *)(bp + pl * ZQ_PS);
+        for (int pl = 0; pl < 4; ++pl)
+            if (!(ZQ_KS == 14 && pr == 4 && pl == 3)) xf[pl] = *(const f16x8 *)(bp + pl * ZQ_PS);
     };
     auto kloop = [&](bool prefetch) {
 #pragma unroll
         for (int pr = 0; pr < 5; ++pr) {
             if (prefetch) load_part(pr);
+            constexpr bool DP = ZQ_KS == 14;
+            const int ndz = DP && pr == 4 ? 2 : 3;
             f16x8 wf[3][ZQ_NB];
 #pragma unroll
             for (int dz = 0; dz < 3; ++dz)
 #pragma unroll
-                for (int nb = 0; nb < ZQ_NB; ++nb) wf[dz][nb] = *(const f16x8 *)(sW + ((nb * ZQ_KS + pr * 3 + dz) * 64 + lane) * 16);
+                for (int nb = 0; nb < ZQ_NB; ++nb)
+                    if (dz < ndz) wf[dz][nb] = *(const f16x8 *)(sW + ((nb * ZQ_KS + pr * 3 + dz) * 64 + lane) * 16);
             f16x8 xa[4], xb[4];
             read_x(xa, pr, 0);
 #pragma unroll
@@ -147,7 +153,7 @@
                         for (int j = 0; j < 2; ++j)
 #pragma unroll
                             for (int nb = 0; nb < ZQ_NB; ++nb)
-                                acc[i][j][nb] = __builtin_amdgcn_mfma_f32_16x16x32_f16(wf[dz][nb], cur[j + dz], acc[i][j][nb], 0, 0, 0);
+                                if (dz < ndz) acc[i][j][nb] = __builtin_amdgcn_mfma_f32_16x16x32_f16(wf[dz][nb], cur[j + dz], acc[i][j][nb], 0, 0, 0);
                 }
                 __builtin_amdgcn_sched_barrier(0);
             }
@@ -230,5 +236,6 @@
     p.ident_ssh = conv3d_identity_ssh();
     if (!p.ident_ss || !p.ident_ssh) return -2;
     dim3 grid(p.N * p.tiles_d, (p.Cout / 16) / ZQ_NB);
-    return fnn_launch_lds<conv3d_zq12_kernel>(grid, dim3(ZQ_NT), Zq12Lds::bytes(), st, p);
-}
+    if (p.packing == FNN_PACK_ZRD) return fnn_launch_lds<conv3d_zq12_kernel<14>>(grid, dim3(ZQ_NT), Zq12Lds<14>::bytes(), st, p);
+    return fnn_launch_lds<conv3d_zq12_kernel<15>>(grid, dim3(ZQ_NT), Zq12Lds<15>::bytes(), st, p);
+}
diff --git a/fast-nnunet_amd/csrc/conv3d_zr.hip b/fast-nnunet_amd/csrc/conv3d_zr.hip
--- a/fast-nnunet_amd/csrc/conv3d_zr.hip
+++ b/fast-nnunet_amd/csrc/conv3d_zr.hip
@@ -8,7 +8,8 @@
     if (p.kd != 3 || p.kh != 3 || p.kw != 3 || p.sd != 1) return false;
     const int nblk = p.Cout / 16;
     const int plan_n = p.plan_N > 0 ? p.plan_N : p.N;
-    c.packing = FNN_PACK_ZR; c.ksteps = 15; c.chunks = p.chunks;
+    const bool zrd = !p.fp8 && !o.no_zrd;
+    c.packing = zrd ? FNN_PACK_ZRD : FNN_PACK_ZR; c.ksteps = conv3d_ksteps(c.packing, 27); c.chunks = p.chunks;
     bool zr6_shape = false;
     if (p.sh == 2 && p.sw == 2) {
         if (p.fp8 || nblk % 2 != 0 || (long long)p.Di * p.Hi * p.Wi >= (1 << 23) || p.Do < 8) return false;
@@ -73,27 +74,27 @@
         snprintf(c.name, sizeof c.name, "conv3d_zrw_kernel<%d>", nb);
     } else {
         c.kernel = CK_ZR;
-        if (p.chunks >= 2 && !zr6_shape && !o.no_zrp) c.packing = FNN_PACK_ZRP;
+        if (p.chunks >= 2 && !zr6_shape && !o.no_zrp) { c.packing = FNN_PACK_ZRP; c.ksteps = 15; }
         snprintf(c.name, sizeof c.name, "conv3d_zr_kernel<%d,%d>", nb, td);
     }
     return true;
 }
 
 typedef unsigned fnn_u32x4v __attribute__((ext_vector_type(4)));
-template <int NB, int TD, int TH = 8>
+template <int NB, int TD, int TH = 8, int KS = 15>
 __global__ __launch_bounds__(TH * 32, 2) void conv3d_zr_kernel(const ConvParams p) {
     extern __shared__ __attribute__((aligned(16))) char smem[];
     const int tid = threadIdx.x, lane = tid & 63, wave = __builtin_amdgcn_readfirstlane(tid >> 6);
     FNN_STAMP_DECL
     FNN_STAMP();
     constexpr int NT = TH * 32;
-    using L = ZrLds<NB, TD, TH>;
+    using L = ZrLds<NB, TD, TH, KS>;
     constexpr int IH = TH + 2, IW = 10, PW = L::PW, ID = TD + 2;
     constexpr int PS = L::PS, ABYTES = L::image;
-    constexpr int KS = 15;
     constexpr int WB = KS * 64;
     constexpr int WPB = (WB + NT - 1) / NT;
-    static_assert(WB - (WPB - 1) * NT == 192, "the last weight element group covers exactly waves 0 .. 2");
+    constexpr int WLAST = (WB - (WPB - 1) * NT) / 64;
+    static_assert(WB - (WPB - 1) * NT == WLAST * 64, "the last weight element group covers whole waves");
 
     int t = __builtin_amdgcn_readfirstlane(fnn_xcd_tile(gridDim.x, blockIdx.x));
     const int tw = __builtin_amdgcn_readfirstlane(t % p.tiles_w); t = __builtin_amdgcn_readfirstlane(t / p.tiles_w);
@@ -124,7 +125,7 @@
 
     f32x4 acc[TD][NB];
     fnn_u32x4v xr[ID], wr[NB][WPB];
-    constexpr bool PAIR = TH == 8;
+    constexpr bool PAIR = TH == 8 && KS == 15;
     const bool paired = PAIR && p.packing == FNN_PACK_ZRP;
     f16x8 xl[PAIR ? ID : 1];
 #ifdef FNN_NORM_FP32
@@ -226,7 +227,7 @@
         for (int nb = 0; nb < NB; ++nb)
 #pragma unroll
             for (int u = 0; u < WPB; ++u)
-                if (u + 1 < WPB || wave < 3) *(fnn_u32x4v *)(smem + wlds + (nb * WB + u * NT) * 16) = wr[nb][u];
+                if (u + 1 < WPB || wave < WLAST) *(fnn_u32x4v *)(smem + wlds + (nb * WB + u * NT) * 16) = wr[nb][u];
     };
     int toff[5];
     const bool khalf1 = lane >= 32;
@@ -237,6 +238,12 @@
             const int pr = MODE == 2 ? (i + 4) % 5 : i;
             if (prefetch && i < SL) load_part(i);
             const char *bp = sA + toff[pr];
+            if constexpr (KS == 14) {
+                if (pr == 4) {
+                    zr_dpair_mfma<TD, NB>(acc, bp, sW, lane, [](int pl) { return pl * PS; });
+                    break;
+                }
+            }
             if (MODE == 1 && pr == 4) {
 #pragma unroll
                 for (int pl = 0; pl < ID; ++pl) xl[pl] = *(const f16x8 *)(bp + pl * PS);
@@ -273,7 +280,7 @@
         for (int pr = 0; pr < 5; ++pr) {
             const int tp = 2 * pr + hl < 9 ? 2 * pr + hl : 8;
             const int row = 2 * wave + (r >> 3) + tp / 3, col2 = (r & 7) + tp % 3;
-            toff[pr] = (row * PW + col2) * 32 + ((kh ^ (row & 1)) * 16);
+            toff[pr] = (row * PW + col2) * 32 + ((kh ^ (row & 1)) * 16) + (KS == 14 && pr == 4 && hl ? PS : 0);
         }
     }
 
@@ -332,13 +339,13 @@
 }
 
 
-template <int NB>
+template <int NB, int KS = 15>
 __global__ __launch_bounds__(256, NB == 1 ? 3 : 2) void conv3d_zrw_kernel(const ConvParams p, const int segs, const int tps) {
     extern __shared__ __attribute__((aligned(16))) char smem[];
     const int tid = threadIdx.x, lane = tid & 63, wave = __builtin_amdgcn_readfirstlane(tid >> 6);
-    using L = ZrLds<NB, 8>;
+    using L = ZrLds<NB, 8, 8, KS>;
     constexpr int TD = 8, IH = 10, IW = 10, PW = L::PW, ID = TD + 2;
-    constexpr int PS = L::PS, ABYTES = L::image, KS = 15, WB = KS * 64, WPB = (WB + 255) / 256;
+    constexpr int PS = L::PS, ABYTES = L::image, WB = KS * 64, WPB = (WB + 255) / 256, WLAST = (WB - (WPB - 1) * 256) / 64;
 
     int t = __builtin_amdgcn_readfirstlane(fnn_xcd_tile(gridDim.x, blockIdx.x));
     const int tw = __builtin_amdgcn_readfirstlane(t % p.tiles_w); t = __builtin_amdgcn_readfirstlane(t / p.tiles_w);
@@ -414,7 +421,7 @@
         int roff[ID];
 #pragma unroll
         for (int pl = 0; pl < ID; ++pl) roff[pl] = ((k0 + pl) % ID) * PS;
-        zr_kloop<TD, NB, KS>(acc, sA, toff, sW, lane, [&](int pl) { return roff[pl]; });
+        zr_kloop<TD, NB, KS>(acc, sA, toff, sW, lane, [&](int pl) { return roff[pl]; }, [&](int pl) { return lane >= 32 ? roff[pl + 1] : roff[pl]; });
     };
 
     load_planes(td0, 0);
@@ -436,7 +443,7 @@
     for (int nb = 0; nb < NB; ++nb)
 #pragma unroll
         for (int u = 0; u < WPB; ++u)
-            if (u + 1 < WPB || wave < 3) *(fnn_u32x4v *)(sW + ((nb * WB + u * 256) + tid) * 16) = wr[nb][u];
+            if (u + 1 < WPB || wave < WLAST) *(fnn_u32x4v *)(sW + ((nb * WB + u * 256) + tid) * 16) = wr[nb][u];
     __syncthreads();
 
     auto finish = [&](int td) {
@@ -473,15 +480,14 @@
     finish(td1 - 1);
 }
 
-template <int TD>
+template <int TD, int KS = 15>
 __global__ __launch_bounds__(576, 1) void conv3d_zr12_kernel(const ConvParams p) {
     constexpr int NB = 2, NT = 576;
     extern __shared__ __attribute__((aligned(16))) char smem[];
     const int tid = threadIdx.x, lane = tid & 63, wave = tid >> 6;
-    using L = Zr12Lds<TD, 9>;
+    using L = Zr12Lds<TD, 9, KS>;
     constexpr int IH = 14, IW = 14, PW = L::PW, ID = TD + 2;
     constexpr int PS = L::PS, ABYTES = L::image;
-    constexpr int KS = 15;
     constexpr int IELEM = ID * IH * IW * 2;
     constexpr int PF = (IELEM + NT - 1) / NT;
     constexpr int WTOT = NB * KS * 64;
@@ -559,7 +565,7 @@
 
     issue(0);
     __builtin_amdgcn_sched_barrier(0);
-    zr_tap_offsets<PW, true>(toff, lane, [=](int r) { return 4 * bh + (r >> 2); }, [=](int r) { return 4 * bw + (r & 3); });
+    zr_tap_offsets<PW, true>(toff, lane, [=](int r) { return 4 * bh + (r >> 2); }, [=](int r) { return 4 * bw + (r & 3); }, 0, KS == 14 ? PS : 0);
 #pragma unroll
     for (int j = 0; j < TD; ++j)
 #pragma unroll
@@ -610,26 +616,25 @@
     }
 }
 
-template <int TD>
+template <int TD, int KS = 15>
 static int launch_zr12(ConvParams p, hipStream_t st) {
     p.tile_d = TD;
     p.tiles_d = (p.Do + TD - 1) / TD; p.tiles_h = 1; p.tiles_w = 1;
     p.ident_ss = conv3d_identity_ss();
     if (!p.ident_ss) return -2;
     dim3 grid(p.N * p.tiles_d, (p.Cout / 16) / 2);
-    return fnn_launch_lds<conv3d_zr12_kernel<TD>>(grid, dim3(576), Zr12Lds<TD, 9>::bytes(), st, p);
+    return fnn_launch_lds<conv3d_zr12_kernel<TD, KS>>(grid, dim3(576), Zr12Lds<TD, 9, KS>::bytes(), st, p);
 }
 
-template <int NB>
+template <int NB, int KS = 15>
 __global__ __launch_bounds__(256, 2) void conv3d_zs_kernel(const ConvParams p) {
     static_assert(NB == 2, "two cout blocks per workgroup");
     extern __shared__ __attribute__((aligned(16))) char smem[];
     const int tid = threadIdx.x, lane = tid & 63, wave = tid >> 6;
-    using L = ZsLds<NB, false>;
+    using L = ZsLds<NB, false, KS>;
     constexpr int TD = 8, TH = 4, TDW = 4;
     constexpr int ID = TD + 2, IH = 2 * TH + 1, IW = 17, PW = L::PW;
     constexpr int PS = L::PS, ABYTES = L::image;
-    constexpr int KS = 15;
     constexpr int IELEM = ID * IH * IW * 2;
     constexpr int PF = (IELEM + 255) / 256;
     constexpr int WTOT = NB * KS * 64;
@@ -719,7 +724,7 @@
     if (tid < NB * 16) sBias[tid] = p.bias[cb0 * 16 + tid];
     issue(0);
     __builtin_amdgcn_sched_barrier(0);
-    zr_tap_offsets<PW, false>(toff, lane, [=](int r) { return 2 * (2 * hp + (r >> 3)); }, [](int r) { return 2 * (r & 7); }, (TDW * dh) * PS);
+    zr_tap_offsets<PW, false>(toff, lane, [=](int r) { return 2 * (2 * hp + (r >> 3)); }, [](int r) { return 2 * (r & 7); }, (TDW * dh) * PS, KS == 14 ? PS : 0);
 #pragma unroll
     for (int j = 0; j < TDW; ++j)
 #pragma unroll
@@ -752,15 +757,15 @@
     }
 }
 
+template <int KS = 15>
 __global__ __launch_bounds__(256, 2) void conv3d_zsp_kernel(const ConvParams p, const int total_tiles) {
     constexpr int NB = 2;
     extern __shared__ __attribute__((aligned(16))) char smem[];
     const int tid = threadIdx.x, lane = tid & 63, wave = tid >> 6;
-    using L = ZsLds<NB, true>;
+    using L = ZsLds<NB, true, KS>;
     constexpr int TD = 8, TH = 4, TDW = 4;
     constexpr int ID = TD + 2, IH = 2 * TH + 1, IW = 17, PW = L::PW;
     constexpr int PS = L::PS, ABYTES = L::image;
-    constexpr int KS = 15;
     constexpr int IELEM = ID * IH * IW * 2;
     constexpr int PF = (IELEM + 255) / 256;
     constexpr int WTOT = NB * KS * 64;
@@ -798,7 +803,7 @@
     const bool has_last = tid + (PF - 1) * 256 < IELEM;
 #define ZSP_REL(u) ((relp[(u) >> 1] >> (((u) & 1) * 16)) & 0x1fffu)
     int toff[5];
-    zr_tap_offsets<PW, false>(toff, lane, [=](int r) { return 2 * (2 * hp + (r >> 3)); }, [](int r) { return 2 * (r & 7); }, (TDW * dh) * PS);
+    zr_tap_offsets<PW, false>(toff, lane, [=](int r) { return 2 * (2 * hp + (r >> 3)); }, [](int r) { return 2 * (r & 7); }, (TDW * dh) * PS, KS == 14 ? PS : 0);
     const int q = lane >> 4, r = lane & 15;
     float4 bv[NB];
 #pragma unroll
@@ -874,6 +879,12 @@
 #pragma unroll
         for (int pr = 0; pr < 5; ++pr) {
             const char *bp = sA + toff[pr];
+            if constexpr (KS == 14) {
+                if (pr == 4) {
+                    zr_dpair_mfma<TDW, NB>(acc, bp, sW, lane, [](int pl) { return pl * PS; });
+                    break;
+                }
+            }
             f16x8 xf[TDW + 2];
 #pragma unroll
             for (int pl = 0; pl < TDW + 2; ++pl) xf[pl] = *(const f16x8 *)(bp + pl * PS);
@@ -958,15 +969,16 @@
 #undef ZSP_REL
 }
 
+template <int KS = 15>
 __global__ __launch_bounds__(256, 2) void conv3d_zsw_kernel(const ConvParams p, const int segs, const int tps) {
     constexpr int NB = 2;
     extern __shared__ __attribute__((aligned(16))) char smem[];
     const int tid = threadIdx.x, lane = tid & 63, wave = __builtin_amdgcn_readfirstlane(tid >> 6);
-    using L = ZsLds<NB, true>;
+    using L = ZsLds<NB, true, KS>;
     constexpr int TD = 8, TH = 4, TDW = 4;
     constexpr int ID = TD + 2, IH = 2 * TH + 1, IW = 17, PW = L::PW;
     constexpr int PS = L::PS, ABYTES = L::image;
-    constexpr int KS = 15, WB = KS * 64, WPB = (WB + 255) / 256;
+    constexpr int WB = KS * 64, WPB = (WB + 255) / 256, WLAST = (WB - (WPB - 1) * 256) / 64;
     constexpr int NCOL = IH * IW * 2;
     const int hp = wave & 1, dh = wave >> 1;
 
@@ -1056,7 +1068,7 @@
         for (int j = 0; j < TDW; ++j)
 #pragma unroll
             for (int nb = 0; nb < NB; ++nb) acc[j][nb] = (f32x4){0.f, 0.f, 0.f, 0.f};
-        zr_kloop<TDW, NB, KS>(acc, sA, toff, sW, lane, [&](int pl) { return roff[pl]; });
+        zr_kloop<TDW, NB, KS>(acc, sA, toff, sW, lane, [&](int pl) { return roff[pl]; }, [&](int pl) { return lane >= 32 ? roff[pl + 1] : roff[pl]; });
     };
     auto finish = [&](int td) {
         const int od0 = td * TD;
@@ -1103,7 +1115,7 @@
     for (int nb = 0; nb < NB; ++nb)
 #pragma unroll
         for (int u = 0; u < WPB; ++u)
-            if (u + 1 < WPB || wave < 3) *(fnn_u32x4v *)(sW + ((nb * WB + u * 256) + tid) * 16) = wr[nb][u];
+            if (u + 1 < WPB || wave < WLAST) *(fnn_u32x4v *)(sW + ((nb * WB + u * 256) + tid) * 16) = wr[nb][u];
     __syncthreads();
 
     for (int td = td0; td + 1 < td1; ++td) {
@@ -1118,22 +1130,23 @@
     finish(td1 - 1);
 }
 
+template <int KS>
 static int launch_zs(ConvParams p, const ConvChoice &c, hipStream_t st) {
     p.tile_d = 8;
     p.tiles_d = (p.Do + 7) / 8;
     p.tiles_h = (p.Ho + 3) / 4;
     p.tiles_w = (p.Wo + 7) / 8;
-    fnn_allow_lds<conv3d_zs_kernel<2>>();
+    fnn_allow_lds<conv3d_zs_kernel<2, KS>>();
     p.ident_ss = conv3d_identity_ss();
     if (!p.ident_ss) return -2;
     const int total = p.N * p.tiles_d * p.tiles_h * p.tiles_w, groups = (p.Cout / 16) / 2;
     if (c.kernel == CK_ZSW) {
-        return fnn_launch_lds<conv3d_zsw_kernel>(dim3(p.N * p.tiles_h * p.tiles_w * c.segs, groups), dim3(256), ZsLds<2, true>::bytes(), st, p, c.segs, c.tps);
+        return fnn_launch_lds<conv3d_zsw_kernel<KS>>(dim3(p.N * p.tiles_h * p.tiles_w * c.segs, groups), dim3(256), ZsLds<2, true, KS>::bytes(), st, p, c.segs, c.tps);
     }
     if (c.kernel == CK_ZSP) {
-        return fnn_launch_lds<conv3d_zsp_kernel>(dim3(c.gx, groups), dim3(256), ZsLds<2, true>::bytes(), st, p, total);
-    }
-    return fnn_launch_lds<conv3d_zs_kernel<2>>(dim3(total, groups), dim3(256), ZsLds<2, false>::bytes(), st, p);
+        return fnn_launch_lds<conv3d_zsp_kernel<KS>>(dim3(c.gx, groups), dim3(256), ZsLds<2, true, KS>::bytes(), st, p, total);
+    }
+    return fnn_launch_lds<conv3d_zs_kernel<2, KS>>(dim3(total, groups), dim3(256), ZsLds<2, false, KS>::bytes(), st, p);
 }
 
 typedef long fnn_i64;
@@ -1315,13 +1328,13 @@
     return fnn_launch_lds<conv3d_zr8_kernel<NB, TD>>(grid, dim3(256), Zr8Lds<NB, TD>::bytes(), st, p);
 }
 
-template <int NB, int TD, int TH = 8>
+template <int NB, int TD, int TH = 8, int KS = 15>
 static int launch_zr(ConvParams p, hipStream_t st) {
     p.tile_d = TD;
     p.tiles_d = (p.Do + TD - 1) / TD;
     p.tiles_h = (p.Ho + 7) / 8;
     p.tiles_w = (p.Wo + 7) / 8;
-    size_t lds = ZrLds<NB, TD, TH>::bytes();
+    size_t lds = ZrLds<NB, TD, TH, KS>::bytes();
     if (const char *pad = fnn_knob("FNN_ZR_LDS_PAD")) lds += (size_t)atoi(pad);
     p.ident_ss = conv3d_identity_ss();
     p.ident_ssh = conv3d_identity_ssh();
@@ -1330,10 +1343,10 @@
 #ifdef FNN_TMODE
     p.tmode = getenv("FNN_ZR_TMODE") ? atoi(getenv("FNN_ZR_TMODE")) : 0;
 #endif
-    return fnn_launch_lds<conv3d_zr_kernel<NB, TD, TH>>(grid, dim3(TH * 32), lds, st, p);
+    return fnn_launch_lds<conv3d_zr_kernel<NB, TD, TH, KS>>(grid, dim3(TH * 32), lds, st, p);
 }
 
-template <int NB>
+template <int NB, int KS = 15>
 static int launch_zrw(ConvParams p, const ConvChoice &c, hipStream_t st) {
     constexpr int TD = 8;
     p.tile_d = TD;
@@ -1344,20 +1357,28 @@
     p.ident_ssh = conv3d_identity_ssh();
     if (!p.ident_ss || !p.ident_ssh) return -2;
     dim3 grid(p.N * p.tiles_h * p.tiles_w * c.segs, (p.Cout / 16) / NB);
-    return fnn_launch_lds<conv3d_zrw_kernel<NB>>(grid, dim3(256), ZrLds<NB, TD>::bytes(), st, p, c.segs, c.tps);
+    return fnn_launch_lds<conv3d_zrw_kernel<NB, KS>>(grid, dim3(256), ZrLds<NB, TD, 8, KS>::bytes(), st, p, c.segs, c.tps);
 }
 
 int launch_conv3d_zr(ConvParams p, const ConvChoice &c, hipStream_t st) {
     const int nb = c.t[0], td = c.t[1];
+    const bool d = c.packing == FNN_PACK_ZRD;
     switch (c.kernel) {
-        case CK_ZS: case CK_ZSP: case CK_ZSW: return launch_zs(p, c, st);
+        case CK_ZS: case CK_ZSP: case CK_ZSW: return d ? launch_zs<14>(p, c, st) : launch_zs<15>(p, c, st);
         case CK_ZR8:
             if (nb == 2) return td == 8 ? launch_zr8<2, 8>(p, st) : launch_zr8<2, 4>(p, st);
             return td == 8 ? launch_zr8<1, 8>(p, st) : launch_zr8<1, 4>(p, st);
         case CK_ZQ12: return launch_conv3d_zq12(p, st);
-        case CK_ZR12: return launch_zr12<4>(p, st);
-        case CK_ZRW: return nb == 2 ? launch_zrw<2>(p, c, st) : launch_zrw<1>(p, c, st);
+        case CK_ZR12: return d ? launch_zr12<4, 14>(p, st) : launch_zr12<4>(p, st);
+        case CK_ZRW:
+            if (d) return nb == 2 ? launch_zrw<2, 14>(p, c, st) : launch_zrw<1, 14>(p, c, st);
+            return nb == 2 ? launch_zrw<2>(p, c, st) : launch_zrw<1>(p, c, st);
         case CK_ZR:
+            if (d) {
+                if (c.t[2] == 6) return launch_zr<2, 10, 6, 14>(p, st);
+                if (nb == 2) return td == 8 ? launch_zr<2, 8, 8, 14>(p, st) : launch_zr<2, 4, 8, 14>(p, st);
+                return td == 8 ? launch_zr<1, 8, 8, 14>(p, st) : launch_zr<1, 4, 8, 14>(p, st);
+            }
             if (c.t[2] == 6) return launch_zr<2, 10, 6>(p, st);
             if (nb == 2) return td == 8 ? launch_zr<2, 8>(p, st) : launch_zr<2, 4>(p, st);
             return td == 8 ? launch_zr<1, 8>(p, st) : launch_zr<1, 4>(p, st);
diff --git a/fast-nnunet_amd/csrc/conv_pack.hip b/fast-nnunet_amd/csrc/conv_pack.hip
--- a/fast-nnunet_amd/csrc/conv_pack.hip
+++ b/fast-nnunet_amd/csrc/conv_pack.hip
@@ -4,7 +4,7 @@
 #include <vector>
 
 int conv3d_ksteps(int packing, int taps) {
-    return packing == FNN_PACK_ZR || packing == FNN_PACK_ZRP ? 15 : packing == FNN_PACK_ZP ? 9 : (taps + 1) / 2;
+    return packing == FNN_PACK_ZR || packing == FNN_PACK_ZRP ? 15 : packing == FNN_PACK_ZRD ? 14 : packing == FNN_PACK_ZP ? 9 : (taps + 1) / 2;
 }
 
 int conv3d_kstep_tap(int packing, int ks, int half, int taps, int ch, int chunks, int *tch) {
@@ -17,12 +17,17 @@
         *tch = ch - 1 + half;
         return dz * 9 + 8;
     }
+    if (packing == FNN_PACK_ZRD) {
+        if (ks < 12) return (ks % 3) * 9 + 2 * (ks / 3) + half;
+        if (ks == 12) return half * 9 + 8;
+        return half ? 2 * 9 + 8 : -1;
+    }
     const int t = 2 * ks + half;
     return t < taps ? t : -1;
 }
 
 int conv3d_pack_cout(int packing, int nblk, int cb, int m) {
-    if ((packing != FNN_PACK_ZR && packing != FNN_PACK_ZRP && packing != FNN_PACK_ZP) || nblk % 2 != 0) return cb * 16 + m;
+    if ((packing != FNN_PACK_ZR && packing != FNN_PACK_ZRP && packing != FNN_PACK_ZRD && packing != FNN_PACK_ZP) || nblk % 2 != 0) return cb * 16 + m;
     return (cb >> 1) * 32 + (m >> 2) * 8 + (cb & 1) * 4 + (m & 3);
 }
 
diff --git a/fast-nnunet_amd/csrc/conv_zr_common.h b/fast-nnunet_amd/csrc/conv_zr_common.h
--- a/fast-nnunet_amd/csrc/conv_zr_common.h
+++ b/fast-nnunet_amd/csrc/conv_zr_common.h
@@ -1,26 +1,26 @@
 #pragma once
 #include "conv_common.h"
 
-template <int NB, int TD, int TH = 8>
+template <int NB, int TD, int TH = 8, int KS = 15>
 struct ZrLds {
     static constexpr int PW = 12, PS = (TH + 2) * PW * 32;
     static constexpr int image = (TD + 2) * PS;
-    static constexpr int weights = NB * 15 * 1024;
+    static constexpr int weights = NB * KS * 1024;
     static constexpr int bytes() { return image + weights; }
 };
-template <int TD, int NW>
+template <int TD, int NW, int KS = 15>
 struct Zr12Lds {
     static constexpr int PW = 20, PS = 14 * PW * 32;
     static constexpr int image = (TD + 2) * PS;
-    static constexpr int weights = 2 * 15 * 1024;
+    static constexpr int weights = 2 * KS * 1024;
     static constexpr int tail = NW * 32 * 2 * 4;
     static constexpr int bytes() { return image + weights + tail; }
 };
-template <int NB, bool RED>
+template <int NB, bool RED, int KS = 15>
 struct ZsLds {
     static constexpr int PW = 17, PS = 9 * PW * 32;
     static constexpr int image = (10 * PS + 1023) & ~1023;
-    static constexpr int weights = NB * 15 * 1024;
+    static constexpr int weights = NB * KS * 1024;
     static constexpr int tail = RED ? 4 * NB * 16 * 2 * 4 : NB * 16 * 4;
     static constexpr int bytes() { return image + weights + tail; }
 };
@@ -34,19 +34,19 @@
 };
 
 template <class Row, class Col, class At>
-static __device__ __forceinline__ void zr_tap_offsets(int (&toff)[5], int lane, Row row_of_r, Col col_of_r, At at) {
+static __device__ __forceinline__ void zr_tap_offsets(int (&toff)[5], int lane, Row row_of_r, Col col_of_r, At at, int dpair = 0) {
     const int r = lane & 15, hl = lane >> 5, kh = (lane >> 4) & 1;
 #pragma unroll
     for (int pr = 0; pr < 5; ++pr) {
         const int tp = 2 * pr + hl < 9 ? 2 * pr + hl : 8;
         const int row = row_of_r(r) + tp / 3, col = col_of_r(r) + tp % 3;
-        toff[pr] = at(row, col, kh);
+        toff[pr] = at(row, col, kh) + (pr == 4 && hl ? dpair : 0);
     }
 }
 template <int PW, bool SWAP, class Row, class Col>
-static __device__ __forceinline__ void zr_tap_offsets(int (&toff)[5], int lane, Row row_of_r, Col col_of_r, int base = 0) {
+static __device__ __forceinline__ void zr_tap_offsets(int (&toff)[5], int lane, Row row_of_r, Col col_of_r, int base = 0, int dpair = 0) {
     zr_tap_offsets(toff, lane, row_of_r, col_of_r,
-                   [base](int row, int col, int kh) { return base + (row * PW + col) * 32 + ((SWAP ? kh ^ (row & 1) : kh) * 16); });
+                   [base](int row, int col, int kh) { return base + (row * PW + col) * 32 + ((SWAP ? kh ^ (row & 1) : kh) * 16); }, dpair);
 }
 
 template <int TDW, int NB, int KS>
@@ -64,17 +64,43 @@
     }
     __builtin_amdgcn_sched_barrier(0);
 }
-template <int TDW, int NB, int KS, class PlaneOff>
+template <int TDW, int NB, class DpairOff>
+static __device__ __forceinline__ void zr_dpair_mfma(f32x4 (&acc)[TDW][NB], const char *bp, const char *sW, int lane, DpairOff dpair_off) {
+    constexpr int KS = 14;
+    f16x8 y[TDW + 1];
+#pragma unroll
+    for (int pl = 0; pl < TDW + 1; ++pl) y[pl] = *(const f16x8 *)(bp + dpair_off(pl));
+#pragma unroll
+    for (int s = 0; s < 2; ++s) {
+        f16x8 wf[NB];
+#pragma unroll
+        for (int nb = 0; nb < NB; ++nb) wf[nb] = *(const f16x8 *)(sW + ((nb * KS + 12 + s) * 64 + lane) * 16);
+#pragma unroll
+        for (int j = 0; j < TDW; ++j)
+#pragma unroll
+            for (int nb = 0; nb < NB; ++nb)
+                acc[j][nb] = __builtin_amdgcn_mfma_f32_16x16x32_f16(wf[nb], y[j + s], acc[j][nb], 0, 0, 0);
+    }
+    __builtin_amdgcn_sched_barrier(0);
+}
+template <int TDW, int NB, int KS, class PlaneOff, class DpairOff>
 static __device__ __forceinline__ void zr_kloop(f32x4 (&acc)[TDW][NB], const char *sA, const int (&toff)[5], const char *sW, int lane,
-                                                PlaneOff plane_off) {
+                                                PlaneOff plane_off, DpairOff dpair_off) {
+    static_assert(KS == 15 || KS == 14, "the padded or the depth-paired order");
 #pragma unroll
-    for (int pr = 0; pr < 5; ++pr) {
+    for (int pr = 0; pr < (KS == 14 ? 4 : 5); ++pr) {
         const char *bp = sA + toff[pr];
         f16x8 xf[TDW + 2];
 #pragma unroll
         for (int pl = 0; pl < TDW + 2; ++pl) xf[pl] = *(const f16x8 *)(bp + plane_off(pl));
         zr_pair_mfma<TDW, NB, KS>(acc, xf, sW, pr, lane);
     }
+    if constexpr (KS == 14) zr_dpair_mfma<TDW, NB>(acc, sA + toff[4], sW, lane, dpair_off);
+}
+template <int TDW, int NB, int KS, class PlaneOff>
+static __device__ __forceinline__ void zr_kloop(f32x4 (&acc)[TDW][NB], const char *sA, const int (&toff)[5], const char *sW, int lane,
+                                                PlaneOff plane_off) {
+    zr_kloop<TDW, NB, KS>(acc, sA, toff, sW, lane, plane_off, plane_off);
 }
 
 typedef int fnn_i32x4 __attribute__((ext_vector_type(4)));
diff --git a/fast-nnunet_amd/csrc/fnn_device.h b/fast-nnunet_amd/csrc/fnn_device.h
--- a/fast-nnunet_amd/csrc/fnn_device.h
+++ b/fast-nnunet_amd/csrc/fnn_device.h
@@ -62,6 +62,7 @@
 #define FNN_PACK_ZR 1
 #define FNN_PACK_ZP 2
 #define FNN_PACK_ZRP 3
+#define FNN_PACK_ZRD 4
 int conv_zp_chunks(int cin_pad0, int cin_pad1);
 void conv_zp_pack(const float *W, int cout_real, int cout_pad, int cin_real0, int cin_pad0, int cin_real1, int cin_pad1, unsigned short *dst);
 
@@ -372,7 +373,7 @@
 };
 struct ConvOverrides {
     bool conv_v1 = false;
-    bool no_row = false, no_stem_row = false, no_zr6 = false, no_zrp = false, no_zq12 = false, no_zsw = false, no_zp = false;
+    bool no_row = false, no_stem_row = false, no_zr6 = false, no_zrp = false, no_zrd = false, no_zq12 = false, no_zsw = false, no_zp = false;
     bool zp_no_half = false, zps_no_half = false;
     int zr_min_wgs = 480;
     int fp8_levels = -1;
```

New measurement: 3618 patches/s, median of 6. No clear change (+0.4%).
